# usexfg/xfg-stark

Measured on AMD Instinct MI355X. Metric: burn-proofs/sec (2^16-step trace, blowup=8), higher is better.
Workload: dtype u64; 1 GPU; batch of 64 burn proofs per GPU (configs[2]; configs[3] = 512 proofs on 8 GPUs); trace_length=65536, blowup=8, proof_options=42/8/4/None/8/31, parallelism=dp1 (independent proofs; RCCL scatter of inputs, gather of proof bytes), submission=pipelined, depth 6 (xfg_prove_batch_submit / xfg_batch_wait)

## Files before the change

include/xfg_stark.h:

```cpp
#ifndef XFG_STARK_H
#define XFG_STARK_H
#include <stddef.h>
#include <stdint.h>
#ifdef __cplusplus
extern "C" {
#endif

typedef struct xfg_ctx xfg_ctx;

typedef enum {
    XFG_OK = 0,
    XFG_INVALID_BURN_AMOUNT = 1,
    XFG_MINT_MISMATCH = 2,
    XFG_ZERO_TX_HASH = 3,
    XFG_BAD_RECIPIENT_LEN = 4,
    XFG_SHORT_SECRET = 5,
    XFG_PROVER_ERROR = 6,
    XFG_DEVICE_ERROR = 7,
    XFG_BUFFER_TOO_SMALL = 8,
    XFG_INVALID_ARGUMENT = 9,
    XFG_VERIFY_FAILED = 10,
    XFG_INVALID_TRACE = 11
} xfg_status;

typedef struct {
    uint32_t num_queries;
    uint32_t blowup_factor;
    uint32_t grinding_factor;
    uint32_t field_extension;
    uint32_t fri_folding_factor;
    uint32_t fri_remainder_max_degree;
} xfg_options;

typedef struct {
    uint64_t burn_amount;
    uint64_t mint_amount;
    uint8_t tx_prefix_hash[32];
    const uint8_t* recipient_address;
    size_t recipient_len;
    const uint8_t* secret;
    size_t secret_len;
    uint32_t network_id;
    uint32_t target_chain_id;
    uint32_t commitment_version;
} xfg_burn_inputs;

typedef struct {
    uint64_t pub_inputs[12];
    uint64_t nullifier;
    uint64_t commitment;
} xfg_air_consts;

xfg_ctx* xfg_ctx_create(int device_id);
void xfg_ctx_destroy(xfg_ctx* ctx);
int xfg_default_options(xfg_options* out);
int xfg_last_error(const xfg_ctx* ctx, char* buf, size_t len);
size_t xfg_proof_size_bound(uint64_t trace_length, const xfg_options* opts);

int xfg_prove_burn_mint(xfg_ctx* ctx, const xfg_burn_inputs* in, uint64_t trace_length, const xfg_options* opts,
                        uint8_t* out, size_t* out_len);
int xfg_prove_trace(xfg_ctx* ctx, const uint64_t* trace, uint32_t width, uint64_t n, const xfg_air_consts* air,
                    const xfg_options* opts, uint8_t* out, size_t* out_len);
int xfg_prove_batch(xfg_ctx* ctx, uint32_t count, const xfg_burn_inputs* inputs, uint64_t trace_length,
                    const xfg_options* opts, uint8_t* const* outs, size_t* out_lens, int* statuses);

int xfg_prove_batch_submit(xfg_ctx* ctx, uint32_t count, const xfg_burn_inputs* inputs, uint64_t trace_length,
                           const xfg_options* opts, uint8_t* const* outs, size_t* out_lens, int* statuses,
                           uint64_t* ticket);
int xfg_batch_wait(xfg_ctx* ctx, uint64_t ticket);

typedef struct {
    uint32_t kind;
    uint32_t index;
    uint32_t column;
    uint64_t step;
    uint64_t expected;
    uint64_t found;
} xfg_trace_fault;

#define XFG_TRACE_VALIDATE   1u
#define XFG_TRACE_ON_DEVICE  2u

int xfg_check_traces(xfg_ctx* ctx, uint32_t count, const uint64_t* traces, uint64_t n, const xfg_air_consts* airs,
                     uint32_t flags, xfg_trace_fault* faults);
int xfg_prove_trace_batch(xfg_ctx* ctx, uint32_t count, const uint64_t* traces, uint32_t width, uint64_t n,
                          const xfg_air_consts* airs, const xfg_options* opts, uint32_t flags, uint8_t* const* outs,
                          size_t* out_lens, int* statuses, xfg_trace_fault* faults);
int xfg_prove_trace_batch_submit(xfg_ctx* ctx, uint32_t count, const uint64_t* traces, uint32_t width, uint64_t n,
                                 const xfg_air_consts* airs, const xfg_options* opts, uint32_t flags,
                                 uint8_t* const* outs, size_t* out_lens, int* statuses, xfg_trace_fault* faults,
                                 uint64_t* ticket);

int xfg_prepare(xfg_ctx* ctx, uint32_t count, uint64_t trace_length, const xfg_options* opts);

int xfg_burn_air_consts(const xfg_burn_inputs* in, xfg_air_consts* out);

typedef struct {
    uint32_t trace_width;
    uint64_t trace_length;
    xfg_options options;
    uint32_t num_unique_queries;
    uint32_t num_fri_layers;
    uint32_t remainder_len;
    uint64_t pow_nonce;
    uint8_t trace_root[32];
    uint8_t constraint_root[32];
    uint64_t ood_trace[14];
    uint64_t ood_composition;
    size_t size;
} xfg_proof_info;

int xfg_proof_parse(const uint8_t* proof, size_t len, xfg_proof_info* info, char* err, size_t err_len);

int xfg_verify(const uint8_t* proof, size_t len, const xfg_air_consts* air, const xfg_options* acceptable, char* err,
               size_t err_len);
int xfg_verify_batch(uint32_t count, const uint8_t* const* proofs, const size_t* lens, const xfg_air_consts* airs,
                     const xfg_options* acceptable, int* results, uint32_t threads);

int xfg_verify_batch_gpu(xfg_ctx* ctx, uint32_t count, const uint8_t* const* proofs, const size_t* lens,
                         const xfg_air_consts* airs, const xfg_options* acceptable, int* results);

int xfg_selftest_blake3(const uint8_t* in, size_t len, uint8_t out[32]);
int xfg_selftest_field(uint64_t a, uint64_t b, uint64_t* out3);
int xfg_set_timing(xfg_ctx* ctx, int enabled);
int xfg_stage_times(const xfg_ctx* ctx, double* ms, const char** names, int max);
int xfg_bench_lde(xfg_ctx* ctx, uint32_t count, uint64_t n, uint32_t blowup, uint32_t iters, double* avg_ms);
int xfg_lde_probe(xfg_ctx* ctx, int enabled, double* total_ms, uint64_t* launch_sets, uint64_t* polys);
int xfg_debug_lde(xfg_ctx* ctx, const uint64_t* coef, uint32_t npoly, uint64_t n, uint32_t blowup, uint64_t* out);
int xfg_debug_interpolate(xfg_ctx* ctx, const uint64_t* evals, uint32_t npoly, uint64_t n, int offset7,
                          uint64_t* out);
int xfg_debug_const_columns(xfg_ctx* ctx, const uint64_t* trace, uint32_t count, uint32_t width, uint64_t n,
                            uint8_t* flags_out);
int xfg_debug_lde_skip(xfg_ctx* ctx, const uint64_t* coef, uint32_t npoly, uint64_t n, uint32_t blowup,
                       const uint8_t* skip, uint64_t* out);
int xfg_debug_interpolate_skip(xfg_ctx* ctx, const uint64_t* evals, uint32_t npoly, uint64_t n, int offset7,
                               const uint8_t* skip, uint64_t* out);
int xfg_debug_field(xfg_ctx* ctx, uint32_t op, uint64_t count, const uint64_t* a, const uint64_t* b, uint64_t* out);
int xfg_debug_ood_deep(xfg_ctx* ctx, uint32_t count, uint64_t n, const uint64_t* coef, const uint64_t* hcoef,
                       const uint64_t* zpts, const uint64_t* coeffs, uint64_t* ood_out, uint64_t* deep_out);
int xfg_debug_ood_deep_e(xfg_ctx* ctx, uint32_t count, uint64_t n, uint32_t ext, const uint64_t* coef,
                         const uint64_t* hcoef, const uint64_t* zpts, const uint64_t* coeffs,
                         const uint32_t* coin_seeds, const uint64_t* coin_counters, uint64_t ginv, uint64_t* ood_out,
                         uint64_t* deep_out, uint64_t* dp_out, uint32_t* seeds_out, uint64_t* counters_out,
                         int* fail_out);
int xfg_debug_constraint_eval(xfg_ctx* ctx, uint32_t count, uint64_t n, uint32_t blowup, uint32_t ext,
                              const uint64_t* trace, const xfg_air_consts* airs, const uint64_t* coeffs,
                              uint64_t* ce);
int xfg_debug_fri_fold(xfg_ctx* ctx, uint32_t count, uint32_t ext, uint32_t logn, uint32_t logbeta, int coset_major,
                       const uint64_t* vals, const uint64_t* alpha, uint64_t* out);
int xfg_debug_fri_fold_f(xfg_ctx* ctx, uint32_t count, uint32_t ext, uint32_t logn, uint32_t logbeta, int coset_major,
                         uint32_t fold, const uint64_t* vals, const uint64_t* alpha, uint64_t* out);
int xfg_debug_coin_draws(xfg_ctx* ctx, const uint32_t seed[8], uint64_t counter, uint32_t k, uint32_t ext,
                         const uint64_t reject[4], uint64_t* out_wave, uint64_t* out_seq, uint64_t counters[2],
                         int ok[2]);
int xfg_debug_merkle_lde(xfg_ctx* ctx, uint32_t count, uint32_t nc, uint64_t n, uint32_t blowup, const uint64_t* lde,
                         const uint64_t* entries, uint64_t nentries, uint8_t* nodes_out, uint8_t* local_out);
int xfg_debug_merkle_lde_const(xfg_ctx* ctx, uint32_t count, uint32_t nc, uint64_t n, uint32_t blowup,
                               const uint64_t* lde, const uint8_t* flags, const uint64_t* vals,
                               const uint64_t* entries, uint64_t nentries, uint8_t* nodes_out, uint8_t* local_out);
int xfg_debug_poison_lde(xfg_ctx* ctx, int on);
int xfg_debug_merkle_fri(xfg_ctx* ctx, uint32_t count, uint32_t ext, uint32_t logn, uint32_t logbeta, int coset_major,
                         const uint64_t* vals, uint8_t* nodes_out);
int xfg_debug_merkle_fri_f(xfg_ctx* ctx, uint32_t count, uint32_t ext, uint32_t logn, uint32_t logbeta, int coset_major,
                           uint32_t fold, const uint64_t* vals, uint8_t* nodes_out);
int xfg_debug_grind(xfg_ctx* ctx, uint32_t count, const uint32_t* seeds, uint32_t grind, uint64_t first_nonce,
                    uint64_t max_nonce, uint32_t chunk_log, uint32_t blocks, uint64_t* nonces_out);
int xfg_grind_probe(const xfg_ctx* ctx, uint32_t* device_min, uint64_t* device_searches, uint64_t* host_searches);
int xfg_debug_verify_batch_gpu(xfg_ctx* ctx, uint32_t count, const uint8_t* const* proofs, const size_t* lens,
                               const xfg_air_consts* airs, const xfg_options* acceptable, int* results,
                               uint64_t* flags, char* errs, size_t err_stride);

#ifdef __cplusplus
}
#endif
#endif
```

xfg-stark_amd/csrc/debug_abi.hip:

```cpp
#include <cstring>
#include <vector>

#include "dev_coin.hpp"
#include "field_dft.hpp"
#include "prover_internal.hpp"

using namespace xfg;

__global__ void field_op_kernel(int op, const u64* a, const u64* b, u64* out, u64 count) {
    const u64 i = (u64)blockIdx.x * blockDim.x + threadIdx.x;
    if (i >= count) return;
    const u64 x = a[i], y = b[i];
    u64 r = 0;
    switch (op) {
        case 0: r = gl_mul(x, y); break;
        case 1: r = gl_add(x, y); break;
        case 2: r = gl_sub(x, y); break;
        case 3: r = gl_canon(x); break;
        case 4: {
            const int sh = (int)(y % 96);
            static_for<96>([&](auto sc) {
                if (sh == decltype(sc)::value) r = mul_pow2<decltype(sc)::value>(x);
            });
            break;
// ... 73 lines not shown
                                  u64* ctr, int* ok, hipStream_t s) {
    hipLaunchKernelGGL(coin_draw_test_kernel, dim3(1), dim3(64), 0, s, c0, k, ext, rej, out_wave, out_seq, ctr, ok);
}

static int debug_lde(xfg_ctx* c, const uint64_t* coef, uint32_t npoly, uint64_t n, uint32_t blowup, const uint8_t* skip,
                     uint64_t* out) {
    if (!c || !coef || !out || !is_pow2(n) || !is_pow2(blowup) || n < 8 || blowup < 2 || blowup > 128)
        return XFG_INVALID_ARGUMENT;
    if (!lde_supported((int)ilog2(n), (int)ilog2(blowup))) return XFG_INVALID_ARGUMENT;
    return on_lane0(c, [&](Lane* L) -> int {
        const int logn = (int)ilog2(n), logbeta = (int)ilog2(blowup);
        const u64 N = n * blowup;
        ensure_tables(c, logn + logbeta);
        ensure_fourstep(c, logn, logbeta);
        Tables T = tables_of(c);
        L->coef.ensure((size_t)npoly * n);
        L->scratch.ensure((size_t)npoly * N);
        L->lde.ensure((size_t)npoly * N);
        HIPCHK(hipMemcpy(L->coef.p, coef, (size_t)npoly * n * 8, hipMemcpyHostToDevice));
        if (skip) {
            L->const_col.ensure(npoly);
            HIPCHK(hipMemcpy(L->const_col.p, skip, npoly, hipMemcpyHostToDevice));
            HIPCHK(hipMemsetAsync(L->scratch.p, 0xFF, (size_t)npoly * N * 8, L->stream));
            HIPCHK(hipMemsetAsync(L->lde.p, 0xFF, (size_t)npoly * N * 8, L->stream));
        }
        launch_lde(L->coef.p, n, L->lde.p, L->scratch.p, npoly, logn, logbeta, T, L->stream, skip ? L->const_col.p : nullptr);
        if (skip) launch_const_fill(L->const_col.p, L->coef.p, n, nullptr, L->lde.p, npoly, logn, logbeta, L->stream);
        std::vector<u64> cm((size_t)npoly * N);
        HIPCHK(hipMemcpyAsync(cm.data(), L->lde.p, cm.size() * 8, hipMemcpyDeviceToHost, L->stream));
        HIPCHK(hipStreamSynchronize(L->stream));
        for (u64 p = 0; p < npoly; p++)
            for (u64 t = 0; t < blowup; t++)
                for (u64 m = 0; m < n; m++) out[p * N + t + blowup * m] = cm[(p * blowup + t) * n + m];
        return XFG_OK;
    });
}

static int debug_interpolate(xfg_ctx* c, const uint64_t* evals, uint32_t npoly, uint64_t n, int offset7,
                             const uint8_t* skip, uint64_t* out) {
    if (!c || !evals || !out || !is_pow2(n) || n < 8 || !ntt_supported((int)ilog2(n), 0, true)) return XFG_INVALID_ARGUMENT;
    return on_lane0(c, [&](Lane* L) -> int {
        const int logn = (int)ilog2(n);
        ensure_tables(c, std::max(logn, c->tables.LM));
        if (logn >= 4) ensure_fourstep(c, logn - 1, 1);
        Tables T = tables_of(c);
        L->trace.ensure((size_t)npoly * n);
        L->coef.ensure((size_t)npoly * n);
        L->scratch.ensure((size_t)npoly * n);
        HIPCHK(hipMemcpy(L->trace.p, evals, (size_t)npoly * n * 8, hipMemcpyHostToDevice));
        if (skip) {
            L->const_col.ensure(npoly);
            HIPCHK(hipMemcpy(L->const_col.p, skip, npoly, hipMemcpyHostToDevice));
            HIPCHK(hipMemsetAsync(L->scratch.p, 0xFF, (size_t)npoly * n * 8, L->stream));
            HIPCHK(hipMemsetAsync(L->coef.p, 0xFF, (size_t)npoly * n * 8, L->stream));
        }
        launch_interpolate(L->trace.p, n, L->coef.p, n, L->scratch.p, npoly, logn, offset7 != 0, n, T, L->stream,
                           skip ? L->const_col.p : nullptr);
        if (skip) launch_const_fill(L->const_col.p, L->trace.p, n, L->coef.p, nullptr, npoly, logn, 0, L->stream);
        HIPCHK(hipMemcpyAsync(out, L->coef.p, (size_t)npoly * n * 8, hipMemcpyDeviceToHost, L->stream));
        HIPCHK(hipStreamSynchronize(L->stream));
        return XFG_OK;
    });
}

extern "C" {

int xfg_bench_lde(xfg_ctx* c, uint32_t count, uint64_t n, uint32_t blowup, uint32_t iters, double* avg_ms) {
    if (!c || !avg_ms || !is_pow2(n) || !is_pow2(blowup) || n < 8 || blowup < 2 || blowup > 128 || iters == 0)
        return XFG_INVALID_ARGUMENT;
    if (!lde_supported((int)ilog2(n), (int)ilog2(blowup))) return XFG_INVALID_ARGUMENT;
    return on_lane0(c, [&](Lane* L) -> int {
        const int logn = (int)ilog2(n), logbeta = (int)ilog2(blowup);
        const u64 N = n * blowup;
        ensure_tables(c, logn + logbeta);
        ensure_fourstep(c, logn, logbeta);
        Tables T = tables_of(c);
        L->coef.ensure((size_t)count * 7 * n);
        L->scratch.ensure((size_t)count * 7 * N);
        L->lde.ensure((size_t)count * 7 * N);
        std::vector<u64> h((size_t)count * 7 * n);
        u64 x = 0x46472d535441524bULL;
        for (auto& v : h) {
            x += 0x9E3779B97F4A7C15ULL;
            u64 z = x;
            z = (z ^ (z >> 30)) * 0xBF58476D1CE4E5B9ULL;
            z = (z ^ (z >> 27)) * 0x94D049BB133111EBULL;
            v = (z ^ (z >> 31)) % P;
        }
        HIPCHK(hipMemcpy(L->coef.p, h.data(), h.size() * 8, hipMemcpyHostToDevice));
        launch_lde(L->coef.p, n, L->lde.p, L->scratch.p, count * 7, logn, logbeta, T, L->stream);
        HIPCHK(hipEventRecord(L->ev[0], L->stream));
        for (uint32_t i = 0; i < iters; i++)
            launch_lde(L->coef.p, n, L->lde.p, L->scratch.p, count * 7, logn, logbeta, T, L->stream);
        HIPCHK(hipEventRecord(L->ev[1], L->stream));
        HIPCHK(hipEventSynchronize(L->ev[1]));
        float ms = 0;
        HIPCHK(hipEventElapsedTime(&ms, L->ev[0], L->ev[1]));
        *avg_ms = ms / iters;
        return XFG_OK;
    });
}

int xfg_lde_probe(xfg_ctx* c, int enabled, double* total_ms, uint64_t* launch_sets, uint64_t* polys) {
    if (!c) return XFG_INVALID_ARGUMENT;
    return on_lane0(c, [&](Lane*) -> int {
        double ms = 0;
        u64 sets = 0, np = 0;
        for (auto& L : c->lanes) {
            ms += L->lde_ms;
            sets += L->lde_sets;
            np += L->lde_polys;
            if (enabled) L->lde_ms = 0, L->lde_sets = 0, L->lde_polys = 0;
            L->lde_probe = enabled != 0;
        }
        if (total_ms) *total_ms = ms;
        c->lde_probe = enabled != 0;
        if (launch_sets) *launch_sets = sets;
        if (polys) *polys = np;
        return XFG_OK;
    });
}

int xfg_debug_lde(xfg_ctx* c, const uint64_t* coef, uint32_t npoly, uint64_t n, uint32_t blowup, uint64_t* out) {
    return debug_lde(c, coef, npoly, n, blowup, nullptr, out);
}
int xfg_debug_lde_skip(xfg_ctx* c, const uint64_t* coef, uint32_t npoly, uint64_t n, uint32_t blowup,
                       const uint8_t* skip, uint64_t* out) {
    if (!skip) return XFG_INVALID_ARGUMENT;
    return debug_lde(c, coef, npoly, n, blowup, skip, out);
}

int xfg_debug_interpolate(xfg_ctx* c, const uint64_t* evals, uint32_t npoly, uint64_t n, int offset7, uint64_t* out) {
    return debug_interpolate(c, evals, npoly, n, offset7, nullptr, out);
}
int xfg_debug_interpolate_skip(xfg_ctx* c, const uint64_t* evals, uint32_t npoly, uint64_t n, int offset7,
                               const uint8_t* skip, uint64_t* out) {
    if (!skip) return XFG_INVALID_ARGUMENT;
    return debug_interpolate(c, evals, npoly, n, offset7, skip, out);
}

int xfg_debug_const_columns(xfg_ctx* c, const uint64_t* trace, uint32_t count, uint32_t width, uint64_t n,
                            uint8_t* flags_out) {
    if (!c || !trace || !flags_out || count == 0 || width == 0 || !is_pow2(n) || n < 8 ||
        (uint64_t)count * width > 0xFFFF)
        return XFG_INVALID_ARGUMENT;
    return on_lane0(c, [&](Lane* L) -> int {
        const size_t cols = (size_t)count * width;
        L->trace.ensure(cols * n);
        L->const_col.ensure(cols);
        HIPCHK(hipMemcpy(L->trace.p, trace, cols * n * 8, hipMemcpyHostToDevice));
        launch_const_detect(L->trace.p, (int)cols, (int)ilog2(n), L->const_col.p, L->stream);
        HIPCHK(hipMemcpyAsync(flags_out, L->const_col.p, cols, hipMemcpyDeviceToHost, L->stream));
        HIPCHK(hipStreamSynchronize(L->stream));
        return XFG_OK;
    });
}

int xfg_debug_field(xfg_ctx* c, uint32_t op, uint64_t count, const uint64_t* a, const uint64_t* b, uint64_t* out) {
    if (!c || !a || !b || !out || op > 12 || count == 0 || (op >= 9 && count % 2)) return XFG_INVALID_ARGUMENT;
    return on_lane0(c, [&](Lane* L) -> int {
        L->trace.ensure((size_t)count * 3);
        u64* da = L->trace.p;
        u64* db = da + count;
        u64* dout = db + count;
        HIPCHK(hipMemcpy(da, a, count * 8, hipMemcpyHostToDevice));
        HIPCHK(hipMemcpy(db, b, count * 8, hipMemcpyHostToDevice));
        launch_field_op((int)op, da, db, dout, count, L->stream);
        HIPCHK(hipMemcpyAsync(out, dout, count * 8, hipMemcpyDeviceToHost, L->stream));
        HIPCHK(hipStreamSynchronize(L->stream));
        return XFG_OK;
    });
}

int xfg_debug_coin_draws(xfg_ctx* c, const uint32_t seed[8], uint64_t counter, uint32_t k, uint32_t ext,
                         const uint64_t reject[4], uint64_t* out_wave, uint64_t* out_seq, uint64_t counters[2],
                         int ok[2]) {
    if (!c || !seed || !reject || !out_wave || !out_seq || !counters || !ok || k == 0 || k > 64 ||
        (ext != 1 && ext != 2))
        return XFG_INVALID_ARGUMENT;
    return on_lane0(c, [&](Lane* L) -> int {
        L->trace.ensure(4 + 4 * (size_t)k + 2 + 1);
        u64* drej = L->trace.p;
        u64* dw = drej + 4;
        u64* ds = dw + 2 * k;
        u64* dctr = ds + 2 * k;
        int* dok = (int*)(dctr + 2);
        HIPCHK(hipMemcpy(drej, reject, 32, hipMemcpyHostToDevice));
        HIPCHK(hipMemset(dw, 0, 16 * (size_t)k));
        DevCoin c0;
        memcpy(c0.seed.w, seed, 32);
        c0.counter = counter;
        c0.pad = 0;
        launch_coin_draw_test(c0, (int)k, (int)ext, drej, dw, ds, dctr, dok, L->stream);
        HIPCHK(hipMemcpyAsync(out_wave, dw, 16 * (size_t)k, hipMemcpyDeviceToHost, L->stream));
        HIPCHK(hipMemcpyAsync(out_seq, ds, 16 * (size_t)k, hipMemcpyDeviceToHost, L->stream));
        HIPCHK(hipMemcpyAsync(counters, dctr, 16, hipMemcpyDeviceToHost, L->stream));
        HIPCHK(hipMemcpyAsync(ok, dok, 8, hipMemcpyDeviceToHost, L->stream));
        HIPCHK(hipStreamSynchronize(L->stream));
        return XFG_OK;
    });
}

int xfg_debug_grind(xfg_ctx* c, uint32_t count, const uint32_t* seeds, uint32_t grind, uint64_t first_nonce,
                    uint64_t max_nonce, uint32_t chunk_log, uint32_t blocks, uint64_t* nonces_out) {
    if (!c || !seeds || !nonces_out || count == 0 || grind > GRIND_MAX || first_nonce == 0 ||
        (chunk_log != 0 && (chunk_log < GRIND_CHUNK_LOG_MIN || chunk_log > GRIND_CHUNK_LOG_MAX)) ||
        blocks > GRIND_FORCED_BLOCKS_MAX)
        return XFG_INVALID_ARGUMENT;
    return on_lane0(c, [&](Lane* L) -> int {
        const GrindPlan gp = grind_plan(grind, count, (unsigned)L->cus);
        memcpy(grind_seeds(L, count), seeds, (size_t)count * sizeof(Digest));
        const u64* got = grind_search(L, (int)count, grind, first_nonce, max_nonce ? max_nonce : gp.max_nonce,
                                      chunk_log ? chunk_log : gp.chunk_log, blocks ? blocks : gp.blocks);
        memcpy(nonces_out, got, (size_t)count * 8);
        return XFG_OK;
    });
}

int xfg_grind_probe(const xfg_ctx* c, uint32_t* device_min, uint64_t* device_searches, uint64_t* host_searches) {
    if (!c) return XFG_INVALID_ARGUMENT;
    uint64_t dev = 0, host = 0;
    for (auto& L : c->lanes) {
        dev += L->grind_dev;
        host += L->grind_host;
    }
    if (device_min) *device_min = GRIND_DEVICE_MIN;
    if (device_searches) *device_searches = dev;
    if (host_searches) *host_searches = host;
    return XFG_OK;
}

int xfg_debug_ood_deep(xfg_ctx* c, uint32_t count, uint64_t n, const uint64_t* coef, const uint64_t* hcoef,
                       const uint64_t* zpts, const uint64_t* coeffs, uint64_t* ood_out, uint64_t* deep_out) {
    return xfg_debug_ood_deep_e(c, count, n, 1, coef, hcoef, zpts, coeffs, nullptr, nullptr, 0, ood_out, deep_out,
                                nullptr, nullptr, nullptr, nullptr);
}

int xfg_debug_ood_deep_e(xfg_ctx* c, uint32_t count, uint64_t n, uint32_t ext, const uint64_t* coef,
                         const uint64_t* hcoef, const uint64_t* zpts, const uint64_t* coeffs,
                         const uint32_t* coin_seeds, const uint64_t* coin_counters, uint64_t ginv, uint64_t* ood_out,
                         uint64_t* deep_out, uint64_t* dp_out, uint32_t* seeds_out, uint64_t* counters_out,
                         int* fail_out) {
    if (!c) return XFG_INVALID_ARGUMENT;
    c->err.clear();
    const bool coin = coin_seeds != nullptr;
    if ((ext != 1 && ext != 2) || !is_pow2(n) || n < 8 || n > (1ULL << 21) || count == 0 || count > 0xFFFF) {
        c->err = "xfg_debug_ood_deep: ext is 1 or 2, n a power of two in [8, 2^21], count in [1, 65535]";
        return XFG_INVALID_ARGUMENT;
    }
    if (!coef || !hcoef || !zpts || !ood_out || !deep_out ||
        (coin ? !coin_counters || !dp_out || !seeds_out || !counters_out || !fail_out : !coeffs)) {
        c->err = "xfg_debug_ood_deep: null argument";
        return XFG_INVALID_ARGUMENT;
    }
    const size_t B = count, D = ext;
    if (!all_canonical(coef, B * 7 * n) || !all_canonical(hcoef, B * D * n) || !all_canonical(zpts, B * 2 * D) ||
        (coin ? ginv >= P : !all_canonical(coeffs, B * 8 * D))) {
        c->err = "xfg_debug_ood_deep: a word is not a canonical field element";
        return XFG_INVALID_ARGUMENT;
    }
    auto e_at = [D](const u64* v) { return E2{v[0], D == 2 ? v[1] : 0}; };
    if (!coin)
        for (size_t k = 0; k < B * 2; k++)
            if (e2_eq(e_at(zpts + k * D), E2{0, 0})) {
                c->err = "xfg_debug_ood_deep: z and z g must not be zero";
                return XFG_INVALID_ARGUMENT;
            }
    return on_lane0(c, [&](Lane* L) -> int {
        const ProofShape sh(n, Opts{0, 2, 0, ext, 8, 31});
        const int logn = sh.logn;
        L->coef.ensure(B * 7 * n);
        size_ood_deep(L, B, sh);
        hipStream_t s = L->stream;
        HIPCHK(hipMemcpyAsync(L->coef.p, coef, B * 7 * n * 8, hipMemcpyHostToDevice, s));
        HIPCHK(hipMemcpyAsync(L->hcoef.p, hcoef, B * D * n * 8, hipMemcpyHostToDevice, s));
        HIPCHK(hipMemcpyAsync(L->zpts.p, zpts, B * 2 * D * 8, hipMemcpyHostToDevice, s));
        const size_t nblk = ood_partial_count(logn);
        HIPCHK(hipMemsetAsync(L->partial.p, 0xFF, B * nblk * 15 * D * 8, s));
        HIPCHK(hipMemsetAsync(L->carry.p, 0xFF, B * nblk * 2 * D * 8, s));
        HIPCHK(hipMemsetAsync(L->ood.p, 0xFF, B * 15 * D * 8, s));
        HIPCHK(hipMemsetAsync(L->dp.p, 0xFF, B * sizeof(DeepParams), s));
        HIPCHK(hipMemsetAsync(L->deep.p, 0xFF, B * D * n * 8, s));
        if (coin) {
            L->dcoin.ensure(B);
            L->dfail.ensure(B);
            std::vector<DevCoin> hc(B);
            for (size_t b = 0; b < B; b++) {
                memcpy(hc[b].seed.w, coin_seeds + 8 * b, 32);
                hc[b].counter = coin_counters[b];
                hc[b].pad = 0;
            }
            HIPCHK(hipMemcpyAsync(L->dcoin.p, hc.data(), B * sizeof(DevCoin), hipMemcpyHostToDevice, s));
            HIPCHK(hipMemsetAsync(L->dfail.p, 0, B * sizeof(int), s));
            DeepCoinStep dc;
            dc.coins = L->dcoin.p;
            dc.fail = L->dfail.p;
            dc.zpts = L->zpts.p;
            dc.dp = L->dp.p;
            dc.ginv = ginv;
            launch_ood(L->coef.p, L->hcoef.p, L->zpts.p, L->partial.p, L->ood.p, logn, (int)B, (int)ext, s, dc);
            launch_deep(L->coef.p, L->hcoef.p, L->dp.p, L->partial.p, L->carry.p, L->deep.p, logn, (int)B, (int)ext, s);
            std::vector<DeepParams> dps(B);
            HIPCHK(hipMemcpyAsync(ood_out, L->ood.p, B * 15 * D * 8, hipMemcpyDeviceToHost, s));
            HIPCHK(hipMemcpyAsync(deep_out, L->deep.p, B * D * n * 8, hipMemcpyDeviceToHost, s));
            HIPCHK(hipMemcpyAsync(dps.data(), L->dp.p, B * sizeof(DeepParams), hipMemcpyDeviceToHost, s));
            HIPCHK(hipMemcpyAsync(hc.data(), L->dcoin.p, B * sizeof(DevCoin), hipMemcpyDeviceToHost, s));
            HIPCHK(hipMemcpyAsync(fail_out, L->dfail.p, B * sizeof(int), hipMemcpyDeviceToHost, s));
            HIPCHK(hipStreamSynchronize(s));
            for (size_t b = 0; b < B; b++) {
                static_assert(sizeof(DeepParams) == 30 * 8, "dp_out: the 28 words before DeepParams::pad");
                memcpy(dp_out + 28 * b, &dps[b], 28 * 8);
                memcpy(seeds_out + 8 * b, hc[b].seed.w, 32);
                counters_out[b] = hc[b].counter;
            }
            return XFG_OK;
        }
        launch_ood(L->coef.p, L->hcoef.p, L->zpts.p, L->partial.p, L->ood.p, logn, (int)B, (int)ext, s);
        HIPCHK(hipMemcpyAsync(ood_out, L->ood.p, B * 15 * D * 8, hipMemcpyDeviceToHost, s));
        HIPCHK(hipStreamSynchronize(s));
        std::vector<DeepParams> dps(B);
        for (size_t b = 0; b < B; b++) {
            DeepParams& dp = dps[b];
            memset(&dp, 0, sizeof dp);
            auto put = [D](u64* d, E2 v) {
                d[0] = v.a;
                if (D == 2) d[1] = v.b;
            };
            const u64* cf = coeffs + b * 8 * D;
            const u64* o = ood_out + b * 15 * D;
            const E2 z = e_at(zpts + b * 2 * D), zg = e_at(zpts + b * 2 * D + D), gamma = e_at(cf + 7 * D);
            E2 c1 = e2_mul(gamma, e_at(o + 14 * D)), c2{0, 0};
            for (int k = 0; k < 7; k++) {
                const E2 a = e_at(cf + k * D);
                put(dp.a[k], a);
                c1 = e2_add(c1, e2_mul(a, e_at(o + 2 * k * D)));
                c2 = e2_add(c2, e2_mul(a, e_at(o + (2 * k + 1) * D)));
            }
            put(dp.gamma, gamma);
            put(dp.z, z);
            put(dp.zg, zg);
            put(dp.zinv, e2_inv(z));
            put(dp.zginv, e2_inv(zg));
            put(dp.c1, c1);
            put(dp.c2, c2);
        }
        HIPCHK(hipMemcpyAsync(L->dp.p, dps.data(), B * sizeof(DeepParams), hipMemcpyHostToDevice, s));
        launch_deep(L->coef.p, L->hcoef.p, L->dp.p, L->partial.p, L->carry.p, L->deep.p, logn, (int)B, (int)ext, s);
        HIPCHK(hipMemcpyAsync(deep_out, L->deep.p, B * D * n * 8, hipMemcpyDeviceToHost, s));
        HIPCHK(hipStreamSynchronize(s));
        return XFG_OK;
    });
}

int xfg_debug_constraint_eval(xfg_ctx* c, uint32_t count, uint64_t n, uint32_t blowup, uint32_t ext,
                              const uint64_t* trace, const xfg_air_consts* airs, const uint64_t* coeffs,
                              uint64_t* ce) {
    if (!c) return XFG_INVALID_ARGUMENT;
    c->err.clear();
    if (!trace || !airs || !coeffs || !ce || count == 0 || !is_pow2(n) || n < 8 || !is_pow2(blowup) || blowup < 2 ||
        blowup > 128 || wide_lde_too_large(n, blowup) || (ext != 1 && ext != 2)) {
        c->err = "xfg_debug_constraint_eval: null or unsupported argument";
        return XFG_INVALID_ARGUMENT;
    }
    return on_lane0(c, [&](Lane* L) -> int {
        const size_t B = count;
        if (!all_canonical(trace, B * 7 * n) || !all_canonical(coeffs, B * 15 * ext)) {
            c->err = "trace element or coefficient is not a canonical field element";
            return XFG_INVALID_ARGUMENT;
        }
        std::vector<AirConst> ha(B);
        for (size_t b = 0; b < B; b++) {
            if (!air_canonical(&airs[b])) {
                c->err = "AIR constant is not a canonical field element";
                return XFG_INVALID_ARGUMENT;
            }
            ha[b] = air_of(&airs[b]);
        }
        const ProofShape sh(n, Opts{0, blowup, 0, ext, 8, 31});
        ensure_tables(c, std::max(sh.logn + sh.logbeta, sh.logn + 1));
        ensure_fourstep(c, sh.logn, sh.logbeta);
        const Tables T = tables_of(c);
        const u64* ce_div = ensure_ce_table(c, sh.logn);
        size_trace_lde(L, B, sh);
        size_constraint_eval(L, B, sh);
        hipStream_t s = L->stream;
        HIPCHK(hipMemcpy(L->trace.p, trace, B * 7 * n * 8, hipMemcpyHostToDevice));
        HIPCHK(hipMemcpy(L->air.p, ha.data(), B * sizeof(AirConst), hipMemcpyHostToDevice));
        HIPCHK(hipMemcpy(L->coeffs.p, coeffs, B * 15 * ext * 8, hipMemcpyHostToDevice));
        launch_trace_lde(L, T, (int)B, sh, false);
        launch_constraint_eval(L->lde.p, L->air.p, L->coeffs.p, ce_div, L->ce.p, sh.logn, sh.logbeta, (int)B, sh.DE, s,
                               trace_const(L, sh));
        HIPCHK(hipMemcpyAsync(ce, L->ce.p, B * ext * 2 * n * 8, hipMemcpyDeviceToHost, s));
        HIPCHK(hipStreamSynchronize(s));
        return XFG_OK;
    });
}

static unsigned debug_logf(uint32_t fold) { return fold == 2 ? 1 : fold == 4 ? 2 : fold == 8 ? 3 : fold == 16 ? 4 : 0; }

int xfg_debug_fri_fold(xfg_ctx* c, uint32_t count, uint32_t ext, uint32_t logn, uint32_t logbeta, int coset_major,
                       const uint64_t* vals, const uint64_t* alpha, uint64_t* out) {
    return xfg_debug_fri_fold_f(c, count, ext, logn, logbeta, coset_major, 8, vals, alpha, out);
}

int xfg_debug_fri_fold_f(xfg_ctx* c, uint32_t count, uint32_t ext, uint32_t logn, uint32_t logbeta, int coset_major,
                         uint32_t fold, const uint64_t* vals, const uint64_t* alpha, uint64_t* out) {
    if (!c) return XFG_INVALID_ARGUMENT;
    c->err.clear();
    const unsigned logf = debug_logf(fold);
    if (!vals || !alpha || !out || count == 0 || (ext != 1 && ext != 2) || logn > 28 || logbeta > 28 || !logf ||
        logn + logbeta < logf + 1 || logn + logbeta > 28) {
        c->err = "xfg_debug_fri_fold: null or unsupported argument";
        return XFG_INVALID_ARGUMENT;
    }
    return on_lane0(c, [&](Lane* L) -> int {
        const size_t B = count;
        const int logD = (int)(logn + logbeta);
        const u64 D = 1ULL << logD, rows = D / fold;
        if (!all_canonical(vals, B * ext * D) || !all_canonical(alpha, B * ext)) {
            c->err = "layer value or alpha is not a canonical field element";
            return XFG_INVALID_ARGUMENT;
        }
        ensure_tables(c, logD);
        const Tables T = tables_of(c);
        L->f0.ensure(B * ext * D);
        L->alpha7.ensure(B * ext);
        L->deep.ensure(B * ext * rows);
        const u64 i7 = gl_inv(GEN);
        std::vector<u64> a7(B * ext);
        for (size_t k = 0; k < a7.size(); k++) a7[k] = gl_mul(alpha[k], i7);
        hipStream_t s = L->stream;
        HIPCHK(hipMemcpy(L->f0.p, vals, B * ext * D * 8, hipMemcpyHostToDevice));
        HIPCHK(hipMemcpy(L->alpha7.p, a7.data(), a7.size() * 8, hipMemcpyHostToDevice));
        launch_fri_fold(L->f0.p, ext * D, D, coset_major != 0, (int)logn, (int)logbeta, rows, logD, L->alpha7.p,
                        L->deep.p, rows, T, (int)B, (int)ext, (int)fold, s);
        HIPCHK(hipMemcpyAsync(out, L->deep.p, B * ext * rows * 8, hipMemcpyDeviceToHost, s));
        HIPCHK(hipStreamSynchronize(s));
        return XFG_OK;
    });
}

static int debug_merkle_lde(xfg_ctx* c, uint32_t count, uint32_t nc, uint64_t n, uint32_t blowup, uint32_t max_blowup,
                            const uint64_t* lde, const uint8_t* flags, const uint64_t* vals, const uint64_t* entries,
                            uint64_t nentries, uint8_t* nodes_out, uint8_t* local_out) {
    if (!c) return XFG_INVALID_ARGUMENT;
    c->err.clear();
    if (!lde || !nodes_out || (nentries && (!entries || !local_out)) || count == 0 || count > 0xFFFF ||
        (nc != 1 && nc != 2 && nc != 7) || !is_pow2(blowup) || blowup < 2 || blowup > max_blowup || !is_pow2(n) ||
        n < 8 || n > (1ULL << 24) || (flags && (!vals || nc != 7))) {
        c->err = "xfg_debug_merkle_lde: null or unsupported argument";
        return XFG_INVALID_ARGUMENT;
    }
    for (uint64_t e = 0; e < nentries; e++)
        if (entries[e] >= (uint64_t)count * n) {
            c->err = "xfg_debug_merkle_lde: entry names a proof or row out of range";
            return XFG_INVALID_ARGUMENT;
        }
    return on_lane0(c, [&](Lane* L) -> int {
        const int logn = (int)ilog2(n), logbeta = (int)ilog2(blowup);
        const size_t B = count, nlde = B * nc * blowup * n, nloc = (size_t)nentries * 2 * blowup;
        L->lde.ensure(nlde);
        L->tnodes.ensure(B * 2 * n);
        hipStream_t s = L->stream;
        HIPCHK(hipMemcpyAsync(L->lde.p, lde, nlde * 8, hipMemcpyHostToDevice, s));
        HIPCHK(hipMemsetAsync(L->tnodes.p, 0xFF, B * 2 * n * sizeof(Digest), s));
        ColConst cc;
        if (flags) {
            const size_t cols = B * nc, N = (size_t)blowup * n;
            L->const_col.ensure((cols + 3) & ~(size_t)3);
            L->coef.ensure(cols);
            HIPCHK(hipMemcpyAsync(L->const_col.p, flags, cols, hipMemcpyHostToDevice, s));
            HIPCHK(hipMemcpyAsync(L->coef.p, vals, cols * 8, hipMemcpyHostToDevice, s));
            for (size_t k = 0; k < cols; k++)
                if (flags[k]) HIPCHK(hipMemsetAsync(L->lde.p + k * N, 0xFF, N * 8, s));
            cc.flags = L->const_col.p;
            cc.vals = L->coef.p;
            cc.val_stride = 1;
        }
        launch_merkle_lde(L->lde.p, (int)nc, L->tnodes.p, (int)B, logn, logbeta, s, CoinStep{}, cc);
        HIPCHK(hipMemcpyAsync(nodes_out, L->tnodes.p, B * 2 * n * sizeof(Digest), hipMemcpyDeviceToHost, s));
        if (nentries) {
            L->scratch.ensure(nentries);
            L->hnodes.ensure(nloc);
            HIPCHK(hipMemcpyAsync(L->scratch.p, entries, nentries * 8, hipMemcpyHostToDevice, s));
            HIPCHK(hipMemsetAsync(L->hnodes.p, 0xFF, nloc * sizeof(Digest), s));
            launch_open_rows(L->lde.p, (int)nc, L->scratch.p, nentries, L->hnodes.p, logn, logbeta, s, cc);
            HIPCHK(hipMemcpyAsync(local_out, L->hnodes.p, nloc * sizeof(Digest), hipMemcpyDeviceToHost, s));
        }
        HIPCHK(hipStreamSynchronize(s));
        return XFG_OK;
    });
}

int xfg_debug_merkle_lde(xfg_ctx* c, uint32_t count, uint32_t nc, uint64_t n, uint32_t blowup, const uint64_t* lde,
                         const uint64_t* entries, uint64_t nentries, uint8_t* nodes_out, uint8_t* local_out) {
    return debug_merkle_lde(c, count, nc, n, blowup, 16, lde, nullptr, nullptr, entries, nentries, nodes_out, local_out);
}
int xfg_debug_merkle_lde_const(xfg_ctx* c, uint32_t count, uint32_t nc, uint64_t n, uint32_t blowup,
                               const uint64_t* lde, const uint8_t* flags, const uint64_t* vals, const uint64_t* entries,
                               uint64_t nentries, uint8_t* nodes_out, uint8_t* local_out) {
// ... 49 lines not shown
```

xfg-stark_amd/csrc/kernels.hip:

```cpp
#include "dev_coin.hpp"
#include "field_dft.hpp"
#include "hip_util.hpp"
#include <algorithm>
#include <stdexcept>

namespace xfg {

#define XFG_CHECK_LAUNCH() (void)hipGetLastError()

__device__ __forceinline__ unsigned brev(unsigned x, int bits) { return __brev(x) >> (32 - bits); }

__device__ __forceinline__ u64 shfl_xor_u64(u64 v, int m, int w) {
    u32 lo = __shfl_xor((u32)v, m, w), hi = __shfl_xor((u32)(v >> 32), m, w);
    return (u64)lo | ((u64)hi << 32);
}

__device__ __forceinline__ u64 tw_pow(const Tables& T, int k, u64 e) {
    u64 M = 1ULL << T.LM;
    return T.tw[(e << (T.LM - k)) & (M - 1)];
}
__device__ __forceinline__ u64 tw_ipow(const Tables& T, int k, u64 e) {
    u64 M = 1ULL << T.LM;
    return T.tw[(M - ((e << (T.LM - k)) & (M - 1))) & (M - 1)];
}

__global__ void trace_gen_kernel(const AirConst* air, u64* trace, int logn) {
    const u64 n = 1ULL << logn;
    const u64 s = (u64)blockIdx.x * blockDim.x + threadIdx.x;
    const int proof = blockIdx.y;
    if (s >= n) return;
    const AirConst& A = air[proof];
    u64* tr = trace + (u64)proof * 7 * n;
    tr[0 * n + s] = A.pub[0];
    tr[1 * n + s] = A.pub[1];
    tr[2 * n + s] = A.pub[2];
    tr[3 * n + s] = A.pub[3];
    tr[4 * n + s] = (4 * s) >> logn;
    tr[5 * n + s] = A.nullifier;
    tr[6 * n + s] = A.commitment;
}
void launch_trace_gen(const AirConst* air, u64* trace, int logn, int npoly, hipStream_t s) {
    u64 n = 1ULL << logn;
    dim3 g((unsigned)((n + 255) / 256), npoly);
    hipLaunchKernelGGL(trace_gen_kernel, g, dim3(256), 0, s, air, trace, logn);
    XFG_CHECK_LAUNCH();
}

__device__ __forceinline__ void air_transition(const AirConst& A, const u64 (&cur)[7], u64 nxt4, u64 (&r)[7]) {
    const u64 std_burn = 8000000ULL, large_burn = 8000000000ULL;
    r[0] = gl_mul(gl_sub(cur[0], std_burn), gl_sub(cur[0], large_burn));
    r[1] = gl_sub(cur[1], cur[0]);
    r[2] = gl_sub(cur[2], A.pub[2] & 0xFFFFFFFFULL);
    r[3] = gl_sub(cur[3], A.pub[3] & 0xFFFFFFFFULL);
    const u64 d = gl_sub(nxt4, cur[4]);
    r[4] = gl_mul(d, gl_sub(d, 1));
    r[5] = gl_sub(cur[5], A.nullifier);
    r[6] = gl_sub(cur[6], A.commitment);
}
__device__ __forceinline__ void air_step0_values(const AirConst& A, u64 (&v0)[7]) {
    v0[0] = A.pub[0]; v0[1] = A.pub[1]; v0[2] = A.pub[2]; v0[3] = A.pub[3];
    v0[4] = 0; v0[5] = A.nullifier; v0[6] = A.commitment;
}

struct CeArgs {
    const u64* lde;
    const AirConst* air;
    const u64* coeffs;
    const u64* div;
    u64* ce;
    int logn, logbeta;
    ColConst cc;
};
template <int D, bool CC>
__global__ __launch_bounds__(256) void constraint_eval_kernel(CeArgs a) {
    using F = FE<D>;
    const u64 n = 1ULL << a.logn, nce = 2 * n;
    const int proof = blockIdx.y;
    const u64 g = (u64)blockIdx.x * blockDim.x + threadIdx.x;
    const u64 par = g >> a.logn, m = g & (n - 1), i = 2 * m + par;
    const AirConst& A = a.air[proof];
    const u64* co = a.coeffs + (u64)proof * 15 * D;
    const u64 beta = 1ULL << a.logbeta;
    const u64* lde = a.lde + (u64)proof * 7 * beta * n;
    const u64 t = par * (beta / 2), mn = (m + 1) & (n - 1);
    u64 cur[7], nxt4;
    if constexpr (CC) {
        const RowConst rc = row_const_uniform(a.cc, (u64)proof);
#pragma unroll
        for (int c = 0; c < 7; c++) {
            if ((rc.mask >> c) & 1) cur[c] = rc.v[c];
            else cur[c] = lde[(((u64)c << a.logbeta) + t) * n + m];
        }
        if ((rc.mask >> 4) & 1) nxt4 = rc.v[4];
        else nxt4 = lde[((4ULL << a.logbeta) + t) * n + mn];
    } else {
#pragma unroll
        for (int c = 0; c < 7; c++) cur[c] = lde[(((u64)c << a.logbeta) + t) * n + m];
        nxt4 = lde[((4ULL << a.logbeta) + t) * n + mn];
    }
    const u64 di = par * n + m;
    const u64 dv0 = a.div[di], dv1 = a.div[nce + di], dv2 = a.div[2 * nce + di];
    u64 r[7];
    air_transition(A, cur, nxt4, r);
    F tr = F::zero();
#pragma unroll
    for (int c = 0; c < 7; c++) tr = fe_add(tr, fe_mulb(F::load(co + c * D), r[c]));
    u64 v0[7];
    air_step0_values(A, v0);
    F b0 = F::zero();
#pragma unroll
    for (int c = 0; c < 7; c++) b0 = fe_add(b0, fe_mulb(F::load(co + (7 + c) * D), gl_sub(cur[c], v0[c])));
    const F b1 = fe_mulb(F::load(co + 14 * D), gl_sub(cur[4], AIR_LAST_STATE));
    F val = fe_mulb(tr, dv0);
    val = fe_add(val, fe_mulb(b0, dv1));
    val = fe_add(val, fe_mulb(b1, dv2));
#pragma unroll
    for (int c = 0; c < D; c++) a.ce[((u64)proof * D + c) * nce + i] = val.c(c);
}
void launch_constraint_eval(const u64* lde, const AirConst* air, const u64* coeffs, const u64* div, u64* ce, int logn,
                            int logbeta, int npoly, int ext, hipStream_t s, const ColConst& cc) {
    CeArgs a;
    a.lde = lde; a.air = air; a.coeffs = coeffs; a.div = div; a.ce = ce; a.logn = logn; a.logbeta = logbeta;
    a.cc = cc;
    u64 nce = 2ULL << logn;
    int threads = nce < 256 ? (int)nce : 256;
    dim3 g((unsigned)(nce / threads), npoly);
    if (cc.flags) {
        if (ext == 2) hipLaunchKernelGGL((constraint_eval_kernel<2, true>), g, dim3(threads), 0, s, a);
        else hipLaunchKernelGGL((constraint_eval_kernel<1, true>), g, dim3(threads), 0, s, a);
    } else {
        if (ext == 2) hipLaunchKernelGGL((constraint_eval_kernel<2, false>), g, dim3(threads), 0, s, a);
        else hipLaunchKernelGGL((constraint_eval_kernel<1, false>), g, dim3(threads), 0, s, a);
    }
    XFG_CHECK_LAUNCH();
}

template <bool AIR>
__global__ __launch_bounds__(256) void trace_check_kernel(u64* trace, const AirConst* air, u64* keys, int logn) {
    const u64 n = 1ULL << logn;
    const u64 s = (u64)blockIdx.x * blockDim.x + threadIdx.x;
    const int proof = blockIdx.y;
    u64 key = TRACE_KEY_VALID;
    if (s < n) {
        u64* tr = trace + (u64)proof * 7 * n;
        u64 cur[7];
#pragma unroll
        for (int c = 0; c < 7; c++) cur[c] = tr[(u64)c * n + s];
        u64 nxt4 = 0;
        if (AIR && s + 1 < n) nxt4 = tr[4 * n + s + 1];
#pragma unroll
        for (int c = 6; c >= 0; c--) {
            if (cur[c] >= P) {
                key = trace_key(TRACE_KEY_NONCANONICAL, s, (unsigned)c);
                cur[c] -= P;
                tr[(u64)c * n + s] = cur[c];
            }
        }
        if (AIR && key == TRACE_KEY_VALID) {
            const AirConst& A = air[proof];
            if (s + 1 < n) {
                if (nxt4 >= P) nxt4 -= P;
                u64 r[7];
                air_transition(A, cur, nxt4, r);
#pragma unroll
                for (int c = 6; c >= 0; c--)
                    if (r[c] != 0) key = trace_key(TRACE_KEY_TRANSITION, s, (unsigned)c);
            } else if (cur[4] != AIR_LAST_STATE) {
                key = trace_key(TRACE_KEY_ASSERTION, s, 7);
            }
            if (s == 0) {
                u64 v0[7];
                air_step0_values(A, v0);
#pragma unroll
                for (int c = 6; c >= 0; c--)
                    if (cur[c] != v0[c]) key = trace_key(TRACE_KEY_ASSERTION, 0, (unsigned)c);
            }
        }
    }
#pragma unroll
    for (int m = 32; m > 0; m >>= 1) {
        const u64 o = shfl_xor_u64(key, m, 64);
        key = o < key ? o : key;
    }
    if ((threadIdx.x & 63) == 0 && key != TRACE_KEY_VALID) atomicMin((unsigned long long*)(keys + proof), (unsigned long long)key);
}
void launch_trace_check(u64* trace, const AirConst* air, u64* keys, int logn, int npoly, bool with_air, hipStream_t s) {
    const u64 n = 1ULL << logn;
    HIPCHK(hipMemsetAsync(keys, 0xFF, (size_t)npoly * 8, s));
    dim3 g((unsigned)((n + 255) / 256), npoly);
    if (with_air) hipLaunchKernelGGL(trace_check_kernel<true>, g, dim3(256), 0, s, trace, air, keys, logn);
    else hipLaunchKernelGGL(trace_check_kernel<false>, g, dim3(256), 0, s, trace, air, keys, logn);
    XFG_CHECK_LAUNCH();
}

#define OOD_R 8
static inline int ood_threads(u64 n) { return (int)std::min<u64>(256, n / OOD_R); }

template <int D>
__device__ __forceinline__ FE<D> fe_pow(FE<D> b, u64 e) {
    FE<D> r = FE<D>::zero();
    r.a = 1;
    while (e) {
        if (e & 1) r = fe_mul(r, b);
        b = fe_mul(b, b);
        e >>= 1;
    }
    return r;
}
template <int D>
__device__ __forceinline__ FE<D> fe_plane(const u64* planes, u64 plane_stride, u64 j) {
    FE<D> v;
    v.a = planes[j];
    if constexpr (D == 2) v.b = planes[plane_stride + j];
    return v;
}

template <int D>
__global__ __launch_bounds__(256) void ood_kernel(const u64* coef, const u64* hcoef, const u64* zpts, u64* partial,
                                                  int logn) {
    using F = FE<D>;
    __shared__ u64 zb[4][D];
    __shared__ u64 red[4][15][D];
    const u64 n = 1ULL << logn;
    const int proof = blockIdx.y, t = threadIdx.x, T = blockDim.x;
    const u64 base = (u64)blockIdx.x * T * OOD_R;
    const F z = F::load(zpts + (u64)proof * 2 * D), zg = F::load(zpts + (u64)proof * 2 * D + D);
    for (int k = t; k < 4; k += T)
        fe_pow(k & 1 ? zg : z, k < 2 ? base : (u64)T).store(zb[k]);
    __syncthreads();
    F pz = fe_mul(F::load(zb[0]), fe_pow(z, (u64)t)), pzg = fe_mul(F::load(zb[1]), fe_pow(zg, (u64)t));
    const F zT = F::load(zb[2]), zgT = F::load(zb[3]);
    const u64* co = coef + (u64)proof * 7 * n;
    const u64* h = hcoef + (u64)proof * D * n;
    F acc[15];
#pragma unroll
    for (int q = 0; q < 15; q++) acc[q] = F::zero();
    u64 cur[7], nxt[7];
    F hc, hn;
    {
        const u64 j = base + t;
#pragma unroll
        for (int c = 0; c < 7; c++) cur[c] = co[(u64)c * n + j];
        hc = fe_plane<D>(h, n, j);
    }
#pragma unroll
    for (int r = 0; r < OOD_R; r++) {
        if (r + 1 < OOD_R) {
            const u64 j = base + (u64)(r + 1) * T + t;
#pragma unroll
            for (int c = 0; c < 7; c++) nxt[c] = co[(u64)c * n + j];
            hn = fe_plane<D>(h, n, j);
        }
#pragma unroll
        for (int c = 0; c < 7; c++) {
            acc[2 * c] = fe_add(acc[2 * c], fe_mulb(pz, cur[c]));
            acc[2 * c + 1] = fe_add(acc[2 * c + 1], fe_mulb(pzg, cur[c]));
        }
        acc[14] = fe_add(acc[14], fe_mul(hc, pz));
        pz = fe_mul(pz, zT);
        pzg = fe_mul(pzg, zgT);
        if (r + 1 < OOD_R) {
#pragma unroll
            for (int c = 0; c < 7; c++) cur[c] = nxt[c];
            hc = hn;
        }
    }
    const int W = T < 64 ? T : 64;
    for (int m = W / 2; m > 0; m >>= 1) {
#pragma unroll
        for (int q = 0; q < 15; q++) {
            acc[q].a = gl_add(acc[q].a, shfl_xor_u64(acc[q].a, m, W));
            if constexpr (D == 2) acc[q].b = gl_add(acc[q].b, shfl_xor_u64(acc[q].b, m, W));
        }
    }
    if ((t & 63) == 0) {
#pragma unroll
        for (int q = 0; q < 15; q++) acc[q].store(red[t >> 6][q]);
    }
    __syncthreads();
    for (int qc = t; qc < 15 * D; qc += T) {
        const int q = qc / D, cc = qc % D;
        u64 v = red[0][q][cc];
        for (int w = 1; w < (T + 63) / 64; w++) v = gl_add(v, red[w][q][cc]);
        partial[((u64)proof * gridDim.x + blockIdx.x) * 15 * D + qc] = v;
    }
}
__device__ void deep_coin_block(const DeepCoinStep& dc, int b, const u64* o, int D) {
    __shared__ u64 ab[8][2];
    __shared__ E2 zinv;
    __shared__ int ok_s;
    const u64* zb = dc.zpts + (u64)b * 2 * D;
    const E2 z{zb[0], D == 2 ? zb[1] : 0}, zg{zb[D], D == 2 ? zb[D + 1] : 0};
    const bool zz = z.a == 0 && z.b == 0;
    if (threadIdx.x < 64) {
        DevCoin c = dc.coins[b];
        dev_reseed(c, dev_hash_elems(o, 14 * D));
        dev_reseed(c, dev_hash_elems(o + 14 * D, D));
        const bool ok = wave_draw_e(c, 8, D, &ab[0][0], 2);
        if (threadIdx.x == 0) {
            dc.coins[b] = c;
            ok_s = ok;
        }
    } else if (threadIdx.x == 64) {
        zinv = zz ? E2{0, 0} : e2_inv(z);
    }
    __syncthreads();
    if (threadIdx.x != 0) return;
    DeepParams P = {};
    for (int k = 0; k < 7; k++)
        for (int d = 0; d < D; d++) P.a[k][d] = ab[k][d];
    for (int d = 0; d < D; d++) P.gamma[d] = ab[7][d];
    auto put = [](u64* d, E2 v) { d[0] = v.a; d[1] = v.b; };
    auto ood_e = [&](int q) { return E2{o[q * D], D == 2 ? o[q * D + 1] : 0}; };
    put(P.z, z);
    put(P.zg, zg);
    put(P.zinv, zinv);
    put(P.zginv, e2_mulb(zinv, dc.ginv));
    E2 c1 = e2_mul(E2{P.gamma[0], P.gamma[1]}, ood_e(14)), c2{0, 0};
    for (int k = 0; k < 7; k++) {
        const E2 a{P.a[k][0], P.a[k][1]};
        c1 = e2_add(c1, e2_mul(a, ood_e(2 * k)));
        c2 = e2_add(c2, e2_mul(a, ood_e(2 * k + 1)));
    }
    put(P.c1, c1);
    put(P.c2, c2);
    dc.dp[b] = P;
    if (!ok_s || zz) dc.fail[b] = 1;
}
__global__ __launch_bounds__(128) void ood_final_kernel(const u64* partial, int nblk, int d, u64* ood, DeepCoinStep dc) {
    __shared__ u64 o[30];
    __shared__ u64 red[8][30];
    const int proof = blockIdx.x, t = threadIdx.x, nq = 15 * d;
    int S = 1;
    while (nq * S * 2 <= (int)blockDim.x && S < 8) S <<= 1;
    const int q = t % nq, k = t / nq;
    if (k < S) {
        const u64* pp = partial + (u64)proof * nblk * nq + q;
        u64 s = 0;
        for (int b0 = k; b0 < nblk; b0 += 8 * S) {
            u64 v[8];
#pragma unroll
            for (int u = 0; u < 8; u++) {
                const int b = b0 + u * S;
                v[u] = b < nblk ? pp[(u64)b * nq] : 0;
            }
#pragma unroll
            for (int u = 0; u < 8; u++) s = gl_add(s, v[u]);
        }
        red[k][q] = s;
    }
    __syncthreads();
    if (t < nq) {
        u64 s = red[0][t];
        for (int j = 1; j < S; j++) s = gl_add(s, red[j][t]);
        ood[(u64)proof * nq + t] = s;
        o[t] = s;
    }
    if (!dc.coins) return;
    __syncthreads();
    deep_coin_block(dc, proof, o, d);
}
void launch_ood(const u64* coef, const u64* hcoef, const u64* zpts, u64* partial, u64* ood, int logn, int npoly,
                int ext, hipStream_t s, const DeepCoinStep& dc) {
    const u64 n = 1ULL << logn;
    const int T = ood_threads(n), nblk = (int)(n / ((u64)T * OOD_R));
    if (ext == 2)
        hipLaunchKernelGGL(ood_kernel<2>, dim3(nblk, npoly), dim3(T), 0, s, coef, hcoef, zpts, partial, logn);
    else
        hipLaunchKernelGGL(ood_kernel<1>, dim3(nblk, npoly), dim3(T), 0, s, coef, hcoef, zpts, partial, logn);
    hipLaunchKernelGGL(ood_final_kernel, dim3(npoly), dim3(dc.coins ? 128 : 64), 0, s, partial, nblk, ext, ood, dc);
    XFG_CHECK_LAUNCH();
}
u64 ood_partial_count(int logn) {
    const u64 n = 1ULL << logn;
    return n / ((u64)ood_threads(n) * OOD_R);
}

template <int D>
__global__ __launch_bounds__(1024) void deep_carry_kernel(const u64* partial, const DeepParams* dp, u64* carry,
                                                          int nblk, int logch) {
    using F = FE<D>;
    __shared__ u64 S1[1024][D], S2[1024][D];
    const int proof = blockIdx.x, b = threadIdx.x;
    const DeepParams& P = dp[proof];
    F b1 = F::zero(), b2 = F::zero();
    if (b < nblk) {
        const u64* pp = partial + ((u64)proof * nblk + b) * 15 * D;
        F t1 = F::zero(), t2 = F::zero();
#pragma unroll
        for (int c = 0; c < 7; c++) {
            const F a = F::load(P.a[c]);
            t1 = fe_add(t1, fe_mul(a, F::load(pp + 2 * c * D)));
            t2 = fe_add(t2, fe_mul(a, F::load(pp + (2 * c + 1) * D)));
        }
        b1 = fe_add(t1, fe_mul(F::load(P.gamma), F::load(pp + 14 * D)));
        b2 = t2;
        if (b == 0) {
            b1 = fe_sub(b1, F::load(P.c1));
            b2 = fe_sub(b2, F::load(P.c2));
        }
    }
    b1.store(S1[b]);
    b2.store(S2[b]);
    __syncthreads();
    for (int off = 1; off < (int)blockDim.x; off <<= 1) {
        F v1 = F::load(S1[b]), v2 = F::load(S2[b]);
        if (b + off < (int)blockDim.x) {
            v1 = fe_add(v1, F::load(S1[b + off]));
            v2 = fe_add(v2, F::load(S2[b + off]));
        }
        __syncthreads();
        v1.store(S1[b]);
        v2.store(S2[b]);
        __syncthreads();
    }
    if (b < nblk) {
        const u64 e = (u64)(b + 1) << logch;
        const F x1 = b + 1 < nblk ? F::load(S1[b + 1]) : F::zero();
        const F x2 = b + 1 < nblk ? F::load(S2[b + 1]) : F::zero();
        fe_mul(x1, fe_pow(F::load(P.zinv), e)).store(carry + (((u64)proof * nblk + b) * 2) * D);
        fe_mul(x2, fe_pow(F::load(P.zginv), e)).store(carry + (((u64)proof * nblk + b) * 2 + 1) * D);
    }
}
__device__ __forceinline__ int dpad(int i) { return i + i / OOD_R; }
template <int D>
__global__ __launch_bounds__(256) void deep_final_kernel(const u64* coef, const u64* hcoef, const DeepParams* dp,
                                                         const u64* carry, u64* deep, int logn) {
    using F = FE<D>;
    constexpr int R = OOD_R, CHMAX = 256 * OOD_R, PADN = CHMAX + CHMAX / R;
    __shared__ u64 s1[D][PADN], s2[D][PADN];
    __shared__ u64 S1[256][D], S2[256][D];
    const u64 n = 1ULL << logn;
    const int proof = blockIdx.y, t = threadIdx.x, T = blockDim.x;
    const u64 base = (u64)blockIdx.x * T * R;
    const DeepParams& P = dp[proof];
    const F z = F::load(P.z), zg = F::load(P.zg), gam = F::load(P.gamma);
    F ac[7];
#pragma unroll
    for (int c = 0; c < 7; c++) ac[c] = F::load(P.a[c]);
    const u64* co = coef + (u64)proof * 7 * n;
    const u64* h = hcoef + (u64)proof * D * n;
    auto lds_ld = [&](u64 (*arr)[PADN], int k) {
        F v;
        v.a = arr[0][k];
        if constexpr (D == 2) v.b = arr[1][k];
        return v;
    };
    auto lds_st = [&](u64 (*arr)[PADN], int k, F v) {
        arr[0][k] = v.a;
        if constexpr (D == 2) arr[1][k] = v.b;
    };
#pragma unroll 2
    for (int r = 0; r < R; r++) {
        const int li = r * T + t;
        const u64 j = base + li;
        F sacc = F::zero();
#pragma unroll
        for (int c = 0; c < 7; c++) sacc = fe_add(sacc, fe_mulb(ac[c], co[(u64)c * n + j]));
        F p1 = fe_add(sacc, fe_mul(gam, fe_plane<D>(h, n, j))), p2 = sacc;
        if (j == 0) {
            p1 = fe_sub(p1, F::load(P.c1));
            p2 = fe_sub(p2, F::load(P.c2));
        }
        lds_st(s1, dpad(li), p1);
        lds_st(s2, dpad(li), p2);
    }
    __syncthreads();
    const int a = t * R;
    F L1 = F::zero(), L2 = F::zero();
#pragma unroll
    for (int i = R - 1; i >= 0; i--) {
        L1 = fe_add(lds_ld(s1, dpad(a + i)), fe_mul(z, L1));
        L2 = fe_add(lds_ld(s2, dpad(a + i)), fe_mul(zg, L2));
    }
    F w1 = z, w2 = zg;
#pragma unroll
    for (int i = 1; i < R; i <<= 1) {
        w1 = fe_mul(w1, w1);
        w2 = fe_mul(w2, w2);
    }
    const F cin1 = F::load(carry + (((u64)proof * gridDim.x + blockIdx.x) * 2) * D);
    const F cin2 = F::load(carry + (((u64)proof * gridDim.x + blockIdx.x) * 2 + 1) * D);
    if (t == T - 1) {
        L1 = fe_add(L1, fe_mul(w1, cin1));
        L2 = fe_add(L2, fe_mul(w2, cin2));
    }
    L1.store(S1[t]);
    L2.store(S2[t]);
    __syncthreads();
    for (int off = 1; off < T; off <<= 1) {
        F v1 = F::load(S1[t]), v2 = F::load(S2[t]);
        if (t + off < T) {
            v1 = fe_add(v1, fe_mul(w1, F::load(S1[t + off])));
            v2 = fe_add(v2, fe_mul(w2, F::load(S2[t + off])));
        }
        __syncthreads();
        v1.store(S1[t]);
        v2.store(S2[t]);
        __syncthreads();
        w1 = fe_mul(w1, w1);
        w2 = fe_mul(w2, w2);
    }
    F q1 = t + 1 < T ? F::load(S1[t + 1]) : cin1, q2 = t + 1 < T ? F::load(S2[t + 1]) : cin2;
#pragma unroll
    for (int i = R - 1; i >= 0; i--) {
        const int k = dpad(a + i);
        const F p1 = lds_ld(s1, k), p2 = lds_ld(s2, k);
        lds_st(s1, k, fe_add(q1, q2));
        q1 = fe_add(p1, fe_mul(z, q1));
        q2 = fe_add(p2, fe_mul(zg, q2));
    }
    __syncthreads();
#pragma unroll
    for (int c = 0; c < D; c++) {
        u64* out = deep + ((u64)proof * D + c) * n + base;
#pragma unroll
        for (int r = 0; r < R; r++) out[r * T + t] = s1[c][dpad(r * T + t)];
    }
}
void launch_deep(const u64* coef, const u64* hcoef, const DeepParams* dp, const u64* partial, u64* carry, u64* deep,
                 int logn, int npoly, int ext, hipStream_t s) {
    const u64 n = 1ULL << logn;
    const int T = ood_threads(n), nblk = (int)(n / ((u64)T * OOD_R));
    int logch = 0;
    while ((1ULL << logch) < (u64)T * OOD_R) logch++;
    int ct = 64;
    while (ct < nblk) ct <<= 1;
    if (ext == 2) {
        hipLaunchKernelGGL(deep_carry_kernel<2>, dim3(npoly), dim3(ct), 0, s, partial, dp, carry, nblk, logch);
        hipLaunchKernelGGL(deep_final_kernel<2>, dim3(nblk, npoly), dim3(T), 0, s, coef, hcoef, dp, carry, deep, logn);
    } else {
        hipLaunchKernelGGL(deep_carry_kernel<1>, dim3(npoly), dim3(ct), 0, s, partial, dp, carry, nblk, logch);
        hipLaunchKernelGGL(deep_final_kernel<1>, dim3(nblk, npoly), dim3(T), 0, s, coef, hcoef, dp, carry, deep, logn);
    }
    XFG_CHECK_LAUNCH();
}

struct FoldArgs {
    const u64* vals;
    u64 val_stride, comp_stride;
    int coset_major, logn, logbeta;
    u64 rows;
    int logD;
    const u64* alpha7;
    u64* out;
    u64 out_stride;
    Tables T;
};
template <int D, int LOGF>
__global__ __launch_bounds__(256) void fri_fold_kernel(FoldArgs a) {
    using F = FE<D>;
    constexpr int NF = 1 << LOGF;
    const int proof = blockIdx.y;
    const u64 i = (u64)blockIdx.x * blockDim.x + threadIdx.x;
    if (i >= a.rows) return;
    const u64* base = a.vals + (u64)proof * a.val_stride;
    u64 c[D][NF];
#pragma unroll
    for (int k = 0; k < NF; k++) {
        const u64 K = i + (u64)k * a.rows;
        c[0][k] = layer_at(base, a.coset_major, a.logn, a.logbeta, K);
        if constexpr (D == 2) c[1][k] = layer_at(base + a.comp_stride, a.coset_major, a.logn, a.logbeta, K);
    }
    F v[NF];
#pragma unroll
    for (int d = 0; d < D; d++) {
        dft_reg<LOGF, true>(c[d]);
#pragma unroll
        for (int k = 0; k < NF; k++) {
            if (d == 0) v[k].a = canon(c[d][k]);
            if constexpr (D == 2) if (d == 1) v[k].b = canon(c[d][k]);
        }
    }
    const F y = fe_mulb(F::load(a.alpha7 + (u64)proof * D), tw_ipow(a.T, a.logD, i));
    F r = v[NF - 1];
#pragma unroll
    for (int j = NF - 2; j >= 0; j--) r = fe_add(fe_mul(r, y), v[j]);
#pragma unroll
    for (int d = 0; d < D; d++) {
        const u64 x = gl_neg(mul_pow2<96 - LOGF>(r.c(d)));
        if (d == 0) r.a = x;
        if constexpr (D == 2) if (d == 1) r.b = x;
    }
#pragma unroll
    for (int c = 0; c < D; c++) a.out[((u64)proof * D + c) * a.out_stride + i] = r.c(c);
}
template <int D>
static void fold_launch(int fold, dim3 g, dim3 b, hipStream_t s, const FoldArgs& a) {
    switch (fold) {
        case 2: hipLaunchKernelGGL((fri_fold_kernel<D, 1>), g, b, 0, s, a); break;
        case 4: hipLaunchKernelGGL((fri_fold_kernel<D, 2>), g, b, 0, s, a); break;
        case 8: hipLaunchKernelGGL((fri_fold_kernel<D, 3>), g, b, 0, s, a); break;
        case 16: hipLaunchKernelGGL((fri_fold_kernel<D, 4>), g, b, 0, s, a); break;
        default: throw std::invalid_argument("FRI fold: no kernel for this folding factor");
    }
}
void launch_fri_fold(const u64* vals, u64 val_stride, u64 comp_stride, bool coset_major, int logn, int logbeta,
                     u64 rows, int logD, const u64* alpha7, u64* out, u64 out_stride, const Tables& T, int npoly,
                     int ext, int fold, hipStream_t s) {
    FoldArgs a;
    a.vals = vals; a.val_stride = val_stride; a.comp_stride = comp_stride; a.coset_major = coset_major ? 1 : 0;
    a.logn = logn; a.logbeta = logbeta; a.rows = rows; a.logD = logD; a.alpha7 = alpha7; a.out = out;
    a.out_stride = out_stride;
    a.T = T;
    int threads = rows < 256 ? (int)rows : 256;
    dim3 g((unsigned)((rows + threads - 1) / threads), npoly);
    if (ext == 2) fold_launch<2>(fold, g, dim3(threads), s, a);
    else fold_launch<1>(fold, g, dim3(threads), s, a);
    XFG_CHECK_LAUNCH();
}

__global__ void gather_set_kernel(GatherSet g, const u64* idx) {
    const u64 i = (u64)blockIdx.x * blockDim.x + threadIdx.x;
    if (i >= g.first[g.nseg]) return;
    int k = 0;
    while (i >= g.first[k + 1]) k++;
    const u64 src = idx[i];
    if (g.digest[k]) {
        const Digest* s = (const Digest*)g.src[k];
        ((Digest*)g.dst[k])[i - g.first[k]] = s[src];
    } else {
        u64 v;
        const u64 plane = src >> g.cc_shift;
        if (k == g.cc_seg && g.cc.flags[plane]) v = g.cc.vals[plane * g.cc.val_stride];
        else v = ((const u64*)g.src[k])[src];
        ((u64*)g.dst[k])[i - g.first[k]] = v;
    }
}
void launch_gather_set(const GatherSet& g, const u64* idx, hipStream_t s) {
    const u64 total = g.first[g.nseg];
    if (!total) return;
    hipLaunchKernelGGL(gather_set_kernel, dim3((unsigned)((total + 255) / 256)), dim3(256), 0, s, g, idx);
    XFG_CHECK_LAUNCH();
}

__global__ void pack_kernel(PackSet p, u32* dst) {
    const int k = blockIdx.y;
    const u32* src = (const u32*)p.src[k];
    u32* out = dst + p.off[k];
    for (u64 i = (u64)blockIdx.x * blockDim.x + threadIdx.x; i < p.words[k]; i += (u64)gridDim.x * blockDim.x)
        out[i] = src[i];
}
void launch_pack(const PackSet& p, void* dst, hipStream_t s) {
    u64 most = 0;
    for (int k = 0; k < p.nseg; k++) most = std::max(most, p.words[k]);
    if (!most) return;
    const unsigned bx = (unsigned)std::min<u64>(32, (most + 255) / 256);
    hipLaunchKernelGGL(pack_kernel, dim3(bx, p.nseg), dim3(256), 0, s, p, (u32*)dst);
    XFG_CHECK_LAUNCH();
}

}
```

xfg-stark_amd/csrc/kernels.hpp:

```cpp
#pragma once
#include <hip/hip_runtime.h>
#include "gl.hpp"
#include "blake3.hpp"
#include "ntt_plan.hpp"

namespace xfg {

struct AirConst {
    u64 pub[12];
    u64 nullifier;
    u64 commitment;
    u64 pad[2];
};

struct DeepParams {
    u64 a[7][2];
    u64 gamma[2];
    u64 z[2], zg[2], zinv[2], zginv[2];
    u64 c1[2], c2[2];
    u64 pad[2];
};

struct FourStep {
    const u64* fwd[FOURSTEP_MAX_LOG + 1][5] = {};
    const u64* inv[FOURSTEP_MAX_LOG + 1] = {};
    const u64* pass_fwd[PASS_MAX_LOG + 1][5] = {};
};
struct Tables {
    const u64* tw;
    int LM;
    const u64* pow7;
    const u64* ipow7;
    const FourStep* fs;
};

void launch_lde(const u64* coef, u64 coef_stride, u64* out, u64* scratch, int npoly, int logn, int logbeta,
                const Tables& T, hipStream_t s, const unsigned char* skip = nullptr);
void build_fourstep(u64* out, int logn, int logbeta, const Tables& T, hipStream_t s);
void build_pass_tables(u64* out, int logn, int logbeta, const Tables& T, hipStream_t s);
void launch_interpolate(const u64* evals, u64 in_stride, u64* out, u64 out_stride, u64* scratch, int npoly, int logn,
                        bool off7, u64 keep, const Tables& T, hipStream_t s, const unsigned char* skip = nullptr);
constexpr int CONST_DETECT_SPAN = 1024, CONST_FILL_SPAN = 4096;
void launch_const_detect(const u64* cols, int ncols, int logn, unsigned char* flags, hipStream_t s);
void launch_const_fill(const unsigned char* flags, const u64* src, u64 src_stride, u64* coef, u64* lde, int ncols,
                       int logn, int logbeta, hipStream_t s);

struct ColConst {
    const unsigned char* flags = nullptr;
    const u64* vals = nullptr;
    u64 val_stride = 0;
};
struct RowConst {
    unsigned mask;
    u64 v[7];
};
__device__ __forceinline__ RowConst row_const_uniform(const ColConst& cc, u64 proof) {
    const u64 o = proof * 7;
    const uint32_t* w = reinterpret_cast<const uint32_t*>(cc.flags) + (o >> 2);
    const unsigned r = (unsigned)(o & 3);
    u64 bytes = ((u64)w[0] | ((u64)w[1] << 32)) >> (8 * r);
    if (r >= 2) bytes |= (u64)w[2] << (64 - 8 * r);
    RowConst rc;
    rc.mask = 0;
#pragma unroll
    for (int c = 0; c < 7; c++) rc.mask |= ((bytes >> (8 * c)) & 0xFF ? 1u : 0u) << c;
    rc.mask = __builtin_amdgcn_readfirstlane(rc.mask);
#pragma unroll
    for (int c = 0; c < 7; c++) {
        rc.v[c] = 0;
        if ((rc.mask >> c) & 1) {
            const u64 v = cc.vals[(o + c) * cc.val_stride];
            const uint32_t lo = (uint32_t)__builtin_amdgcn_readfirstlane((int)(uint32_t)v);
            const uint32_t hi = (uint32_t)__builtin_amdgcn_readfirstlane((int)(uint32_t)(v >> 32));
            rc.v[c] = (u64)lo | ((u64)hi << 32);
        }
    }
    return rc;
}
__device__ __forceinline__ RowConst row_const_lane(const ColConst& cc, u64 proof) {
    RowConst rc;
    rc.mask = 0;
#pragma unroll
    for (int c = 0; c < 7; c++) {
        rc.v[c] = cc.vals[(proof * 7 + c) * cc.val_stride];
        rc.mask |= (cc.flags[proof * 7 + c] ? 1u : 0u) << c;
    }
    return rc;
}

struct DevCoin {
    Digest seed;
    u64 counter;
    u64 pad;
};
struct CoinStep {
    enum Kind : int { NONE = 0, COEFFS = 1, OOD_POINT = 2, FRI_ALPHA = 3 };
    int kind = NONE;
    int ext = 1;
    DevCoin* coins = nullptr;
    int* fail = nullptr;
    u64* out = nullptr;
    u64 g = 0;
    Digest* root_out = nullptr;
    u64* hist = nullptr;
};
struct DeepCoinStep {
    DevCoin* coins = nullptr;
    int* fail = nullptr;
    const u64* zpts = nullptr;
    DeepParams* dp = nullptr;
    u64 ginv = 0;
};

void launch_merkle_lde(const u64* lde, int nc, Digest* nodes, int npoly, int logn, int logbeta, hipStream_t s,
                       const CoinStep& cs = CoinStep{}, const ColConst& cc = ColConst{});
void launch_open_rows(const u64* lde, int nc, const u64* entries, u64 count, Digest* out, int logn, int logbeta,
                      hipStream_t s, const ColConst& cc = ColConst{});
void launch_merkle_fri(const u64* vals, u64 val_stride, u64 comp_stride, bool coset_major, int logn, int logbeta,
                       u64 rows, Digest* nodes, int npoly, int ext, int fold, hipStream_t s,
                       const CoinStep& cs = CoinStep{});

void launch_trace_gen(const AirConst* air, u64* trace, int logn, int npoly, hipStream_t s);
constexpr u64 AIR_LAST_STATE = 3;
constexpr u64 TRACE_KEY_VALID = ~0ULL;
enum : unsigned { TRACE_KEY_NONCANONICAL = 0, TRACE_KEY_ASSERTION = 1, TRACE_KEY_TRANSITION = 2 };
__host__ __device__ constexpr u64 trace_key(unsigned kind, u64 step, unsigned index) {
    return ((u64)kind << 62) | (step << 3) | index;
}
void launch_trace_check(u64* trace, const AirConst* air, u64* keys, int logn, int npoly, bool with_air, hipStream_t s);
void launch_constraint_eval(const u64* lde, const AirConst* air, const u64* coeffs, const u64* div, u64* ce, int logn,
                            int logbeta, int npoly, int ext, hipStream_t s, const ColConst& cc = ColConst{});

void launch_ood(const u64* coef, const u64* hcoef, const u64* zpts, u64* partial, u64* ood, int logn, int npoly,
                int ext, hipStream_t s, const DeepCoinStep& dc = DeepCoinStep{});
u64 ood_partial_count(int logn);
void launch_deep(const u64* coef, const u64* hcoef, const DeepParams* dp, const u64* partial, u64* carry, u64* deep,
                 int logn, int npoly, int ext, hipStream_t s);

__device__ __forceinline__ u64 layer_at(const u64* base, bool coset_major, int logn, int logbeta, u64 K) {
    if (!coset_major) return base[K];
    u64 t = K & ((1ULL << logbeta) - 1), m = K >> logbeta;
    return base[(t << logn) + m];
}
void launch_fri_fold(const u64* vals, u64 val_stride, u64 comp_stride, bool coset_major, int logn, int logbeta,
                     u64 rows, int logD, const u64* alpha7, u64* out, u64 out_stride, const Tables& T, int npoly,
                     int ext, int fold, hipStream_t s);

struct GatherSet {
    static constexpr int MAX = 24;
    int nseg = 0;
    const void* src[MAX];
    void* dst[MAX];
    int digest[MAX];
    u64 first[MAX + 1] = {0};
    int cc_seg = -1, cc_shift = 0;
    ColConst cc;
};
void launch_gather_set(const GatherSet& g, const u64* idx, hipStream_t s);

struct PackSet {
    static constexpr int MAX = 12;
    int nseg = 0;
    const void* src[MAX];
    u64 off[MAX], words[MAX];
};
void launch_pack(const PackSet& p, void* dst, hipStream_t s);

constexpr size_t grind_state_words(size_t B) { return 2 * ((B + 1) & ~(size_t)1); }
void launch_grind(const Digest* seeds, u64* state, u64* out, unsigned B, unsigned grind, u64 first, u64 max_nonce,
                  unsigned chunk_log, unsigned blocks, hipStream_t s);

}
```

xfg-stark_amd/csrc/lane_unit.hip:

```cpp
#include <algorithm>
#include <chrono>
#include <cstring>

#include "host_pool.hpp"
#include "prover_internal.hpp"

namespace xfg {

static void stage_mark(Lane* c, int k, hipStream_t on = nullptr) {
    if (c->timing) HIPCHK(hipEventRecord(c->ev[k], on ? on : c->stream));
}

static hipStream_t gather_stream(Lane* c) {
    if (!c->gstream) {
        int least = 0, greatest = 0;
        if (hipDeviceGetStreamPriorityRange(&least, &greatest) != hipSuccess) greatest = 0;
        HIPCHK(hipStreamCreateWithPriority(&c->gstream, hipStreamNonBlocking, greatest));
    }
    return c->gstream;
}

void size_trace_lde(Lane* c, size_t B, const ProofShape& sh) {
    c->trace.ensure(B * 7 * sh.n);
    c->coef.ensure(B * 7 * sh.n);
    c->scratch.ensure(B * 7 * sh.N);
    c->lde.ensure(B * 7 * sh.N);
    c->const_col.ensure((B * 7 + 3) & ~(size_t)3);
}
void size_constraint_eval(Lane* c, size_t B, const ProofShape& sh) {
    c->air.ensure(B);
    c->coeffs.ensure(B * 15 * sh.DE);
    c->ce.ensure(B * sh.DE * 2 * sh.n);
}
void size_ood_deep(Lane* c, size_t B, const ProofShape& sh) {
    c->hcoef.ensure(B * sh.DE * sh.n);
    c->zpts.ensure(B * 2 * sh.DE);
    c->partial.ensure(B * 15 * sh.DE * ood_partial_count(sh.logn));
    c->ood.ensure(B * 15 * sh.DE);
    c->dp.ensure(B);
    c->carry.ensure(B * 2 * sh.DE * ood_partial_count(sh.logn));
    c->deep.ensure(B * sh.DE * sh.n);
}

static void size_lane_buffers(Lane* c, size_t B, const ProofShape& sh, const Opts& o, const TraceSrc& ts) {
    const u64 n = sh.n, N = sh.N;
    const size_t DE = sh.DE;
    const unsigned nl = sh.nl;
    size_trace_lde(c, B, sh);
    size_constraint_eval(c, B, sh);
    size_ood_deep(c, B, sh);
    c->tnodes.ensure(B * 2 * n);
    c->hlde.ensure(B * DE * N);
    c->hnodes.ensure(B * 2 * n);
    c->f0.ensure(B * DE * N);
    c->alpha7.ensure(B * DE);
    c->falpha.ensure((size_t)std::max(1u, nl) * B * DE);
    c->dn2.ensure(B * DE);
    c->dcoin.ensure(B);
    c->dfail.ensure(B);
    c->droots.ensure((size_t)(2 + nl) * B);
    if (c->flayer.size() < nl + 1) {
        c->flayer.resize(nl + 1);
        c->fnodes.resize(nl + 1);
    }
    for (unsigned l = 0; l < nl; l++) {
        c->fnodes[l].ensure(B * 2 * (sh.D[l] / o.fold));
        c->flayer[l + 1].ensure(B * DE * sh.D[l + 1]);
    }
    c->rem.ensure(B * DE * std::max<u64>(sh.rem_len, 1));
    const size_t q = o.q, depth = sh.logn + sh.logbeta;
    const size_t vals = B * q * (7 + DE + o.fold * DE * nl);
    size_t digs = B * q * 2 * depth;
    for (unsigned l = 0; l < nl; l++) digs += B * q * ilog2(sh.D[l] / o.fold);
    const size_t opens = B * q * 2 * 2 * 2 * sh.beta;
    c->h_idx.ensure(vals + digs + B * 2 * q);
    c->h_gv.ensure(vals);
    c->h_gd.ensure(digs + opens);
    size_grind(c, B);
    if (ts.checks()) c->tkeys.ensure(B);
    if (ts.kind == TraceSrc::HOST_STAGED || ts.size_staging) c->h_trace.ensure(B * 7 * n);
}

static void upload(void* dst, const void* host, size_t bytes, hipStream_t s) {
    void* hd = nullptr;
    HIPCHK(hipHostGetDevicePointer(&hd, const_cast<void*>(host), 0));
    PackSet u;
    u.src[0] = hd;
    u.off[0] = 0;
    u.words[0] = bytes / 4;
    u.nseg = 1;
    launch_pack(u, dst, s);
}
static_assert(sizeof(AirConst) % 4 == 0 && sizeof(DevCoin) % 4 == 0, "uploads copy 32-bit words");

void size_grind(Lane* c, size_t B) {
    c->h_gseed.ensure(B);
    c->h_gnonce.ensure(B);
    c->gseed.ensure(B);
    c->gstate.ensure(grind_state_words(B));
}
Digest* grind_seeds(Lane* c, size_t B) {
    size_grind(c, B);
    return c->h_gseed.p;
}
const u64* grind_search(Lane* c, int B, unsigned grind, u64 first, u64 max_nonce, unsigned chunk_log, unsigned blocks) {
    size_grind(c, B);
    const hipStream_t s = gather_stream(c);
    void* out = nullptr;
    HIPCHK(hipHostGetDevicePointer(&out, c->h_gnonce.p, 0));
    upload(c->gseed.p, c->h_gseed.p, (size_t)B * sizeof(Digest), s);
    launch_grind(c->gseed.p, c->gstate.p, (u64*)out, (unsigned)B, grind, first, max_nonce, chunk_log, blocks, s);
    HIPCHK(hipStreamSynchronize(s));
    return c->h_gnonce.p;
}

static void upload_unit_inputs(Lane* c, ProofJob* jobs, int B, const ProofShape& sh, const Opts& o) {
    hipStream_t s = c->stream;
    AirConst* airs = c->h_air.ensure(B);
    for (int b = 0; b < B; b++) airs[b] = jobs[b].air;
    upload(c->air.p, airs, B * sizeof(AirConst), s);
    DevCoin* hc = c->h_coin.ensure(B);
    for (int b = 0; b < B; b++) {
        ProofJob& j = jobs[b];
        u64 e[20];
        context_elements(sh.n, o, e);
        memcpy(e + 8, j.air.pub, 12 * 8);
        j.coin.init(e, 20);
        j.commitments.clear();
        hc[b].seed = j.coin.seed;
        hc[b].counter = j.coin.counter;
        hc[b].pad = 0;
    }
    upload(c->dcoin.p, hc, B * sizeof(DevCoin), s);
    HIPCHK(hipMemsetAsync(c->dfail.p, 0, B * sizeof(int), s));
}

ColConst trace_const(const Lane* c, const ProofShape& sh) {
    ColConst cc;
    cc.flags = c->const_col.p;
    cc.vals = c->coef.p;
    cc.val_stride = sh.n;
    return cc;
}

void launch_trace_lde(Lane* c, const Tables& T, int B, const ProofShape& sh, bool probe) {
    hipStream_t s = c->stream;
    const unsigned char* skip = c->const_col.p;
    if (c->poison_lde) HIPCHK(hipMemsetAsync(c->lde.p, 0xFF, (size_t)B * 7 * sh.N * 8, s));
    launch_const_detect(c->trace.p, B * 7, sh.logn, c->const_col.p, s);
    launch_interpolate(c->trace.p, sh.n, c->coef.p, sh.n, c->scratch.p, B * 7, sh.logn, false, sh.n, T, s, skip);
    if (probe) {
        if (!c->lde_ev[0]) {
            HIPCHK(hipEventCreate(&c->lde_ev[0]));
            HIPCHK(hipEventCreate(&c->lde_ev[1]));
        }
        HIPCHK(hipEventRecord(c->lde_ev[0], s));
    }
    launch_lde(c->coef.p, sh.n, c->lde.p, c->scratch.p, B * 7, sh.logn, sh.logbeta, T, s, skip);
    if (probe) HIPCHK(hipEventRecord(c->lde_ev[1], s));
    launch_const_fill(skip, c->trace.p, sh.n, c->coef.p, nullptr, B * 7, sh.logn, sh.logbeta, s);
}

static void enqueue_fri_layers(Lane* c, const Tables& T, int B, const ProofShape& sh, int fold, CoinStep& cs,
                               HostTrace& ht) {
    hipStream_t s = c->stream;
    const int DE = sh.DE;
    const unsigned nl = sh.nl;
    for (unsigned l = 0; l < nl; l++) {
        const u64 rows = sh.D[l] / fold;
        const bool cm = (l == 0);
        const u64* src = cm ? c->f0.p : c->flayer[l].p;
        const u64 cstride = cm ? sh.N : sh.D[l], sstride = DE * cstride;
        cs.kind = CoinStep::FRI_ALPHA;
        cs.out = c->alpha7.p;
        cs.hist = c->falpha.p + (size_t)l * B * DE;
        cs.root_out = c->droots.p + (size_t)(2 + l) * B;
        launch_merkle_fri(src, sstride, cstride, cm, sh.logn, sh.logbeta, rows, c->fnodes[l].p, B, DE, fold, s, cs);
        launch_fri_fold(src, sstride, cstride, cm, sh.logn, sh.logbeta, rows, (int)ilog2(sh.D[l]), c->alpha7.p,
                        c->flayer[l + 1].p, rows, T, B, DE, fold, s);
    }
    ht.mark("chain_launch");
    if (nl > 0) {
        launch_interpolate(c->flayer[nl].p, sh.D[nl], c->rem.p, sh.rem_len, c->scratch.p, B * DE,
                           (int)ilog2(sh.D[nl]), true, sh.rem_len, T, s);
    } else {
        HIPCHK(hipMemcpy2DAsync(c->rem.p, sh.rem_len * 8, c->deep.p, sh.n * 8, sh.rem_len * 8, (size_t)B * DE,
                                hipMemcpyDeviceToDevice, s));
    }
}

static ReplayView pack_replay_block(Lane* c, size_t B, const ProofShape& sh, bool with_keys) {
    const size_t DE = sh.DE, nl = sh.nl;
    PackSet pk;
    u64 words = 0;
    auto seg = [&](const void* src, size_t bytes) {
        const u64 at = words;
        pk.src[pk.nseg] = src;
        pk.off[pk.nseg] = at;
        pk.words[pk.nseg++] = bytes / 4;
        words = (at + bytes / 4 + 63) & ~63ULL;
        return at * 4;
    };
    const u64 o_roots = seg(c->droots.p, (2 + nl) * B * sizeof(Digest));
    const u64 o_ood = seg(c->ood.p, B * 15 * DE * 8);
    const u64 o_co = seg(c->coeffs.p, B * 15 * DE * 8);
    const u64 o_dp = seg(c->dp.p, B * sizeof(DeepParams));
    const u64 o_falpha = seg(c->falpha.p, nl * B * DE * 8);
    const u64 o_fail = seg(c->dfail.p, B * sizeof(int));
    const u64 o_rem = seg(c->rem.p, B * DE * sh.rem_len * 8);
    const u64 o_dn2 = seg(c->dn2.p, B * DE * 8);
    const u64 o_const = seg(c->const_col.p, (B * 7 + 3) & ~(size_t)3);
    const u64 o_keys = with_keys ? seg(c->tkeys.p, B * 8) : 0;
    unsigned char* hx = c->h_xfer.ensure(words * 4);
    void* hx_dev = nullptr;
    HIPCHK(hipHostGetDevicePointer(&hx_dev, hx, 0));
    launch_pack(pk, hx_dev, c->stream);
    ReplayView rv;
    rv.roots = (const Digest*)(hx + o_roots);
    rv.ood = (const u64*)(hx + o_ood);
    rv.co = (const u64*)(hx + o_co);
    rv.dps = (const DeepParams*)(hx + o_dp);
    rv.falpha = (const u64*)(hx + o_falpha);
    rv.ffail = (const int*)(hx + o_fail);
    rv.remh = (const u64*)(hx + o_rem);
    rv.dn2h = (const u64*)(hx + o_dn2);
    c->h_const_col = hx + o_const;
    c->h_tkeys = with_keys ? (const u64*)(hx + o_keys) : nullptr;
    return rv;
}

static ReplayView enqueue_commit_chain(Lane* c, const Tables& T, const u64* ce_div, ProofJob* jobs, int B,
                                       const TraceSrc& ts, const ProofShape& sh, const Opts& o, u64 g,
                                       HostTrace& ht) {
    const u64 n = sh.n;
    const int logn = sh.logn, logbeta = sh.logbeta, DE = sh.DE;
    hipStream_t s = c->stream;
    upload_unit_inputs(c, jobs, B, sh, o);
    ht.mark("setup");
    stage_mark(c, 0);
    const size_t tbytes = (size_t)7 * n * 8;
    switch (ts.kind) {
        case TraceSrc::GENERATED: launch_trace_gen(c->air.p, c->trace.p, logn, B, s); break;
        case TraceSrc::HOST_DIRECT:
            HIPCHK(hipMemcpyAsync(c->trace.p, ts.p, B * tbytes, hipMemcpyHostToDevice, s));
            break;
        case TraceSrc::HOST_STAGED: {
            u64* st = c->h_trace.p;
            const u64* src = ts.p;
            const int* refused = ts.refused;
            host_pool().parallel_for(B, [st, src, refused, n, tbytes](int b) {
                if (refused[b]) memset(st + (size_t)b * 7 * n, 0, tbytes);
                else memcpy(st + (size_t)b * 7 * n, src + (size_t)b * 7 * n, tbytes);
            });
            HIPCHK(hipMemcpyAsync(c->trace.p, st, B * tbytes, hipMemcpyHostToDevice, s));
            break;
        }
        case TraceSrc::DEVICE:
            HIPCHK(hipMemcpyAsync(c->trace.p, ts.p, B * tbytes, hipMemcpyDeviceToDevice, s));
            break;
    }
    if (ts.checks()) launch_trace_check(c->trace.p, c->air.p, c->tkeys.p, logn, B, ts.validate, s);
    launch_trace_lde(c, T, B, sh, c->lde_probe);
    stage_mark(c, 1);
    CoinStep cs;
    cs.ext = DE;
    cs.coins = c->dcoin.p;
    cs.fail = c->dfail.p;
    cs.kind = CoinStep::COEFFS;
    cs.out = c->coeffs.p;
    cs.root_out = c->droots.p;
    const ColConst cc = trace_const(c, sh);
    launch_merkle_lde(c->lde.p, 7, c->tnodes.p, B, logn, logbeta, s, cs, cc);
    stage_mark(c, 2);
    launch_constraint_eval(c->lde.p, c->air.p, c->coeffs.p, ce_div, c->ce.p, logn, logbeta, B, DE, s, cc);
    stage_mark(c, 3);
    launch_interpolate(c->ce.p, 2 * n, c->hcoef.p, n, c->scratch.p, B * DE, logn + 1, true, n, T, s);
    launch_lde(c->hcoef.p, n, c->hlde.p, c->scratch.p, B * DE, logn, logbeta, T, s);
    stage_mark(c, 4);
    cs.kind = CoinStep::OOD_POINT;
    cs.out = c->zpts.p;
    cs.root_out = c->droots.p + B;
    cs.g = g;
    launch_merkle_lde(c->hlde.p, DE, c->hnodes.p, B, logn, logbeta, s, cs);
    stage_mark(c, 5);
    DeepCoinStep dc;
    dc.coins = c->dcoin.p;
    dc.fail = c->dfail.p;
    dc.zpts = c->zpts.p;
    dc.dp = c->dp.p;
    dc.ginv = gl_inv(g);
    launch_ood(c->coef.p, c->hcoef.p, c->zpts.p, c->partial.p, c->ood.p, logn, B, DE, s, dc);
    stage_mark(c, 6);
    launch_deep(c->coef.p, c->hcoef.p, c->dp.p, c->partial.p, c->carry.p, c->deep.p, logn, B, DE, s);
    launch_lde(c->deep.p, n, c->f0.p, c->scratch.p, B * DE, logn, logbeta, T, s);
    HIPCHK(hipMemcpy2DAsync(c->dn2.p, 8, c->deep.p + (n - 2), n * 8, 8, (size_t)B * DE, hipMemcpyDeviceToDevice, s));
    stage_mark(c, 7);
    enqueue_fri_layers(c, T, B, sh, (int)o.fold, cs, ht);
    const ReplayView rv = pack_replay_block(c, B, sh, ts.checks());
    stage_mark(c, 8);
    ht.mark("launch_rem");
    return rv;
}

struct Gathered {
    const u64* gv;
    const Digest* gd;
};
static Gathered enqueue_gathers(Lane* c, const ProofShape& sh, const OpeningIndex& ix, HostTrace& ht) {
    const size_t nvals = ix.nvals, ndig = ix.ndig, nent = ix.nent, nopen = nent * 2 * sh.beta;
    u64* hidx = c->h_idx.ensure(ix.allidx.size());
    memcpy(hidx, ix.allidx.data(), ix.allidx.size() * 8);
    u64* gv = c->h_gv.ensure(nvals);
    Digest* gd = c->h_gd.ensure(ndig + 2 * nopen);
    void *didx = nullptr, *dgv = nullptr, *dgd = nullptr;
    HIPCHK(hipHostGetDevicePointer(&didx, hidx, 0));
    HIPCHK(hipHostGetDevicePointer(&dgv, gv, 0));
    HIPCHK(hipHostGetDevicePointer(&dgd, gd, 0));
    const u64* gidx = (const u64*)didx;
    u64* gval = (u64*)dgv;
    Digest* gdig = (Digest*)dgd;
    ht.mark("q_idx_host");
    const hipStream_t sq = gather_stream(c);
    ht.mark("q_h2d");
    GatherSet gs;
    size_t vo = 0, dof = 0, gbase = 0;
    auto add = [&](const void* src, void* dst, bool dig, size_t cnt) {
        if (gs.nseg == GatherSet::MAX) {
            launch_gather_set(gs, gidx + gbase, sq);
            gbase += gs.first[gs.nseg];
            gs = GatherSet{};
        }
        gs.src[gs.nseg] = src;
        gs.dst[gs.nseg] = dst;
        gs.digest[gs.nseg] = dig ? 1 : 0;
        gs.first[gs.nseg + 1] = gs.first[gs.nseg] + cnt;
        gs.nseg++;
    };
    const u64* vsrc[2] = {c->lde.p, c->hlde.p};
    const ColConst cc = trace_const(c, sh);
    gs.cc_seg = 0;
    gs.cc_shift = sh.logn + sh.logbeta;
    gs.cc = cc;
    for (size_t k = 0; k < ix.vseg.size(); k++) {
        const u64* src = k < 2 ? vsrc[k] : (k == 2 ? c->f0.p : c->flayer[k - 2].p);
        add(src, gval + vo, false, ix.vseg[k].second);
        vo += ix.vseg[k].second;
    }
    for (size_t k = 0; k < ix.dseg.size(); k++) {
        const Digest* src = k == 0 ? c->tnodes.p : (k == 1 ? c->hnodes.p : c->fnodes[k - 2].p);
        add(src, gdig + dof, true, ix.dseg[k].second);
        dof += ix.dseg[k].second;
    }
    launch_gather_set(gs, gidx + gbase, sq);
    const u64* ent = gidx + nvals + ndig;
    launch_open_rows(c->lde.p, 7, ent, nent, gdig + ndig, sh.logn, sh.logbeta, sq, cc);
    launch_open_rows(c->hlde.p, sh.DE, ent, nent, gdig + ndig + nopen, sh.logn, sh.logbeta, sq);
    ht.mark("q_launch");
    stage_mark(c, 9, sq);
    return Gathered{gv, gd};
}

void prove_lane(Lane* c, const Tables& T, const u64* ce_div, ProofJob* jobs, int B, const TraceSrc& ts,
                       u64 n, const Opts& o) {
    using clk = std::chrono::steady_clock;
    const auto t_host0 = clk::now();
    HostTrace ht;
    ht.mark("start");
    const ProofShape sh(n, o);
    const u64 g = gl_root(sh.logn);
    HostPool& pool = host_pool();

    size_lane_buffers(c, B, sh, o, ts);
    const ReplayView rv = enqueue_commit_chain(c, T, ce_div, jobs, B, ts, sh, o, g, ht);
    HIPCHK(hipStreamSynchronize(c->stream));
    ht.mark("sync_rem");
    u64 live_cols = 0;
    for (int k = 0; k < B * 7; k++) live_cols += c->h_const_col[k] ? 0 : 1;
    pool.parallel_for(B, [jobs, B, &sh, g, &rv](int b) { replay_transcript(jobs[b], b, B, sh, g, rv); });

    const auto t_q0 = clk::now();
    std::vector<LaneLayout>& lay = c->hs.lay;
    if (lay.size() < (size_t)B) lay.resize(B);
    if (o.grind < GRIND_DEVICE_MIN) {
        pool.parallel_for(B, [jobs, &sh, &o, &rv, &lay](int b) { plan_queries(jobs[b], b, sh, o, rv, lay[b]); });
        c->grind_host += (u64)B;
    } else {
        pool.parallel_for(B, [jobs, &sh, &rv, &lay](int b) { plan_commit_remainder(jobs[b], b, sh, rv, lay[b]); });
        Digest* seeds = grind_seeds(c, B);
        for (int b = 0; b < B; b++) seeds[b] = jobs[b].coin.seed;
        const GrindPlan gp = grind_plan((unsigned)o.grind, (uint32_t)B, (unsigned)c->cus);
        const u64* nonces = grind_search(c, B, (unsigned)o.grind, 1, gp.max_nonce, gp.chunk_log, gp.blocks);
        ht.mark("grind");
        for (int b = 0; b < B; b++) {
            if (nonces[b] == 0) {
                jobs[b].status = XFG_PROVER_ERROR;
                jobs[b].pow_exhausted = true;
            } else if (nonces[b] > gp.max_nonce || pow_zeros(jobs[b].coin.seed, nonces[b]) < o.grind) {
                throw std::runtime_error("device / host transcript diverged");
            }
        }
        pool.parallel_for(B, [jobs, &sh, &o, nonces, &lay](int b) { plan_openings(jobs[b], b, sh, o, nonces[b], lay[b]); });
        c->grind_dev += (u64)B;
    }
    ht.mark("queries_plan");
    OpeningIndex& ix = c->hs.ix;
    concat_indices(lay, B, sh, ix);
    const Gathered got = enqueue_gathers(c, sh, ix, ht);
    const auto t_q1 = clk::now();
    ht.mark("queries_host");
    HIPCHK(hipStreamSynchronize(c->gstream));
    ht.mark("sync_gather");
    const auto t_s0 = clk::now();

    pool.parallel_for(B, [jobs, B, &sh, &o, &lay, &ix, got](int b) {
        serialize_proof(jobs[b], b, B, sh, o, lay[b], ix, got.gv, got.gd);
    });
    ht.mark("serialize");
    for (int b = 0; b < B && ts.kind != TraceSrc::GENERATED; b++) {
        const u64 key = c->h_tkeys ? c->h_tkeys[b] : TRACE_KEY_VALID;
        const bool refused = ts.refused && ts.refused[b];
        if (ts.keys && !refused) ts.keys[b] = key;
        if (refused) jobs[b].status = ts.refused[b];
        else if (key != TRACE_KEY_VALID)
            jobs[b].status = (key >> 62) == TRACE_KEY_NONCANONICAL ? XFG_INVALID_ARGUMENT : XFG_INVALID_TRACE;
    }
    ht.dump(B, (long)((u64)B * 7 - live_cols));
    if (c->lde_probe) {
        float ms = 0;
        HIPCHK(hipEventSynchronize(c->lde_ev[1]));
        HIPCHK(hipEventElapsedTime(&ms, c->lde_ev[0], c->lde_ev[1]));
        c->lde_ms += ms;
        c->lde_sets++;
        c->lde_polys += live_cols;
    }
    if (c->timing) {
        for (int k = 0; k < 9; k++) {
            float ms = 0;
            HIPCHK(hipEventElapsedTime(&ms, c->ev[k], c->ev[k + 1]));
            c->stage_ms[k] = ms;
        }
        const auto t_end = clk::now();
        c->stage_ms[ST_HOST] = std::chrono::duration<double, std::milli>(t_end - t_host0).count();
        c->stage_ms[ST_HQUERY] = std::chrono::duration<double, std::milli>(t_q1 - t_q0).count();
        c->stage_ms[ST_HSER] = std::chrono::duration<double, std::milli>(t_end - t_s0).count();
    }
}

static void create_lane_stream(xfg_ctx* c, Lane* L) {
    L->lde_probe = c->lde_probe;
    L->poison_lde = c->poison_lde;
    HIPCHK(hipDeviceGetAttribute(&L->cus, hipDeviceAttributeMultiprocessorCount, c->device));
    HIPCHK(hipStreamCreateWithFlags(&L->stream, hipStreamNonBlocking));
    for (auto& e : L->ev) HIPCHK(hipEventCreate(&e));
}
Lane* lane0(xfg_ctx* c) {
    if (c->lanes.empty()) {
        c->lanes.emplace_back(new Lane());
        create_lane_stream(c, c->lanes[0].get());
    }
    return c->lanes[0].get();
}
void ensure_lanes(xfg_ctx* c, size_t k) {
    lane0(c);
    while (c->lanes.size() < k) {
        c->lanes.emplace_back(new Lane());
        create_lane_stream(c, c->lanes.back().get());
    }
    for (auto& L : c->lanes) gather_stream(L.get());
}

}
```

xfg-stark_amd/csrc/merkle.hip:

```cpp
#include "dev_coin.hpp"
#include <algorithm>
#include <stdexcept>
#include <type_traits>

namespace xfg {

#define XFG_CHECK_LAUNCH() (void)hipGetLastError()

constexpr u64 ROW2_MIN_N = 1024, ROW2_MAX_BLOCKS = 1024;
constexpr int LEAF_LANES_LOG = 1;
constexpr int UP_WMIN = 64;
constexpr int TREE_MID_WMIN = 64, TREE_MID_SHRINK = 8;
constexpr u64 MID4_MAX_BLOCKS = 256;
constexpr u64 TREE_TOP_MAX = 512;

__device__ __forceinline__ void lds_level(Digest& d, bool have, int slot, Digest* lds, int half, Digest* dst) {
    const int t = threadIdx.x;
    if (have) lds[slot] = d;
    __syncthreads();
    if (t < half) {
        d = b3_merge(lds[2 * t], lds[2 * t + 1]);
        dst[t] = d;
    }
}
__device__ __forceinline__ void block_tree_up(Digest d, Digest* nodes, u64 count, Digest* lds, int wmin) {
    u64 c = count;
    for (int w = blockDim.x; w > wmin; w >>= 1) {
        c >>= 1;
        lds_level(d, true, threadIdx.x, lds, w / 2, nodes + c + (u64)blockIdx.x * (w / 2));
        __syncthreads();
    }
}
__device__ __forceinline__ void quad_level(const Digest* src, bool act, int i, int q, Digest* lds, Digest* dst) {
    uint2 o = make_uint2(0, 0);
    if (act) {
        uint32_t m[16];
#pragma unroll
        for (int w = 0; w < 8; w++) {
            m[w] = src[2 * i].w[w];
            m[8 + w] = src[2 * i + 1].w[w];
        }
        o = b3_merge_quad(m, q);
    }
    __syncthreads();
    if (act) {
        lds[i].w[q] = o.x;
        lds[i].w[4 + q] = o.y;
        dst[i].w[q] = o.x;
        dst[i].w[4 + q] = o.y;
    }
    __syncthreads();
}

struct NoConst {};
template <bool CC>
using RowConstOf = std::conditional_t<CC, RowConst, NoConst>;
template <int NC, int LOGB, bool CC>
__device__ __forceinline__ void lde_row(const u64* base, u64 n, u64 m, int t, const RowConstOf<CC>& rc, u64 (&row)[NC]) {
    static_assert(!CC || NC == 7, "constant columns are those of the trace");
#pragma unroll
    for (int c = 0; c < NC; c++) {
        if constexpr (CC) {
            if ((rc.mask >> c) & 1) {
                row[c] = rc.v[c];
                continue;
            }
        }
        row[c] = base[((u64)c * (1 << LOGB) + t) * n + m];
    }
}

template <int NC, int LOGB, int LOG, int T0, bool CC>
__device__ __forceinline__ Digest lde_subtree(const u64* base, u64 n, u64 m, const RowConstOf<CC>& rc) {
    if constexpr (LOG == 0) {
        u64 row[NC];
        lde_row<NC, LOGB, CC>(base, n, m, T0, rc, row);
        return b3_hash_elems<NC>(row);
    } else {
        Digest l = lde_subtree<NC, LOGB, LOG - 1, T0, CC>(base, n, m, rc);
        Digest r = lde_subtree<NC, LOGB, LOG - 1, T0 + (1 << (LOG - 1)), CC>(base, n, m, rc);
        return b3_merge(l, r);
    }
}

template <int NC, int LOGB, int LOG, bool CC>
__device__ __forceinline__ Digest lde_subtree_wide(const u64* base, u64 n, u64 m, int t0, const RowConstOf<CC>& rc) {
    if constexpr (LOG <= 4) {
        return lde_subtree<NC, LOGB, LOG, 0, CC>(base + (u64)t0 * n, n, m, rc);
    } else {
        Digest l, d;
#pragma unroll 1
        for (int i = 0; i < 2; i++) {
            d = lde_subtree_wide<NC, LOGB, LOG - 1, CC>(base, n, m, t0 + (i << (LOG - 1)), rc);
            if (i == 0) l = d;
        }
        return b3_merge(l, d);
    }
}

template <bool CC>
__device__ __forceinline__ RowConstOf<CC> block_row_const(const ColConst& cc, int proof) {
    if constexpr (CC) return row_const_uniform(cc, (u64)proof);
    else return NoConst{};
}

template <int NC, int LOGB, bool CC>
__global__ __launch_bounds__(256) void leaves_row_kernel(const u64* lde, Digest* nodes_all,
                                                         u64 node_stride, int logn, ColConst cc) {
    __shared__ Digest lds[256];
    const u64 n = 1ULL << logn;
    const int proof = blockIdx.y;
    const u64 m = (u64)blockIdx.x * blockDim.x + threadIdx.x;
    const u64* base = lde + (u64)proof * NC * (1 << LOGB) * n;
    const RowConstOf<CC> rc = block_row_const<CC>(cc, proof);
    Digest d = lde_subtree_wide<NC, LOGB, LOGB, CC>(base, n, m, 0, rc);
    block_tree_up(d, nodes_all + (u64)proof * node_stride, n, lds, blockDim.x / 4);
}

template <int LOGB>
constexpr int leaf_lanes_log() { return LOGB < LEAF_LANES_LOG ? LOGB : LEAF_LANES_LOG; }
template <int NC, int LOGB, bool CC>
__global__ __launch_bounds__(256) void leaves_row2_kernel(const u64* lde, Digest* nodes_all,
                                                          u64 node_stride, int logn, ColConst cc) {
    constexpr int LOGL = leaf_lanes_log<LOGB>(), RB = 256 >> LOGL;
    __shared__ Digest lds[RB];
    const u64 n = 1ULL << logn;
    const int proof = blockIdx.y, t = threadIdx.x, h = t & ((1 << LOGL) - 1), rl = t >> LOGL;
    const u64 m = (u64)blockIdx.x * RB + rl;
    const u64* base = lde + (u64)proof * NC * (1 << LOGB) * n + (u64)h * (1 << (LOGB - LOGL)) * n;
    const RowConstOf<CC> rc = block_row_const<CC>(cc, proof);
    Digest d = lde_subtree_wide<NC, LOGB, LOGB - LOGL, CC>(base, n, m, 0, rc);
#pragma unroll
    for (int k = 0; k < LOGL; k++) {
        Digest r;
#pragma unroll
        for (int w = 0; w < 8; w++) r.w[w] = __shfl_xor(d.w[w], 1 << k);
        d = (h >> k) & 1 ? b3_merge(r, d) : b3_merge(d, r);
    }
    Digest* nodes = nodes_all + (u64)proof * node_stride;
    lds_level(d, h == 0, rl, lds, RB / 2, nodes + n / 2 + (u64)blockIdx.x * (RB / 2));
    __syncthreads();
    lds_level(d, t < RB / 2, t, lds, RB / 4, nodes + n / 4 + (u64)blockIdx.x * (RB / 4));
}

template <int LOGB>
constexpr int open_lanes_log() { return LOGB < 6 ? LOGB : 6; }
template <int NC, int LOGB, bool CC>
__global__ __launch_bounds__(64) void open_rows_kernel(const u64* lde, const u64* entries, u64 count, Digest* out,
                                                       int logn, ColConst cc) {
    constexpr int LOGL = open_lanes_log<LOGB>(), LPL = LOGB - LOGL;
    static_assert(LPL <= 1, "at most two leaves per lane");
    const u64 g = (u64)blockIdx.x * blockDim.x + threadIdx.x;
    const u64 e = g >> LOGL;
    const int t = (int)(g & ((1 << LOGL) - 1)) << LPL;
    if (e >= count) return;
    const u64 n = 1ULL << logn, ent = entries[e];
    const u64 proof = ent >> logn, m = ent & (n - 1);
    const u64* base = lde + proof * NC * (1 << LOGB) * n;
    Digest* local = out + e * (2 << LOGB);
    RowConstOf<CC> rc;
    if constexpr (CC) rc = row_const_lane(cc, proof);
    u64 row[NC];
    lde_row<NC, LOGB, CC>(base, n, m, t, rc, row);
    Digest d = b3_hash_elems<NC>(row);
    local[(1 << LOGB) + t] = d;
    if constexpr (LPL == 1) {
        lde_row<NC, LOGB, CC>(base, n, m, t + 1, rc, row);
        const Digest d1 = b3_hash_elems<NC>(row);
        local[(1 << LOGB) + t + 1] = d1;
        d = b3_merge(d, d1);
        local[((1 << LOGB) + t) >> 1] = d;
    }
#pragma unroll
    for (int k = LPL + 1; k <= LOGB; k++) {
        Digest r;
#pragma unroll
        for (int w = 0; w < 8; w++) r.w[w] = __shfl_xor(d.w[w], 1 << (k - 1 - LPL));
        d = b3_merge(d, r);
        if ((t & ((1 << k) - 1)) == 0) local[((1 << LOGB) + t) >> k] = d;
    }
}

template <int V>
using IntC = std::integral_constant<int, V>;
template <int NC, class F>
static bool with_logbeta(int logbeta, F f) {
    switch (logbeta) {
        case 1: f(IntC<NC>{}, IntC<1>{}); return true;
        case 2: f(IntC<NC>{}, IntC<2>{}); return true;
        case 3: f(IntC<NC>{}, IntC<3>{}); return true;
        case 4: f(IntC<NC>{}, IntC<4>{}); return true;
        case 5: f(IntC<NC>{}, IntC<5>{}); return true;
        case 6: f(IntC<NC>{}, IntC<6>{}); return true;
        case 7: f(IntC<NC>{}, IntC<7>{}); return true;
        default: return false;
    }
}
template <class F>
static void with_nc_logbeta(int nc, int logbeta, F f) {
    const bool found = nc == 7   ? with_logbeta<7>(logbeta, f)
                       : nc == 2 ? with_logbeta<2>(logbeta, f)
                       : nc == 1 ? with_logbeta<1>(logbeta, f)
                                 : false;
    if (!found) throw std::invalid_argument("Merkle kernels: no instantiation for this column count and blowup");
}

static void require_trace_width(int nc, const ColConst& cc) {
    if (cc.flags && nc != 7) throw std::invalid_argument("Merkle kernels: constant columns are those of a 7-column trace LDE");
}
template <class F>
static void with_const_logbeta(int logbeta, F f) {
    if (!with_logbeta<7>(logbeta, f))
        throw std::invalid_argument("Merkle kernels: no instantiation for this column count and blowup");
}

void launch_open_rows(const u64* lde, int nc, const u64* entries, u64 count, Digest* out, int logn, int logbeta,
                      hipStream_t s, const ColConst& cc) {
    if (!count) return;
    require_trace_width(nc, cc);
    const int logl = logbeta < 6 ? logbeta : 6;
    dim3 g((unsigned)(((count << logl) + 63) / 64)), b(64);
    if (cc.flags)
        with_const_logbeta(logbeta, [&](auto NC, auto LB) {
            hipLaunchKernelGGL((open_rows_kernel<decltype(NC)::value, decltype(LB)::value, true>), g, b, 0, s, lde, entries, count, out, logn, cc);
        });
    else
        with_nc_logbeta(nc, logbeta, [&](auto NC, auto LB) {
            hipLaunchKernelGGL((open_rows_kernel<decltype(NC)::value, decltype(LB)::value, false>), g, b, 0, s, lde, entries, count, out, logn, cc);
        });
    XFG_CHECK_LAUNCH();
}

__device__ void coin_root_step(const CoinStep& cs, int b, const Digest& root) {
    const int D = cs.ext, lane = threadIdx.x;
    DevCoin c = cs.coins[b];
    dev_reseed(c, root);
    bool ok;
    if (cs.kind == CoinStep::COEFFS) {
        ok = wave_draw_e(c, 15, D, cs.out + (u64)b * 15 * D, D);
    } else {
        u64 a[2] = {0, 0};
        ok = dev_draw_e(c, a, D);
        if (cs.kind == CoinStep::OOD_POINT) {
            if (a[0] == 0 && a[1] == 0) ok = false;
            if (lane == 0)
                for (int k = 0; k < D; k++) {
                    cs.out[(u64)b * 2 * D + k] = a[k];
                    cs.out[(u64)b * 2 * D + D + k] = gl_mul(a[k], cs.g);
                }
        } else if (lane == 0) {
            const u64 inv7 = 0x249249246DB6DB6EULL;
            for (int k = 0; k < D; k++) cs.out[(u64)b * D + k] = gl_mul(a[k], inv7);
            if (cs.hist)
                for (int k = 0; k < D; k++) cs.hist[(u64)b * D + k] = a[k];
        }
    }
    if (lane == 0) {
        if (!ok) cs.fail[b] = 1;
        cs.coins[b] = c;
        if (cs.root_out) cs.root_out[b] = root;
    }
}

__global__ __launch_bounds__(1024) void tree_top_kernel(Digest* nodes_all, u64 node_stride, u64 count, CoinStep cs) {
    __shared__ Digest lds[256];
    Digest* nodes = nodes_all + (u64)blockIdx.x * node_stride;
    const int tid = threadIdx.x, i = tid >> 2, q = tid & 3;
    for (u64 c = count; c > 1; c >>= 1) {
        const u64 half = c >> 1;
        quad_level(c == count ? nodes + c : lds, i < (int)half, i, q, lds, nodes + half);
    }
    if (cs.kind != CoinStep::NONE && tid < 64) coin_root_step(cs, blockIdx.x, count > 1 ? lds[0] : nodes[1]);
}
__global__ __launch_bounds__(256) void tree_mid_kernel(Digest* nodes_all, u64 node_stride, u64 count) {
    __shared__ Digest lds[256];
    Digest* nodes = nodes_all + (u64)blockIdx.y * node_stride;
    const u64 i = (u64)blockIdx.x * 256 + threadIdx.x;
    const Digest d = b3_merge(nodes[count + 2 * i], nodes[count + 2 * i + 1]);
    nodes[count / 2 + i] = d;
    block_tree_up(d, nodes, count / 2, lds, TREE_MID_WMIN);
}
__global__ __launch_bounds__(256) void tree_mid4_kernel(Digest* nodes_all, u64 node_stride, u64 count) {
    __shared__ Digest lds[64];
    Digest* nodes = nodes_all + (u64)blockIdx.y * node_stride;
    const int tid = threadIdx.x, i = tid >> 2, q = tid & 3;
    u64 c = count, first = (u64)blockIdx.x * 64;
    for (int w = 64; w >= 16; w >>= 1, c >>= 1, first >>= 1)
        quad_level(w == 64 ? nodes + c + 2 * first : lds, i < w, i, q, lds, nodes + c / 2 + first);
}
static void finish_tree(Digest* nodes, u64 node_stride, u64 count, int npoly, hipStream_t s, const CoinStep& cs) {
    while (count > TREE_TOP_MAX) {
        if ((count / 512) * (u64)npoly < MID4_MAX_BLOCKS)
            hipLaunchKernelGGL(tree_mid4_kernel, dim3((unsigned)(count / 128), npoly), dim3(256), 0, s, nodes,
                               node_stride, count);
        else
            hipLaunchKernelGGL(tree_mid_kernel, dim3((unsigned)(count / 512), npoly), dim3(256), 0, s, nodes,
                               node_stride, count);
        count /= TREE_MID_SHRINK;
    }
    if (count > 1 || cs.kind != CoinStep::NONE) {
        int threads = (int)(2 * count);
        threads = threads < 64 ? 64 : threads;
        hipLaunchKernelGGL(tree_top_kernel, dim3(npoly), dim3(threads), 0, s, nodes, node_stride, count, cs);
    }
    XFG_CHECK_LAUNCH();
}

void launch_merkle_lde(const u64* lde, int nc, Digest* nodes, int npoly, int logn, int logbeta, hipStream_t s,
                       const CoinStep& cs, const ColConst& cc) {
    const u64 n = 1ULL << logn, node_stride = 2 * n;
    require_trace_width(nc, cc);
    if (n >= ROW2_MIN_N && (u64)npoly * (n / 256) < ROW2_MAX_BLOCKS) {
        const int logl = logbeta < LEAF_LANES_LOG ? logbeta : LEAF_LANES_LOG;
        dim3 g((unsigned)(n >> (8 - logl)), npoly), b(256);
// ... 75 lines not shown
```

xfg-stark_amd/csrc/ntt.hip:

```cpp
#include <algorithm>
#include <atomic>
#include <cstdlib>
#include <string>
#include <type_traits>
#include <utility>
#include "hip_util.hpp"
#include "kernels.hpp"
#include "field_dft.hpp"
#include "ntt_plan.hpp"

namespace xfg {

typedef u32 u32x2 __attribute__((__vector_size__(8)));
__device__ __forceinline__ __amdgpu_buffer_rsrc_t buf_rsrc(const u64* p) {
    const u64 a = (u64)p;
    const u64 u = (u64)(u32)__builtin_amdgcn_readfirstlane((int)(u32)a) |
                  ((u64)(u32)__builtin_amdgcn_readfirstlane((int)(u32)(a >> 32)) << 32);
    return __builtin_amdgcn_make_buffer_rsrc(reinterpret_cast<void*>(u), (short)0, -1, 0x00020000);
}
__device__ __forceinline__ u64 buf_ld(__amdgpu_buffer_rsrc_t r, u32 voff, u32 soff) {
    const u32x2 v = __builtin_amdgcn_raw_buffer_load_b64(r, (int)voff, (int)soff, 0);
    return (u64)v[0] | ((u64)v[1] << 32);
}
__device__ __forceinline__ void buf_st(__amdgpu_buffer_rsrc_t r, u32 voff, u32 soff, u64 x) {
// ... 603 lines not shown
    constexpr int R1 = 1 << PLB::FIRST_LOGR, G1 = C / R1;
    static_assert(PLB::NSTEP > 1 && (1 << LOGE) == R1, "one full-radix first-step group per thread");
    constexpr int logTR = LOGT + LOGE - LOGC, TR = 1 << logTR;
    extern __shared__ u64 lds[];
    u64* tile = lds;
    u64* ltw = lds + lds_pass_b(LOGC, LOGT, LOGE, LOGT + LOGE - LOGC).tw;
    {
        const u64* pt4 = a.pt + a.tab().wC();
        for (int i = threadIdx.x; i < C; i += NT) ltw[i] = pt4[i];
    }
    __syncthreads();
    const u64 n = 1ULL << a.logn;
    const int per_x = gridDim.x >> 3, x = blockIdx.x & 7, slot = blockIdx.x >> 3;
    const int span = (ntiles + 7) >> 3, tend = min((x + 1) * span, ntiles);
    const int seq0 = threadIdx.x / G1, j0 = threadIdx.x % G1;
    auto load = [&](int ti, u64* dst) -> bool {
        const int pt = ti / ntx, k10 = (ti - pt * ntx) * TR;
        if (a.skipped(pt >> a.logbeta)) return true;
        const u64* y = a.y + (u64)pt * n + ((u64)(k10 + seq0) << LOGC) + j0;
#pragma unroll
        for (int r = 0; r < R1; r++) dst[r] = y[r * G1];
        return false;
    };
    int ti = x * span + slot;
    u64 yv[R1] = {};
    bool skip_cur = ti < tend && load(ti, yv);
    for (; ti < tend; ti += per_x) {
        const int pt = ti / ntx, k10 = (ti - pt * ntx) * TR;
        u64 nx[R1] = {};
        const bool skip_nx = ti + per_x < tend && load(ti + per_x, nx);
        if (skip_cur) {
#pragma unroll
            for (int r = 0; r < R1; r++) yv[r] = nx[r];
            skip_cur = skip_nx;
            continue;
        }
        auto ldg = [&](int, int, int o) -> u64 { return yv[o / G1]; };
        u64* out = a.plane_out(pt) + k10;
        auto stg = [&](int, int seq, int base, int stride, u64* v) {
            u64 o[RR];
#pragma unroll
            for (int r = 0; r < RR; r++) o[r] = canon(v[r]);
            store_pairs<RR>(o, [&](int r) { return out + (seq & ~1) + ((u64)(base + r * stride) << a.logR); });
        };
        pass_dft<LOGC, LOGE, false, false, NT>(tile, logTR, ltw, ldg, stg, [](int, int, int, int) {});
#pragma unroll
        for (int r = 0; r < R1; r++) yv[r] = nx[r];
        skip_cur = skip_nx;
    }
}

__global__ void fourstep_kernel(u64* out, int logn, int logbeta, int logC, u64 scale, Tables T) {
    const u64 i = (u64)blockIdx.x * blockDim.x + threadIdx.x;
    const u64 n = 1ULL << logn;
    if (logbeta < 0) {
        if (i >= n) return;
        const u64 k1 = i >> logC, j2 = i & ((1ULL << logC) - 1);
        out[i] = gl_mul(tw_get(T, logn, (j2 * k1) & (n - 1), true), scale);
    } else {
        const int logN = logn + logbeta;
        if (i >= (1ULL << logN)) return;
        const u64 t = i >> logn, k1 = (i & (n - 1)) >> logC, j2 = i & ((1ULL << logC) - 1);
        out[i] = gl_mul(T.pow7[j2], tw_get(T, logN, (j2 * (t + (k1 << logbeta))) & ((1ULL << logN) - 1), false));
    }
}
__global__ void pass_tables_kernel(u64* out, PassTableLayout L, Tables T) {
    const u64 i = (u64)blockIdx.x * blockDim.x + threadIdx.x;
    const int logR = L.logR, logC = L.logC, logbeta = L.logbeta;
    const u64 R = L.R(), C = L.C(), Z = 0;
    if (i >= L.total()) return;
    if (i < L.wC()) {
        out[i] = tw_get(T, logR, i, !L.fwd());
    } else if (i < L.pre(Z)) {
        out[i] = tw_get(T, logC, i - L.wC(), !L.fwd());
    } else if (i < L.comb(Z)) {
        const u64 t = (i - L.pre(Z)) >> logR, j = (i - L.pre(Z)) & (R - 1);
        out[i] = gl_mul(T.pow7[j << logC], tw_get(T, logR + logbeta, (t * j) & ((1ULL << (logR + logbeta)) - 1), false));
    } else if (L.has_r1024() && i < L.r1024_seed(Z)) {
        const u64 q = i - L.comb(Z);
        const u64 t = q >> 10, r = (q >> 5) & 31, k = q & 31;
        const u64 g = gl_mul(T.pow7[r << logC], tw_get(T, logR + logbeta, (t * r) & ((1ULL << (logR + logbeta)) - 1), false));
        out[i] = gl_mul(tw_get(T, logR, r * k, false), g);
    } else if (L.has_r1024()) {
        const int logn = logR + logC, logN = logn + logbeta;
        const u64 j2 = i & (C - 1);
        if (i < L.r1024_t4()) {
            const u64 t = (i - L.r1024_seed(Z)) >> logC;
            out[i] = gl_mul(T.pow7[j2], tw_get(T, logN, (j2 * t) & ((1ULL << logN) - 1), false));
        } else {
            const u64 k1 = (i - L.r1024_t4()) >> logC;
            out[i] = tw_get(T, logn, (j2 * k1) & ((1ULL << logn) - 1), false);
        }
    } else if (i < L.cos2_scal()) {
        const u64 q = i - L.comb(Z);
        const u64 t = q >> 8, r = (q >> 4) & 15, k = q & 15;
        const u64 grp = gl_mul(T.pow7[r << logC], tw_get(T, logR + logbeta, (t * r) & ((1ULL << (logR + logbeta)) - 1), false));
        out[i] = gl_mul(tw_get(T, logR, r * k, false), grp);
    } else {
        const u64 q = i - L.cos2_scal();
        const u64 c = q >> 4, r = q & 15;
        out[i] = gl_mul(T.pow7[(16 * r) << logC], tw_get(T, 4 + logbeta, (c * r) & ((1ULL << (4 + logbeta)) - 1), false));
    }
}
void build_pass_tables(u64* out, int logn, int logbeta, const Tables& T, hipStream_t s) {
    const PassTableLayout L = pass_table_layout(logn, logbeta);
    hipLaunchKernelGGL(pass_tables_kernel, dim3((unsigned)((L.total() + 255) / 256)), dim3(256), 0, s, out, L, T);
}
void build_fourstep(u64* out, int logn, int logbeta, const Tables& T, hipStream_t s) {
    const u64 cnt = fourstep_main(logn, logbeta);
    hipLaunchKernelGGL(fourstep_kernel, dim3((unsigned)((cnt + 255) / 256)), dim3(256), 0, s, out, logn, logbeta,
                       pass_table_layout(logn, logbeta).logC, gl_inv(1ULL << logn), T);
    build_pass_tables(out + cnt, logn, logbeta, T, s);
}

struct NttEntry {
    NttKey key;
    const void* fn;
    std::atomic<bool> big_lds;
};
#define XFG_NTT_ENTRY(K, SYM, S, INV, T, E) {{NttKernel::K, S, T, E, INV}, (const void*)SYM},
static NttEntry ntt_entries[] = {XFG_NTT_KERNELS(XFG_NTT_ENTRY)};
#undef XFG_NTT_ENTRY

static void ntt_launch(const NttPass& p, void** args, hipStream_t s) {
    for (NttEntry& e : ntt_entries) {
        if (!(e.key == p.key)) continue;
        if (p.lds > 65536 && !e.big_lds.load(std::memory_order_acquire)) {
            HIPCHK(hipFuncSetAttribute(e.fn, hipFuncAttributeMaxDynamicSharedMemorySize, 160 * 1024));
            e.big_lds.store(true, std::memory_order_release);
        }
        HIPCHK(hipLaunchKernel(e.fn, dim3(p.gx, p.gy), dim3(p.block), args, p.lds, s));
        return;
    }
    throw std::runtime_error("NTT: planned kernel is not in the kernel list");
}

static void ntt_run(NttArgs& a, int npoly, bool inv, hipStream_t s) {
    static const int cus = [] {
        int dev = 0, n = 256;
        if (hipGetDevice(&dev) == hipSuccess) (void)hipDeviceGetAttribute(&n, hipDeviceAttributeMultiprocessorCount, dev);
        return n;
    }();
    NttPlan p = ntt_plan(a.logn, a.logbeta, inv, npoly, a.t4 != nullptr, a.pt != nullptr, cus);
    if (!p.ok)
        throw std::runtime_error((inv ? "inverse NTT of size 2^" : "forward NTT of size 2^") + std::to_string(a.logn) +
                                 " has no kernel");
    a.logR = p.logR, a.logC = p.logC;
    a.xcd = p.xcd, a.tq_b = p.tq_b, a.preg = p.preg;
    void* args[] = {&a, &p.ntx, &p.ntiles};
    ntt_launch(p.a, args, s);
    ntt_launch(p.b, args, s);
}

__global__ void const_flags_init_kernel(unsigned char* flags, int count) {
    const int i = blockIdx.x * blockDim.x + threadIdx.x;
    if (i < count) flags[i] = 1;
}
__global__ __launch_bounds__(256) void const_detect_kernel(const u64* cols, u64 n, unsigned char* flags) {
    const int col = blockIdx.y;
    const u64* c = cols + (u64)col * n;
    const u64 first = c[0];
    const u64 i0 = (u64)blockIdx.x * CONST_DETECT_SPAN, i1 = i0 + CONST_DETECT_SPAN < n ? i0 + CONST_DETECT_SPAN : n;
    u64 diff = 0;
    for (u64 i = i0 + threadIdx.x; i < i1; i += blockDim.x) diff |= c[i] ^ first;
    if (diff) flags[col] = 0;
}
void launch_const_detect(const u64* cols, int ncols, int logn, unsigned char* flags, hipStream_t s) {
    const u64 n = 1ULL << logn;
    hipLaunchKernelGGL(const_flags_init_kernel, dim3((unsigned)((ncols + 255) / 256)), dim3(256), 0, s, flags, ncols);
    hipLaunchKernelGGL(const_detect_kernel, dim3((unsigned)((n + CONST_DETECT_SPAN - 1) / CONST_DETECT_SPAN), ncols),
                       dim3((unsigned)std::min<u64>(256, n)), 0, s, cols, n, flags);
}
__global__ __launch_bounds__(256) void const_fill_kernel(const unsigned char* flags, const u64* src, u64 src_stride,
                                                         u64* coef, u64* lde, u64 n, int logbeta) {
    const int col = blockIdx.y;
    if (!flags[col]) return;
    const u64 v = src[(u64)col * src_stride];
    const u64 i0 = (u64)blockIdx.x * CONST_FILL_SPAN;
    if (lde) {
        const u64 N = n << logbeta, i1 = i0 + CONST_FILL_SPAN < N ? i0 + CONST_FILL_SPAN : N;
        u64* o = lde + (u64)col * N;
        const u64x2 d = {v, v};
        for (u64 i = i0 + 2 * threadIdx.x; i < i1; i += 2 * blockDim.x) *reinterpret_cast<u64x2*>(o + i) = d;
    }
    if (coef) {
        const u64 span = lde ? (u64)CONST_FILL_SPAN >> logbeta : (u64)CONST_FILL_SPAN;
        const u64 c0 = (u64)blockIdx.x * span, c1 = c0 + span < n ? c0 + span : n;
        u64* o = coef + (u64)col * n;
        for (u64 i = c0 + 2 * threadIdx.x; i < c1; i += 2 * blockDim.x) {
            const u64x2 d = {i == 0 ? v : 0, 0};
            *reinterpret_cast<u64x2*>(o + i) = d;
        }
    }
}
void launch_const_fill(const unsigned char* flags, const u64* src, u64 src_stride, u64* coef, u64* lde, int ncols,
                       int logn, int logbeta, hipStream_t s) {
    if (!coef && !lde) return;
    const u64 n = 1ULL << logn, span = lde ? n << logbeta : n;
    hipLaunchKernelGGL(const_fill_kernel, dim3((unsigned)((span + CONST_FILL_SPAN - 1) / CONST_FILL_SPAN), ncols),
                       dim3(256), 0, s, flags, src, src_stride, coef, lde, n, lde ? logbeta : 0);
}

__global__ __launch_bounds__(256) void lde_twist_kernel(const u64* coef, u64 coef_stride, u64* tw, int logn, int logN,
                                                        const unsigned char* skip, Tables T) {
    const u64 n = 1ULL << logn, j = (u64)blockIdx.x * blockDim.x + threadIdx.x;
    const u64 poly = blockIdx.y, u = blockIdx.z + 1;
    if (j >= n || (skip && skip[poly])) return;
    tw[((u - 1) * gridDim.y + poly) * n + j] = gl_mul(coef[poly * coef_stride + j], tw_get(T, logN, u * j, false));
}

void launch_lde(const u64* coef, u64 coef_stride, u64* out, u64* scratch, int npoly, int logn, int logbeta,
                const Tables& T, hipStream_t s, const unsigned char* skip) {
    const LdePlan lp = lde_plan(logn, logbeta, npoly);
    if (!lp.ok) throw std::runtime_error("forward LDE of 2^" + std::to_string(logn) + " x 2^" + std::to_string(logbeta) + " has no kernel");
    const u64 n = 1ULL << logn;
    const int lb = lp.sub_logbeta;
    u64* twisted = scratch + lp.twist_off;
    if (lp.groups > 1) {
        if (T.LM < logn + logbeta) throw std::runtime_error("forward LDE: the root-of-unity table is smaller than the LDE domain");
        hipLaunchKernelGGL(lde_twist_kernel, dim3((unsigned)((n + 255) / 256), (unsigned)npoly, (unsigned)(lp.groups - 1)), dim3(256),
                           0, s, coef, coef_stride, twisted, logn, logn + logbeta, skip, T);
    }
    const TableKind k = T.fs ? table_kind(logn, lb) : TableKind::none;
    for (int u = 0; u < lp.groups; u++) {
        NttArgs a{u ? twisted + (u64)(u - 1) * npoly * n : coef, scratch, out + (u64)u * n, u ? n : coef_stride, n << logbeta, logn};
        a.out_plane = lp.out_plane;
        a.logbeta = lb;
        a.skip = skip;
        a.T = T;
        a.t4 = k == TableKind::fourstep ? T.fs->fwd[logn][lb] : nullptr;
        a.pt = a.t4 ? a.t4 + fourstep_main(logn, lb) : (k == TableKind::pass_only ? T.fs->pass_fwd[logn][lb] : nullptr);
        ntt_run(a, npoly, false, s);
    }
}

void launch_interpolate(const u64* evals, u64 in_stride, u64* out, u64 out_stride, u64* scratch, int npoly, int logn,
                        bool off7, u64 keep, const Tables& T, hipStream_t s, const unsigned char* skip) {
    NttArgs a{evals, scratch, out, in_stride, out_stride, logn};
    a.skip = skip;
    a.off7 = off7 ? 1 : 0;
    a.keep = keep;
    a.T = T;
    a.scale = gl_inv(1ULL << logn);
    a.t4 = (T.fs && logn <= FOURSTEP_MAX_LOG) ? T.fs->inv[logn] : nullptr;
    a.pt = a.t4 ? a.t4 + fourstep_main(logn, -1) : nullptr;
    ntt_run(a, npoly, true, s);
}

}
```

xfg-stark_amd/csrc/prover_internal.hpp:

```cpp
#pragma once
#include <algorithm>
#include <atomic>
#include <chrono>
#include <cstdlib>
#include <map>
#include <memory>
#include <string>
#include <thread>
#include <vector>

#include "../../include/xfg_stark.h"
#include "grind_plan.hpp"
#include "hip_util.hpp"
#include "host_common.hpp"
#include "kernels.hpp"
#include "proof_assembly.hpp"
#include "unit_queue.hpp"
#include "verifier.hpp"

namespace xfg {

struct TablesHost {
    int LM = -1;
    DBuf<u64> tw, pow7, ipow7;
    std::map<int, DBuf<u64>> ce_div;
    FourStep fs;
    std::map<int, DBuf<u64>> four_buf;
    std::map<int, DBuf<u64>> pass_buf;
};

enum {
    ST_LDE, ST_TCOMMIT, ST_CE, ST_COMP, ST_CCOMMIT, ST_OOD, ST_DEEP, ST_FRI, ST_GATHER, ST_HOST, ST_HQUERY, ST_HSER,
    ST_COUNT
};

struct Lane {
    hipStream_t stream = nullptr;
    hipStream_t gstream = nullptr;
    bool timing = false;
    double stage_ms[ST_COUNT] = {0};
    hipEvent_t ev[ST_COUNT + 1] = {};
    bool lde_probe = false;
    hipEvent_t lde_ev[2] = {};
    double lde_ms = 0;
    u64 lde_sets = 0, lde_polys = 0;
    bool poison_lde = false;
    DBuf<AirConst> air;
    DBuf<u64> coeffs, trace, coef, scratch, lde, ce, hcoef, hlde, zpts, partial, ood, carry, deep, f0, alpha7,
        rem, dn2, falpha;
    DBuf<Digest> tnodes, hnodes, droots;
    DBuf<DeepParams> dp;
    DBuf<DevCoin> dcoin;
    DBuf<int> dfail;
    DBuf<unsigned char> const_col;
    const unsigned char* h_const_col = nullptr;
    DBuf<u64> tkeys;
    const u64* h_tkeys = nullptr;
    HBuf<u64> h_trace;
    std::vector<DBuf<u64>> flayer;
    std::vector<DBuf<Digest>> fnodes;
    MappedHBuf<Digest> h_gd;
    MappedHBuf<u64> h_idx, h_gv;
    MappedHBuf<unsigned char> h_xfer;
    MappedHBuf<AirConst> h_air;
    MappedHBuf<DevCoin> h_coin;
    MappedHBuf<Digest> h_gseed;
    MappedHBuf<u64> h_gnonce;
    DBuf<Digest> gseed;
    DBuf<u64> gstate;
    int cus = 0;
    std::atomic<uint64_t> grind_dev{0}, grind_host{0};
    struct {
        OpeningIndex ix;
        std::vector<LaneLayout> lay;
    } hs;
    Lane() = default;
    Lane(const Lane&) = delete;
    Lane& operator=(const Lane&) = delete;
    ~Lane() {
        if (stream) (void)hipStreamSynchronize(stream);
        if (gstream) (void)hipStreamSynchronize(gstream);
        for (auto& e : ev)
            if (e) (void)hipEventDestroy(e);
        for (auto& e : lde_ev)
            if (e) (void)hipEventDestroy(e);
        if (stream) (void)hipStreamDestroy(stream);
        if (gstream) (void)hipStreamDestroy(gstream);
    }
};

struct TraceSrc {
    enum Kind { GENERATED, HOST_DIRECT, HOST_STAGED, DEVICE };
    Kind kind = GENERATED;
    const u64* p = nullptr;
    bool validate = false;
    bool size_staging = false;
    const int* refused = nullptr;
    u64* keys = nullptr;
    bool checks() const { return validate || kind == DEVICE; }
};

struct Batch {
    std::vector<ProofJob> jobs;
    std::vector<uint32_t> which;
    std::vector<uint8_t*> outs;
    size_t* out_lens = nullptr;
    int* statuses = nullptr;
    std::vector<int> st;
    TraceSrc trace;
    std::vector<int> refused;
    std::vector<u64> keys;
    xfg_trace_fault* faults = nullptr;
    u64 n = 0;
    Opts o{};
    Tables T{};
    const u64* ce_div = nullptr;
    int units_left = 0;
    std::exception_ptr err;
};

struct HostTrace {
    std::vector<std::pair<const char*, std::chrono::steady_clock::time_point>> m;
    std::map<std::string, double> acc;
    using clk = std::chrono::steady_clock;
    clk::time_point t_ = {};
    void tic() {
        if (trace_on()) t_ = clk::now();
    }
    void toc(const char* what) {
        if (!trace_on()) return;
        auto t = clk::now();
        acc[what] += std::chrono::duration<double, std::milli>(t - t_).count();
        t_ = t;
    }
    void mark(const char* what) {
        if (trace_on()) m.push_back({what, std::chrono::steady_clock::now()});
    }
    void dump(int B, long const_cols = -1) {
        if (!trace_on() || m.size() < 2) return;
        std::string line = "[xfg] B=" + std::to_string(B);
        if (const_cols >= 0) line += " const_cols=" + std::to_string(const_cols);
        for (size_t i = 1; i < m.size(); i++) {
            char buf[96];
            snprintf(buf, sizeof buf, " %s=%.2f", m[i].first,
                     std::chrono::duration<double, std::milli>(m[i].second - m[i - 1].second).count());
            line += buf;
        }
        for (auto& kv : acc) {
            char buf[96];
            snprintf(buf, sizeof buf, " [%s=%.3f]", kv.first.c_str(), kv.second);
            line += buf;
        }
        fprintf(stderr, "%s\n", line.c_str());
    }
};

}

struct xfg_ctx {
    int device = 0;
    std::string err;
    bool lde_probe = false;
    bool poison_lde = false;
    bool stage_traces = false;
    xfg::TablesHost tables;
    std::vector<std::unique_ptr<xfg::Lane>> lanes;
    xfg::UnitQueue<xfg::Batch> queue;
    std::vector<std::thread> workers;
    struct {
        xfg::HBuf<uint8_t> stage;
        xfg::DBuf<uint8_t> dstage;
        xfg::DBuf<xfg::u64> flags;
        std::vector<xfg::VState> st;
        std::vector<xfg::VerifyPlan> frag;
    } vb;
};

namespace xfg {

void ensure_tables(xfg_ctx* c, int LM);
const u64* ensure_ce_table(xfg_ctx* c, int logn);
bool fourstep_ready(xfg_ctx* c, int logn, int logbeta);
void ensure_fourstep(xfg_ctx* c, int logn, int logbeta);
Tables tables_of(xfg_ctx* c);
Lane* lane0(xfg_ctx* c);
void ensure_lanes(xfg_ctx* c, size_t k);
void prove_lane(Lane* c, const Tables& T, const u64* ce_div, ProofJob* jobs, int B, const TraceSrc& ts, u64 n,
                const Opts& o);
void size_trace_lde(Lane* c, size_t B, const ProofShape& sh);
void size_constraint_eval(Lane* c, size_t B, const ProofShape& sh);
void size_ood_deep(Lane* c, size_t B, const ProofShape& sh);
void launch_trace_lde(Lane* c, const Tables& T, int B, const ProofShape& sh, bool probe);
ColConst trace_const(const Lane* c, const ProofShape& sh);
void size_grind(Lane* c, size_t B);
Digest* grind_seeds(Lane* c, size_t B);
const u64* grind_search(Lane* c, int B, unsigned grind, u64 first, u64 max_nonce, unsigned chunk_log, unsigned blocks);

static inline bool all_canonical(const uint64_t* v, size_t k) {
    for (size_t i = 0; i < k; i++)
        if (v[i] >= P) return false;
    return true;
}
static inline bool air_canonical(const xfg_air_consts* a) {
    return all_canonical(a->pub_inputs, 12) && a->nullifier < P && a->commitment < P;
}

template <class F>
static int guarded(xfg_ctx* c, F f) {
    try {
        return f();
    } catch (const HipError& e) {
        c->err = e.what();
        return XFG_DEVICE_ERROR;
    } catch (const std::exception& e) {
        c->err = std::string("Prover error: ") + e.what();
        return XFG_PROVER_ERROR;
    }
}

template <class F>
static int on_lane0(xfg_ctx* c, F f) {
    if (c->queue.busy()) {
        c->err = "batches pending: call xfg_batch_wait first";
        return XFG_INVALID_ARGUMENT;
    }
    return guarded(c, [&]() -> int {
        Lane* L = lane0(c);
        L->timing = c->queue.whole_units();
        HIPCHK(hipSetDevice(c->device));
        return f(L);
    });
}

static int env_int(const char* name, int dflt) {
    const char* v = getenv(name);
    return v && *v ? atoi(v) : dflt;
}
static int max_lanes() {
    static const int v = std::max(1, env_int("XFG_LANES", 7));
    return v;
}
static int unit_size() {
    static const int v = std::max(1, env_int("XFG_UNIT", 32));
    return v;
}
static int unit_size(u64 beta) { return beta > 16 ? std::max(1, (int)(unit_size() * 16 / beta)) : unit_size(); }

static int split_min() {
    static const int v = std::max(0, env_int("XFG_SPLIT_MIN", 16));
    return v;
}

}
```

xfg-stark_amd/xfgstark/__init__.py:

```python
import ctypes as C
import mmap
import os
import sys

_HERE = os.path.dirname(os.path.abspath(__file__))
_PKG = os.path.dirname(_HERE)
LIB_PATH = os.environ.get("XFG_LIB") or os.path.join(_PKG, "libxfgstark.so")
HEADER_PATH = os.path.join(os.path.dirname(_PKG), "include", "xfg_stark.h")

if not os.path.exists(LIB_PATH):
    raise ImportError(f"libxfgstark.so not built at {LIB_PATH}: run `make -C xfg-stark_amd` "
                      "(or __graft_entry__.build()); the prover has no CPU fallback")

_lib = C.CDLL(LIB_PATH)

STATUS = {0: "OK", 1: "INVALID_BURN_AMOUNT", 2: "MINT_MISMATCH", 3: "ZERO_TX_HASH", 4: "BAD_RECIPIENT_LEN",
          5: "SHORT_SECRET", 6: "PROVER_ERROR", 7: "DEVICE_ERROR", 8: "BUFFER_TOO_SMALL", 9: "INVALID_ARGUMENT",
          10: "VERIFY_FAILED", 11: "INVALID_TRACE"}
TRACE_VALIDATE, TRACE_ON_DEVICE = 1, 2


class _Options(C.Structure):
    _fields_ = [("num_queries", C.c_uint32), ("blowup_factor", C.c_uint32), ("grinding_factor", C.c_uint32),
                ("field_extension", C.c_uint32), ("fri_folding_factor", C.c_uint32),
                ("fri_remainder_max_degree", C.c_uint32)]


class _BurnInputs(C.Structure):
    _fields_ = [("burn_amount", C.c_uint64), ("mint_amount", C.c_uint64), ("tx_prefix_hash", C.c_uint8 * 32),
                ("recipient_address", C.c_char_p), ("recipient_len", C.c_size_t), ("secret", C.c_char_p),
                ("secret_len", C.c_size_t), ("network_id", C.c_uint32), ("target_chain_id", C.c_uint32),
                ("commitment_version", C.c_uint32)]


class _AirConsts(C.Structure):
    _fields_ = [("pub_inputs", C.c_uint64 * 12), ("nullifier", C.c_uint64), ("commitment", C.c_uint64)]


class _ProofInfo(C.Structure):
    _fields_ = [("trace_width", C.c_uint32), ("trace_length", C.c_uint64), ("options", _Options),
                ("num_unique_queries", C.c_uint32), ("num_fri_layers", C.c_uint32), ("remainder_len", C.c_uint32),
                ("pow_nonce", C.c_uint64), ("trace_root", C.c_uint8 * 32), ("constraint_root", C.c_uint8 * 32),
                ("ood_trace", C.c_uint64 * 14), ("ood_composition", C.c_uint64), ("size", C.c_size_t)]


class _TraceFault(C.Structure):
    _fields_ = [("kind", C.c_uint32), ("index", C.c_uint32), ("column", C.c_uint32), ("step", C.c_uint64),
                ("expected", C.c_uint64), ("found", C.c_uint64)]


_u64p = C.POINTER(C.c_uint64)
_u8p = C.POINTER(C.c_uint8)
_lib.xfg_ctx_create.restype = C.c_void_p
_lib.xfg_ctx_create.argtypes = [C.c_int]
_lib.xfg_ctx_destroy.argtypes = [C.c_void_p]
_lib.xfg_default_options.argtypes = [C.POINTER(_Options)]
_lib.xfg_last_error.argtypes = [C.c_void_p, C.c_char_p, C.c_size_t]
_lib.xfg_proof_size_bound.restype = C.c_size_t
_lib.xfg_proof_size_bound.argtypes = [C.c_uint64, C.POINTER(_Options)]
_lib.xfg_prove_burn_mint.argtypes = [C.c_void_p, C.POINTER(_BurnInputs), C.c_uint64, C.POINTER(_Options), _u8p,
                                     C.POINTER(C.c_size_t)]
_lib.xfg_prove_trace.argtypes = [C.c_void_p, _u64p, C.c_uint32, C.c_uint64, C.POINTER(_AirConsts),
                                 C.POINTER(_Options), _u8p, C.POINTER(C.c_size_t)]
_lib.xfg_prove_batch.argtypes = [C.c_void_p, C.c_uint32, C.POINTER(_BurnInputs), C.c_uint64, C.POINTER(_Options),
                                 C.POINTER(_u8p), C.POINTER(C.c_size_t), C.POINTER(C.c_int)]
_lib.xfg_prove_batch_submit.argtypes = [C.c_void_p, C.c_uint32, C.POINTER(_BurnInputs), C.c_uint64,
                                         C.POINTER(_Options), C.POINTER(_u8p), C.POINTER(C.c_size_t),
                                         C.POINTER(C.c_int), C.POINTER(C.c_uint64)]
_lib.xfg_batch_wait.argtypes = [C.c_void_p, C.c_uint64]
_lib.xfg_proof_parse.argtypes = [_u8p, C.c_size_t, C.POINTER(_ProofInfo), C.c_char_p, C.c_size_t]
_lib.xfg_verify.argtypes = [_u8p, C.c_size_t, C.POINTER(_AirConsts), C.POINTER(_Options), C.c_char_p, C.c_size_t]
_lib.xfg_verify_batch.argtypes = [C.c_uint32, C.POINTER(_u8p), C.POINTER(C.c_size_t), C.POINTER(_AirConsts),
                                  C.POINTER(_Options), C.POINTER(C.c_int), C.c_uint32]
_lib.xfg_verify_batch_gpu.argtypes = [C.c_void_p, C.c_uint32, C.POINTER(_u8p), C.POINTER(C.c_size_t),
                                      C.POINTER(_AirConsts), C.POINTER(_Options), C.POINTER(C.c_int)]
if hasattr(_lib, "xfg_debug_verify_batch_gpu"):
    _lib.xfg_debug_verify_batch_gpu.argtypes = [C.c_void_p, C.c_uint32, C.POINTER(_u8p), C.POINTER(C.c_size_t),
                                                C.POINTER(_AirConsts), C.POINTER(_Options), C.POINTER(C.c_int),
                                                _u64p, C.c_char_p, C.c_size_t]
_lib.xfg_selftest_blake3.argtypes = [_u8p, C.c_size_t, _u8p]
_lib.xfg_prepare.argtypes = [C.c_void_p, C.c_uint32, C.c_uint64, C.POINTER(_Options)]
_lib.xfg_burn_air_consts.argtypes = [C.POINTER(_BurnInputs), C.POINTER(_AirConsts)]
_lib.xfg_set_timing.argtypes = [C.c_void_p, C.c_int]
_lib.xfg_stage_times.argtypes = [C.c_void_p, C.POINTER(C.c_double), C.POINTER(C.c_char_p), C.c_int]
_lib.xfg_bench_lde.argtypes = [C.c_void_p, C.c_uint32, C.c_uint64, C.c_uint32, C.c_uint32, C.POINTER(C.c_double)]
_lib.xfg_lde_probe.argtypes = [C.c_void_p, C.c_int, C.POINTER(C.c_double), C.POINTER(C.c_uint64),
                               C.POINTER(C.c_uint64)]
_lib.xfg_debug_lde.argtypes = [C.c_void_p, _u64p, C.c_uint32, C.c_uint64, C.c_uint32, _u64p]
_lib.xfg_debug_ood_deep.argtypes = [C.c_void_p, C.c_uint32, C.c_uint64, _u64p, _u64p, _u64p, _u64p, _u64p, _u64p]
if hasattr(_lib, "xfg_debug_ood_deep_e"):
    _lib.xfg_debug_ood_deep_e.argtypes = [C.c_void_p, C.c_uint32, C.c_uint64, C.c_uint32, _u64p, _u64p, _u64p, _u64p,
                                          C.POINTER(C.c_uint32), _u64p, C.c_uint64, _u64p, _u64p, _u64p,
                                          C.POINTER(C.c_uint32), _u64p, C.POINTER(C.c_int)]
_lib.xfg_debug_interpolate.argtypes = [C.c_void_p, _u64p, C.c_uint32, C.c_uint64, C.c_int, _u64p]
if hasattr(_lib, "xfg_debug_const_columns"):
    _lib.xfg_debug_const_columns.argtypes = [C.c_void_p, _u64p, C.c_uint32, C.c_uint32, C.c_uint64, _u8p]
    _lib.xfg_debug_lde_skip.argtypes = [C.c_void_p, _u64p, C.c_uint32, C.c_uint64, C.c_uint32, _u8p, _u64p]
    _lib.xfg_debug_interpolate_skip.argtypes = [C.c_void_p, _u64p, C.c_uint32, C.c_uint64, C.c_int, _u8p, _u64p]
if hasattr(_lib, "xfg_debug_constraint_eval"):
    _lib.xfg_debug_constraint_eval.argtypes = [C.c_void_p, C.c_uint32, C.c_uint64, C.c_uint32, C.c_uint32, _u64p,
                                               C.POINTER(_AirConsts), _u64p, _u64p]
    _lib.xfg_debug_fri_fold.argtypes = [C.c_void_p, C.c_uint32, C.c_uint32, C.c_uint32, C.c_uint32, C.c_int, _u64p,
                                        _u64p, _u64p]
if hasattr(_lib, "xfg_debug_field"):
    _lib.xfg_debug_field.argtypes = [C.c_void_p, C.c_uint32, C.c_uint64, _u64p, _u64p, _u64p]
if hasattr(_lib, "xfg_debug_coin_draws"):
    _lib.xfg_debug_coin_draws.argtypes = [C.c_void_p, C.POINTER(C.c_uint32), C.c_uint64, C.c_uint32, C.c_uint32,
                                          _u64p, _u64p, _u64p, _u64p, C.POINTER(C.c_int)]
if hasattr(_lib, "xfg_debug_merkle_lde"):
    _lib.xfg_debug_merkle_lde.argtypes = [C.c_void_p, C.c_uint32, C.c_uint32, C.c_uint64, C.c_uint32, _u64p, _u64p,
                                          C.c_uint64, _u8p, _u8p]
    _lib.xfg_debug_merkle_fri.argtypes = [C.c_void_p, C.c_uint32, C.c_uint32, C.c_uint32, C.c_uint32, C.c_int, _u64p,
                                          _u8p]
if hasattr(_lib, "xfg_debug_merkle_lde_const"):
    _lib.xfg_debug_merkle_lde_const.argtypes = [C.c_void_p, C.c_uint32, C.c_uint32, C.c_uint64, C.c_uint32, _u64p, _u8p,
                                                _u64p, _u64p, C.c_uint64, _u8p, _u8p]
    _lib.xfg_debug_poison_lde.argtypes = [C.c_void_p, C.c_int]
if hasattr(_lib, "xfg_debug_fri_fold_f"):
    _lib.xfg_debug_fri_fold_f.argtypes = [C.c_void_p, C.c_uint32, C.c_uint32, C.c_uint32, C.c_uint32, C.c_int,
                                          C.c_uint32, _u64p, _u64p, _u64p]
    _lib.xfg_debug_merkle_fri_f.argtypes = [C.c_void_p, C.c_uint32, C.c_uint32, C.c_uint32, C.c_uint32, C.c_int,
                                            C.c_uint32, _u64p, _u8p]
if hasattr(_lib, "xfg_debug_grind"):
    _lib.xfg_debug_grind.argtypes = [C.c_void_p, C.c_uint32, C.POINTER(C.c_uint32), C.c_uint32, C.c_uint64, C.c_uint64,
                                     C.c_uint32, C.c_uint32, _u64p]
    _lib.xfg_grind_probe.argtypes = [C.c_void_p, C.POINTER(C.c_uint32), _u64p, _u64p]
if hasattr(_lib, "xfg_prove_trace_batch"):
    _lib.xfg_check_traces.argtypes = [C.c_void_p, C.c_uint32, C.c_void_p, C.c_uint64, C.POINTER(_AirConsts),
                                      C.c_uint32, C.POINTER(_TraceFault)]
    _lib.xfg_prove_trace_batch.argtypes = [C.c_void_p, C.c_uint32, C.c_void_p, C.c_uint32, C.c_uint64,
                                           C.POINTER(_AirConsts), C.POINTER(_Options), C.c_uint32, C.POINTER(_u8p),
                                           C.POINTER(C.c_size_t), C.POINTER(C.c_int), C.POINTER(_TraceFault)]
    _lib.xfg_prove_trace_batch_submit.argtypes = _lib.xfg_prove_trace_batch.argtypes + [C.POINTER(C.c_uint64)]


class XfgStarkError(Exception):

    def __init__(self, status, message):
        super().__init__(message)
        self.status = status
        self.kind = STATUS.get(status, str(status))


class TraceFault:
    ASSERTION, TRANSITION, NONCANONICAL = 1, 2, 3

    def __init__(self, kind, index, column, step, expected, found):
        self.kind, self.index, self.column, self.step = kind, index, column, step
        self.expected, self.found = expected, found

    @classmethod
    def _from_c(cls, f):
        return cls(f.kind, f.index, f.column, f.step, f.expected, f.found) if f.kind else None

    def astuple(self):
        return (self.kind, self.index, self.column, self.step, self.expected, self.found)

    def __eq__(self, other):
        return isinstance(other, TraceFault) and other.astuple() == self.astuple()

    def __str__(self):
        if self.kind == self.ASSERTION:
            return f"trace does not satisfy assertion main_trace({self.column}, {self.step}) == {self.expected}"
        if self.kind == self.TRANSITION:
            return f"main transition constraint {self.index} did not evaluate to ZERO at step {self.step}"
        return "trace element is not a canonical field element"

    def __repr__(self):
        return "TraceFault(kind={}, index={}, column={}, step={}, expected={}, found={})".format(*self.astuple())


class FieldExtension:
    NONE = 1
    QUADRATIC = 2
    CUBIC = 3


class ProofOptions:

    def __init__(self, num_queries, blowup_factor, grinding_factor, field_extension, fri_folding_factor,
                 fri_remainder_max_degree):
        self.num_queries = num_queries
        self.blowup_factor = blowup_factor
        self.grinding_factor = grinding_factor
        self.field_extension = field_extension
        self.fri_folding_factor = fri_folding_factor
        self.fri_remainder_max_degree = fri_remainder_max_degree

    @classmethod
    def reference(cls):
        o = _Options()
        _lib.xfg_default_options(C.byref(o))
        return cls(o.num_queries, o.blowup_factor, o.grinding_factor, o.field_extension, o.fri_folding_factor,
                   o.fri_remainder_max_degree)

    def _c(self):
        return _Options(self.num_queries, self.blowup_factor, self.grinding_factor, self.field_extension,
                        self.fri_folding_factor, self.fri_remainder_max_degree)

    def __repr__(self):
        return ("ProofOptions(num_queries={0.num_queries}, blowup_factor={0.blowup_factor}, grinding_factor="
                "{0.grinding_factor}, field_extension={0.field_extension}, fri_folding_factor="
                "{0.fri_folding_factor}, fri_remainder_max_degree={0.fri_remainder_max_degree})").format(self)


def _bytes_ptr(b):
    return C.cast(C.c_char_p(b), _u8p)


class StarkProof:

    def __init__(self, data: bytes):
        self._data = bytes(data)
        self._info = None

    @classmethod
    def from_bytes(cls, data: bytes):
        p = cls(data)
        p._parse()
        return p

    def _parse(self):
        if self._info is None:
            info, err = _ProofInfo(), C.create_string_buffer(256)
            st = _lib.xfg_proof_parse(_bytes_ptr(self._data), len(self._data), C.byref(info), err, 256)
            if st:
                raise XfgStarkError(st, err.value.decode())
            self._info = info
        return self._info

    def to_bytes(self) -> bytes:
        return self._data

    @property
    def trace_length(self):
        return self._parse().trace_length

    @property
    def options(self):
        o = self._parse().options
        return ProofOptions(o.num_queries, o.blowup_factor, o.grinding_factor, o.field_extension,
                            o.fri_folding_factor, o.fri_remainder_max_degree)

    @property
    def num_unique_queries(self):
        return self._parse().num_unique_queries

    @property
    def num_fri_layers(self):
        return self._parse().num_fri_layers

    @property
    def remainder_len(self):
        return self._parse().remainder_len

    @property
    def pow_nonce(self):
        return self._parse().pow_nonce

    @property
    def trace_root(self):
        return bytes(self._parse().trace_root)

    @property
    def constraint_root(self):
        return bytes(self._parse().constraint_root)

    @property
    def ood_frame(self):
        i = self._parse()
# ... 349 lines not shown
        if k == 0 or cap == 0 or nbytes < 8 * k + cap * k:
            raise XfgStarkError(9, f"submit_batch_record: record of {nbytes} B for {k} proofs of bound {cap} B")
        arr = (_BurnInputs * k)()
        keep = []
        for i, kw in enumerate(inputs):
            s = burn_inputs(**kw)
            keep.append(s._keep)
            arr[i] = s
        base = addr + 8 * k
        outs = (_u8p * k)(*[C.cast(base + i * cap, _u8p) for i in range(k)])
        lens = (C.c_size_t * k).from_address(addr)
        for i in range(k):
            lens[i] = cap
        sts = (C.c_int * k)()
        ticket = C.c_uint64(0)
        st = _lib.xfg_prove_batch_submit(self._ctx, k, arr, trace_length, C.byref(o), outs, lens, sts,
                                         C.byref(ticket))
        if st:
            raise self._err(st)
        return PendingBatch(self, ticket.value, None, base, cap, outs, lens, sts, record=True, owner=owner)

    def _trace_args(self, traces, airs):
        import numpy as np
        if hasattr(traces, "data_ptr"):
            t = traces
            if t.device.type != "cuda" or (t.device.index or 0) != self._device:
                raise XfgStarkError(9, f"traces tensor is on {t.device}, the prover on device {self._device}")
            if str(t.dtype) not in ("torch.int64", "torch.uint64") or not t.is_contiguous():
                raise XfgStarkError(9, "traces tensor must be contiguous with dtype int64 or uint64")
            shape, keep, flags = tuple(t.shape), t, TRACE_ON_DEVICE
            if len(shape) == 3 and t.numel():
                import torch
                torch.cuda.current_stream(t.device).synchronize()
            ptr = t.data_ptr()
        else:
            a = np.ascontiguousarray(np.asarray(traces, dtype=np.uint64))
            shape, keep, flags, ptr = a.shape, a, 0, a.ctypes.data
        if len(shape) != 3:
            raise XfgStarkError(9, "traces: [count][7][n]")
        count, width, n = shape
        if len(airs) != count:
            raise XfgStarkError(9, f"{count} traces, {len(airs)} AIR constants")
        air_np = np.array([list(a[0]) + [a[1], a[2]] for a in airs], dtype=np.uint64).reshape(count, 14)
        return (keep, air_np), ptr or None, count, width, n, air_np.ctypes.data_as(C.POINTER(_AirConsts)), flags

    def submit_traces(self, traces, airs, validate=False):
        keep, ptr, count, width, n, air_p, flags = self._trace_args(traces, airs)
        o = self._options._c()
        cap = _lib.xfg_proof_size_bound(n, C.byref(o)) if count else 0
        buf = self._take_buffer(cap * count)
        base = C.addressof(buf)
        outs = (_u8p * count)(*[C.cast(base + i * cap, _u8p) for i in range(count)])
        lens = (C.c_size_t * count)(*([cap] * count))
        sts = (C.c_int * count)()
        faults = (_TraceFault * count)()
        ticket = C.c_uint64(0)
        st = _lib.xfg_prove_trace_batch_submit(self._ctx, count, ptr, width, n, air_p, C.byref(o),
                                               flags | (TRACE_VALIDATE if validate else 0), outs, lens, sts, faults,
                                               C.byref(ticket))
        if st:
            self._free.append(buf)
            raise self._err(st)
        return PendingBatch(self, ticket.value, buf, base, cap, outs, lens, sts, owner=keep, faults=faults)

    def prove_traces(self, traces, airs, validate=False):
        return self.submit_traces(traces, airs, validate).result()

    def check_traces(self, traces, airs):
        keep, ptr, count, width, n, air_p, flags = self._trace_args(traces, airs)
        if width != 7:
            raise XfgStarkError(9, "XfgBurnMintAir traces have 7 columns")
        faults = (_TraceFault * max(count, 1))()
        st = _lib.xfg_check_traces(self._ctx, count, ptr, n, air_p, flags, faults)
        if st:
            raise self._err(st)
        return [TraceFault._from_c(faults[i]) for i in range(count)]

    def _take_buffer(self, size):
        free = self.__dict__.setdefault("_free", [])
        for i, b in enumerate(free):
            if C.sizeof(b) >= size:
                return free.pop(i)
        size = max(size, 1)
        return (C.c_char * size).from_buffer(_anon_map(size))

    def prepare(self, count, trace_length=64, buffers=0):
        o = self._options._c()
        st = _lib.xfg_prepare(self._ctx, count, trace_length, C.byref(o))
        if st:
            raise self._err(st)
        if buffers:
            size = _lib.xfg_proof_size_bound(trace_length, C.byref(o)) * count
            free = self.__dict__.setdefault("_free", [])
            have = sum(1 for b in free if C.sizeof(b) >= size)
            for _ in range(max(0, buffers - have)):
                b = (C.c_char * size).from_buffer(_anon_map(size))
                C.memset(b, 0, size)
                free.append(b)

    def set_timing(self, on=True):
        _lib.xfg_set_timing(self._ctx, 1 if on else 0)

    def stage_times(self):
        ms = (C.c_double * 16)()
        names = (C.c_char_p * 16)()
        k = _lib.xfg_stage_times(self._ctx, ms, names, 16)
        return {names[i].decode(): ms[i] for i in range(k)}

    def bench_lde(self, count, n, blowup, iters):
        avg = C.c_double()
        st = _lib.xfg_bench_lde(self._ctx, count, n, blowup, iters, C.byref(avg))
        if st:
            raise self._err(st)
        return avg.value

    def lde_probe(self, enabled):
        ms, sets, polys = C.c_double(), C.c_uint64(), C.c_uint64()
        st = _lib.xfg_lde_probe(self._ctx, 1 if enabled else 0, C.byref(ms), C.byref(sets), C.byref(polys))
        if st:
            raise self._err(st)
        return ms.value, sets.value, polys.value

    def debug_lde(self, coef, n, blowup):
        import numpy as np
        c = np.ascontiguousarray(np.asarray(coef, dtype=np.uint64)).reshape(-1, n)
        out = np.zeros((c.shape[0], n * blowup), dtype=np.uint64)
        st = _lib.xfg_debug_lde(self._ctx, c.ctypes.data_as(_u64p), c.shape[0], n, blowup, out.ctypes.data_as(_u64p))
        if st:
            raise self._err(st)
        return out

    def debug_lde_skip(self, coef, n, blowup, skip):
        import numpy as np
        c = np.ascontiguousarray(np.asarray(coef, dtype=np.uint64)).reshape(-1, n)
        f = np.ascontiguousarray(np.asarray(skip, dtype=np.uint8))
        if f.shape != (c.shape[0],):
            raise XfgStarkError(9, "debug_lde_skip: one flag per polynomial")
        out = np.zeros((c.shape[0], n * blowup), dtype=np.uint64)
        st = _lib.xfg_debug_lde_skip(self._ctx, c.ctypes.data_as(_u64p), c.shape[0], n, blowup, f.ctypes.data_as(_u8p),
                                     out.ctypes.data_as(_u64p))
        if st:
            raise self._err(st)
        return out

    def debug_const_columns(self, trace):
        import numpy as np
        tr = np.ascontiguousarray(trace, dtype=np.uint64)
        B, width, n = tr.shape
        out = np.zeros((B, width), dtype=np.uint8)
        st = _lib.xfg_debug_const_columns(self._ctx, tr.ctypes.data_as(_u64p), B, width, n, out.ctypes.data_as(_u8p))
        if st:
            raise self._err(st)
        return out

    def debug_ood_deep(self, coef, hcoef, zpts, coeffs):
        import numpy as np
        c = np.ascontiguousarray(coef, dtype=np.uint64)
        B, _, n = c.shape
        hc = np.ascontiguousarray(hcoef, dtype=np.uint64)
        zp = np.ascontiguousarray(zpts, dtype=np.uint64)
        co = np.ascontiguousarray(coeffs, dtype=np.uint64)
        ood = np.zeros((B, 15), dtype=np.uint64)
        deep = np.zeros((B, n), dtype=np.uint64)
        p = lambda a: a.ctypes.data_as(_u64p)
        st = _lib.xfg_debug_ood_deep(self._ctx, B, n, p(c), p(hc), p(zp), p(co), p(ood), p(deep))
        if st:
            raise self._err(st)
        return ood, deep

    def debug_ood_deep_e(self, coef, hcoef, zpts, coeffs=None, coins=None, ginv=0):
        import numpy as np
        c = np.ascontiguousarray(coef, dtype=np.uint64)
        hc = np.ascontiguousarray(hcoef, dtype=np.uint64)
        zp = np.ascontiguousarray(zpts, dtype=np.uint64)
        B, _, n = c.shape
        ext = hc.shape[1]
        if c.shape[1] != 7 or hc.shape != (B, ext, n) or zp.shape != (B, 2, ext):
            raise XfgStarkError(9, "debug_ood_deep_e: coef [B,7,n], hcoef [B,ext,n], zpts [B,2,ext]")
        ood = np.zeros((B, 15, ext), dtype=np.uint64)
        deep = np.zeros((B, ext, n), dtype=np.uint64)
        p = lambda a: a.ctypes.data_as(_u64p)
        if coins is None:
            co = np.ascontiguousarray(coeffs, dtype=np.uint64)
            if co.shape != (B, 8, ext):
                raise XfgStarkError(9, "debug_ood_deep_e: coeffs [B,8,ext]")
            st = _lib.xfg_debug_ood_deep_e(self._ctx, B, n, ext, p(c), p(hc), p(zp), p(co), None, None, 0, p(ood),
                                           p(deep), None, None, None, None)
            if st:
                raise self._err(st)
            return ood, deep
        if len(coins) != B or any(len(bytes(sd)) != 32 for sd, _ in coins):
            raise XfgStarkError(9, "debug_ood_deep_e: coins are B x (32-byte seed, counter)")
        u32p = C.POINTER(C.c_uint32)
        seeds = np.frombuffer(b"".join(bytes(sd) for sd, _ in coins), dtype="<u4").copy()
        ctrs = np.array([ctr for _, ctr in coins], dtype=np.uint64)
        dp = np.zeros((B, 14, 2), dtype=np.uint64)
        seeds_out = np.zeros(B * 8, dtype="<u4")
        ctrs_out = np.zeros(B, dtype=np.uint64)
        fail = (C.c_int * max(B, 1))()
        st = _lib.xfg_debug_ood_deep_e(self._ctx, B, n, ext, p(c), p(hc), p(zp), None, seeds.ctypes.data_as(u32p),
                                       p(ctrs), ginv, p(ood), p(deep), p(dp), seeds_out.ctypes.data_as(u32p),
                                       p(ctrs_out), fail)
        if st:
            raise self._err(st)
        after = [(seeds_out[8 * b:8 * b + 8].tobytes(), int(ctrs_out[b])) for b in range(B)]
        return ood, deep, dp, after, [fail[b] for b in range(B)]

    def debug_constraint_eval(self, trace, airs, coeffs, blowup):
        import numpy as np
        tr = np.ascontiguousarray(trace, dtype=np.uint64)
        co = np.ascontiguousarray(coeffs, dtype=np.uint64)
        B, width, n = tr.shape
        if width != 7 or co.ndim != 3 or co.shape[:2] != (B, 15) or len(airs) != B:
            raise XfgStarkError(9, "debug_constraint_eval: trace [B,7,n], airs [B], coeffs [B,15,ext]")
        ext = co.shape[2]
        arr = (_AirConsts * B)(*[_air_struct(a) for a in airs])
        ce = np.zeros((B, ext, 2 * n), dtype=np.uint64)
        st = _lib.xfg_debug_constraint_eval(self._ctx, B, n, blowup, ext, tr.ctypes.data_as(_u64p), arr,
                                            co.ctypes.data_as(_u64p), ce.ctypes.data_as(_u64p))
        if st:
            raise self._err(st)
        return ce

    def debug_fri_fold(self, vals, alpha, logn, logbeta, coset_major, fold=8):
        import numpy as np
        v = np.ascontiguousarray(vals, dtype=np.uint64)
        al = np.ascontiguousarray(alpha, dtype=np.uint64)
        B, ext, D = v.shape
        if D != 1 << (logn + logbeta) or al.shape != (B, ext):
            raise XfgStarkError(9, "debug_fri_fold: vals [B,ext,2^(logn+logbeta)], alpha [B,ext]")
        if not 0 < fold < 1 << 32:
            raise XfgStarkError(9, "debug_fri_fold: fold is 2, 4, 8 or 16")
        out = np.zeros((B, ext, D // fold), dtype=np.uint64)
        st = _lib.xfg_debug_fri_fold_f(self._ctx, B, ext, logn, logbeta, 1 if coset_major else 0, fold,
                                       v.ctypes.data_as(_u64p), al.ctypes.data_as(_u64p), out.ctypes.data_as(_u64p))
        if st:
            raise self._err(st)
        return out

    FIELD_OPS = {"mul": 0, "add": 1, "sub": 2, "canon": 3, "pow2": 4, "fold": 5, "sub_weak": 6, "add_w": 7, "mul2": 8,
                 "mul2_pair": 9, "e2_mul": 10, "e2_mulb": 11, "e2_inv": 12}

    def debug_field(self, op, a, b):
        import numpy as np
        x = np.ascontiguousarray(a, dtype=np.uint64)
        y = np.ascontiguousarray(b, dtype=np.uint64)
        out = np.zeros_like(x)
        st = _lib.xfg_debug_field(self._ctx, self.FIELD_OPS[op], x.size, x.ctypes.data_as(_u64p),
                                  y.ctypes.data_as(_u64p), out.ctypes.data_as(_u64p))
        if st:
            raise self._err(st)
        return out

    def debug_coin_draws(self, seed, counter, k, ext=1, reject=(0, 0, 0, 0)):
        import numpy as np
        w = (C.c_uint32 * 8)(*np.frombuffer(bytes(seed), dtype="<u4").tolist())
        rej = np.array(reject, dtype=np.uint64)
        ow = np.zeros((k, 2), dtype=np.uint64)
        osq = np.zeros((k, 2), dtype=np.uint64)
        ctr = np.zeros(2, dtype=np.uint64)
        ok = (C.c_int * 2)()
        st = _lib.xfg_debug_coin_draws(self._ctx, w, counter, k, ext, rej.ctypes.data_as(_u64p),
                                       ow.ctypes.data_as(_u64p), osq.ctypes.data_as(_u64p),
                                       ctr.ctypes.data_as(_u64p), ok)
        if st:
            raise self._err(st)
        return ow, osq, (int(ctr[0]), int(ctr[1])), (ok[0], ok[1])

    def debug_grind(self, seeds, grind, first_nonce=1, max_nonce=0, chunk_log=0, blocks=0):
        import numpy as np
        k = len(seeds)
        if any(len(bytes(sd)) != 32 for sd in seeds):
            raise XfgStarkError(9, "debug_grind: seeds are 32 bytes each")
        w = np.frombuffer(b"".join(bytes(sd) for sd in seeds), dtype="<u4").copy()
        out = np.zeros(k, dtype=np.uint64)
        st = _lib.xfg_debug_grind(self._ctx, k, w.ctypes.data_as(C.POINTER(C.c_uint32)), grind, first_nonce, max_nonce,
                                  chunk_log, blocks, out.ctypes.data_as(_u64p))
        if st:
            raise self._err(st)
        return [int(v) for v in out]

    def grind_probe(self):
        dmin, dev, host = C.c_uint32(), C.c_uint64(), C.c_uint64()
        st = _lib.xfg_grind_probe(self._ctx, C.byref(dmin), C.byref(dev), C.byref(host))
        if st:
            raise self._err(st)
        return dmin.value, dev.value, host.value

    def debug_merkle_lde(self, lde, entries=()):
        import numpy as np
        v = np.ascontiguousarray(lde, dtype=np.uint64)
        ent = np.ascontiguousarray(entries, dtype=np.uint64)
        B, nc, blowup, n = v.shape
        nodes = np.zeros((B, 2 * n, 8), dtype="<u4")
        local = np.zeros((ent.size, 2 * blowup, 8), dtype="<u4")
        st = _lib.xfg_debug_merkle_lde(self._ctx, B, nc, n, blowup, v.ctypes.data_as(_u64p), ent.ctypes.data_as(_u64p),
                                       ent.size, nodes.ctypes.data_as(_u8p), local.ctypes.data_as(_u8p))
        if st:
            raise self._err(st)
        return nodes, local

    def debug_merkle_lde_const(self, lde, flags=None, vals=None, entries=()):
        import numpy as np
        v = np.ascontiguousarray(lde, dtype=np.uint64)
        ent = np.ascontiguousarray(entries, dtype=np.uint64)
        B, nc, blowup, n = v.shape
# ... 61 lines not shown
```

Before: 20380 proofs/s.

## Detect columns shared across proofs and skip constant columns in OOD/DEEP

Extends constant-column detection to also flag trace columns that are identical to the same column of the first proof in the batch, and adds a shared-column read path in the LDE/Merkle gather. OOD and DEEP kernels gain a constant-column template variant that skips loads and multiply-accumulates for constant columns and folds their values in once. The goal is to avoid redundant memory traffic and arithmetic for columns that are constant or duplicated across the batch. The cost is an extra comparison pass during detection and more template instantiations and branching.

```diff
diff --git a/include/xfg_stark.h b/include/xfg_stark.h
--- a/include/xfg_stark.h
+++ b/include/xfg_stark.h
@@ -131,6 +131,8 @@
                           uint64_t* out);
 int xfg_debug_const_columns(xfg_ctx* ctx, const uint64_t* trace, uint32_t count, uint32_t width, uint64_t n,
                             uint8_t* flags_out);
+int xfg_debug_col_classes(xfg_ctx* ctx, const uint64_t* trace, uint32_t count, uint64_t n, uint8_t* classes_out,
+                          uint64_t* vals_out);
 int xfg_debug_lde_skip(xfg_ctx* ctx, const uint64_t* coef, uint32_t npoly, uint64_t n, uint32_t blowup,
                        const uint8_t* skip, uint64_t* out);
 int xfg_debug_interpolate_skip(xfg_ctx* ctx, const uint64_t* evals, uint32_t npoly, uint64_t n, int offset7,
@@ -143,6 +145,11 @@
                          const uint32_t* coin_seeds, const uint64_t* coin_counters, uint64_t ginv, uint64_t* ood_out,
                          uint64_t* deep_out, uint64_t* dp_out, uint32_t* seeds_out, uint64_t* counters_out,
                          int* fail_out);
+int xfg_debug_ood_deep_const(xfg_ctx* ctx, uint32_t count, uint64_t n, uint32_t ext, const uint64_t* coef,
+                             const uint8_t* flags, const uint64_t* vals, const uint64_t* hcoef, const uint64_t* zpts,
+                             const uint64_t* coeffs, const uint32_t* coin_seeds, const uint64_t* coin_counters,
+                             uint64_t ginv, uint64_t* ood_out, uint64_t* deep_out, uint64_t* dp_out,
+                             uint32_t* seeds_out, uint64_t* counters_out, int* fail_out);
 int xfg_debug_constraint_eval(xfg_ctx* ctx, uint32_t count, uint64_t n, uint32_t blowup, uint32_t ext,
                               const uint64_t* trace, const xfg_air_consts* airs, const uint64_t* coeffs,
                               uint64_t* ce);
diff --git a/xfg-stark_amd/csrc/debug_abi.hip b/xfg-stark_amd/csrc/debug_abi.hip
--- a/xfg-stark_amd/csrc/debug_abi.hip
+++ b/xfg-stark_amd/csrc/debug_abi.hip
@@ -249,6 +249,26 @@
         launch_const_detect(L->trace.p, (int)cols, (int)ilog2(n), L->const_col.p, L->stream);
         HIPCHK(hipMemcpyAsync(flags_out, L->const_col.p, cols, hipMemcpyDeviceToHost, L->stream));
         HIPCHK(hipStreamSynchronize(L->stream));
+        return XFG_OK;
+    });
+}
+
+int xfg_debug_col_classes(xfg_ctx* c, const uint64_t* trace, uint32_t count, uint64_t n, uint8_t* classes_out,
+                          uint64_t* vals_out) {
+    if (!c || !trace || !classes_out || count == 0 || !is_pow2(n) || n < 8 || (uint64_t)count * 7 > 0xFFFF)
+        return XFG_INVALID_ARGUMENT;
+    return on_lane0(c, [&](Lane* L) -> int {
+        const size_t cols = (size_t)count * 7;
+        L->trace.ensure(cols * n);
+        L->const_col.ensure(const_flag_bytes(cols));
+        L->const_val.ensure(cols);
+        HIPCHK(hipMemcpy(L->trace.p, trace, cols * n * 8, hipMemcpyHostToDevice));
+        HIPCHK(hipMemsetAsync(L->const_val.p, 0xFF, cols * 8, L->stream));
+        launch_const_detect(L->trace.p, (int)cols, (int)ilog2(n), L->const_col.p, L->stream, 7, L->const_val.p);
+        HIPCHK(hipMemcpyAsync(classes_out, L->const_col.p, cols, hipMemcpyDeviceToHost, L->stream));
+        if (vals_out) HIPCHK(hipMemcpyAsync(vals_out, L->const_val.p, cols * 8, hipMemcpyDeviceToHost, L->stream));
+        HIPCHK(hipStreamSynchronize(L->stream));
+        for (size_t k = 0; k < cols; k++) classes_out[k] = (uint8_t)col_class(classes_out[k]);
         return XFG_OK;
     });
 }
@@ -338,9 +358,26 @@
                          const uint32_t* coin_seeds, const uint64_t* coin_counters, uint64_t ginv, uint64_t* ood_out,
                          uint64_t* deep_out, uint64_t* dp_out, uint32_t* seeds_out, uint64_t* counters_out,
                          int* fail_out) {
+    return xfg_debug_ood_deep_const(c, count, n, ext, coef, nullptr, nullptr, hcoef, zpts, coeffs, coin_seeds,
+                                    coin_counters, ginv, ood_out, deep_out, dp_out, seeds_out, counters_out, fail_out);
+}
+
+int xfg_debug_ood_deep_const(xfg_ctx* c, uint32_t count, uint64_t n, uint32_t ext, const uint64_t* coef,
+                             const uint8_t* flags, const uint64_t* vals, const uint64_t* hcoef, const uint64_t* zpts,
+                             const uint64_t* coeffs, const uint32_t* coin_seeds, const uint64_t* coin_counters,
+                             uint64_t ginv, uint64_t* ood_out, uint64_t* deep_out, uint64_t* dp_out, uint32_t* seeds_out,
+                             uint64_t* counters_out, int* fail_out) {
     if (!c) return XFG_INVALID_ARGUMENT;
     c->err.clear();
     const bool coin = coin_seeds != nullptr;
+    if (flags) {
+        bool ok = vals != nullptr && count <= 0xFFFF;
+        for (size_t k = 0; ok && k < (size_t)count * 7; k++) ok = flags[k] <= 2 && !(k < 7 && flags[k] == 2);
+        if (!ok) {
+            c->err = "xfg_debug_ood_deep_const: flags are 0, 1 or 2 (never 2 for instance 0) and come with vals";
+            return XFG_INVALID_ARGUMENT;
+        }
+    }
     if ((ext != 1 && ext != 2) || !is_pow2(n) || n < 8 || n > (1ULL << 21) || count == 0 || count > 0xFFFF) {
         c->err = "xfg_debug_ood_deep: ext is 1 or 2, n a power of two in [8, 2^21], count in [1, 65535]";
         return XFG_INVALID_ARGUMENT;
@@ -372,6 +409,19 @@
         HIPCHK(hipMemcpyAsync(L->coef.p, coef, B * 7 * n * 8, hipMemcpyHostToDevice, s));
         HIPCHK(hipMemcpyAsync(L->hcoef.p, hcoef, B * D * n * 8, hipMemcpyHostToDevice, s));
         HIPCHK(hipMemcpyAsync(L->zpts.p, zpts, B * 2 * D * 8, hipMemcpyHostToDevice, s));
+        ColConst cc;
+        if (flags) {
+            const size_t cols = B * 7;
+            L->const_col.ensure((cols + 3) & ~(size_t)3);
+            L->const_val.ensure(cols);
+            HIPCHK(hipMemcpyAsync(L->const_col.p, flags, cols, hipMemcpyHostToDevice, s));
+            HIPCHK(hipMemcpyAsync(L->const_val.p, vals, cols * 8, hipMemcpyHostToDevice, s));
+            for (size_t k = 0; k < cols; k++)
+                if (flags[k]) HIPCHK(hipMemsetAsync(L->coef.p + k * n, 0xFF, n * 8, s));
+            cc.flags = L->const_col.p;
+            cc.vals = L->const_val.p;
+            cc.val_stride = 1;
+        }
         const size_t nblk = ood_partial_count(logn);
         HIPCHK(hipMemsetAsync(L->partial.p, 0xFF, B * nblk * 15 * D * 8, s));
         HIPCHK(hipMemsetAsync(L->carry.p, 0xFF, B * nblk * 2 * D * 8, s));
@@ -395,8 +445,8 @@
             dc.zpts = L->zpts.p;
             dc.dp = L->dp.p;
             dc.ginv = ginv;
-            launch_ood(L->coef.p, L->hcoef.p, L->zpts.p, L->partial.p, L->ood.p, logn, (int)B, (int)ext, s, dc);
-            launch_deep(L->coef.p, L->hcoef.p, L->dp.p, L->partial.p, L->carry.p, L->deep.p, logn, (int)B, (int)ext, s);
+            launch_ood(L->coef.p, L->hcoef.p, L->zpts.p, L->partial.p, L->ood.p, logn, (int)B, (int)ext, s, dc, cc);
+            launch_deep(L->coef.p, L->hcoef.p, L->dp.p, L->partial.p, L->carry.p, L->deep.p, logn, (int)B, (int)ext, s, cc);
             std::vector<DeepParams> dps(B);
             HIPCHK(hipMemcpyAsync(ood_out, L->ood.p, B * 15 * D * 8, hipMemcpyDeviceToHost, s));
             HIPCHK(hipMemcpyAsync(deep_out, L->deep.p, B * D * n * 8, hipMemcpyDeviceToHost, s));
@@ -412,7 +462,7 @@
             }
             return XFG_OK;
         }
-        launch_ood(L->coef.p, L->hcoef.p, L->zpts.p, L->partial.p, L->ood.p, logn, (int)B, (int)ext, s);
+        launch_ood(L->coef.p, L->hcoef.p, L->zpts.p, L->partial.p, L->ood.p, logn, (int)B, (int)ext, s, DeepCoinStep{}, cc);
         HIPCHK(hipMemcpyAsync(ood_out, L->ood.p, B * 15 * D * 8, hipMemcpyDeviceToHost, s));
         HIPCHK(hipStreamSynchronize(s));
         std::vector<DeepParams> dps(B);
@@ -442,7 +492,7 @@
             put(dp.c2, c2);
         }
         HIPCHK(hipMemcpyAsync(L->dp.p, dps.data(), B * sizeof(DeepParams), hipMemcpyHostToDevice, s));
-        launch_deep(L->coef.p, L->hcoef.p, L->dp.p, L->partial.p, L->carry.p, L->deep.p, logn, (int)B, (int)ext, s);
+        launch_deep(L->coef.p, L->hcoef.p, L->dp.p, L->partial.p, L->carry.p, L->deep.p, logn, (int)B, (int)ext, s, cc);
         HIPCHK(hipMemcpyAsync(deep_out, L->deep.p, B * D * n * 8, hipMemcpyDeviceToHost, s));
         HIPCHK(hipStreamSynchronize(s));
         return XFG_OK;
diff --git a/xfg-stark_amd/csrc/kernels.hip b/xfg-stark_amd/csrc/kernels.hip
--- a/xfg-stark_amd/csrc/kernels.hip
+++ b/xfg-stark_amd/csrc/kernels.hip
@@ -89,10 +89,10 @@
 #pragma unroll
         for (int c = 0; c < 7; c++) {
             if ((rc.mask >> c) & 1) cur[c] = rc.v[c];
-            else cur[c] = lde[(((u64)c << a.logbeta) + t) * n + m];
+            else cur[c] = rc.plane(c, lde, a.lde)[(((u64)c << a.logbeta) + t) * n + m];
         }
         if ((rc.mask >> 4) & 1) nxt4 = rc.v[4];
-        else nxt4 = lde[((4ULL << a.logbeta) + t) * n + mn];
+        else nxt4 = rc.plane(4, lde, a.lde)[((4ULL << a.logbeta) + t) * n + mn];
     } else {
 #pragma unroll
         for (int c = 0; c < 7; c++) cur[c] = lde[(((u64)c << a.logbeta) + t) * n + m];
@@ -215,9 +215,9 @@
     return v;
 }
 
-template <int D>
+template <int D, bool CC>
 __global__ __launch_bounds__(256) void ood_kernel(const u64* coef, const u64* hcoef, const u64* zpts, u64* partial,
-                                                  int logn) {
+                                                  int logn, ColConst colc) {
     using F = FE<D>;
     __shared__ u64 zb[4][D];
     __shared__ u64 red[4][15][D];
@@ -235,12 +235,17 @@
     F acc[15];
 #pragma unroll
     for (int q = 0; q < 15; q++) acc[q] = F::zero();
-    u64 cur[7], nxt[7];
+    RowConst rc = {};
+    if constexpr (CC) rc = row_const_uniform(colc, (u64)proof);
+    auto live = [&](int c) { return !CC || !((rc.mask >> c) & 1); };
+    auto col = [&](int c) { return (CC ? rc.plane(c, co, coef) : co) + (u64)c * n; };
+    u64 cur[7] = {}, nxt[7] = {};
     F hc, hn;
     {
         const u64 j = base + t;
 #pragma unroll
-        for (int c = 0; c < 7; c++) cur[c] = co[(u64)c * n + j];
+        for (int c = 0; c < 7; c++)
+            if (live(c)) cur[c] = col(c)[j];
         hc = fe_plane<D>(h, n, j);
     }
 #pragma unroll
@@ -248,11 +253,13 @@
         if (r + 1 < OOD_R) {
             const u64 j = base + (u64)(r + 1) * T + t;
 #pragma unroll
-            for (int c = 0; c < 7; c++) nxt[c] = co[(u64)c * n + j];
+            for (int c = 0; c < 7; c++)
+                if (live(c)) nxt[c] = col(c)[j];
             hn = fe_plane<D>(h, n, j);
         }
 #pragma unroll
         for (int c = 0; c < 7; c++) {
+            if (!live(c)) continue;
             acc[2 * c] = fe_add(acc[2 * c], fe_mulb(pz, cur[c]));
             acc[2 * c + 1] = fe_add(acc[2 * c + 1], fe_mulb(pzg, cur[c]));
         }
@@ -282,6 +289,11 @@
         const int q = qc / D, cc = qc % D;
         u64 v = red[0][q][cc];
         for (int w = 1; w < (T + 63) / 64; w++) v = gl_add(v, red[w][q][cc]);
+        if constexpr (CC) {
+#pragma unroll
+            for (int c = 0; c < 7; c++)
+                if ((q >> 1) == c && q < 14 && ((rc.mask >> c) & 1)) v = (blockIdx.x == 0 && cc == 0) ? rc.v[c] : 0;
+        }
         partial[((u64)proof * gridDim.x + blockIdx.x) * 15 * D + qc] = v;
     }
 }
@@ -361,13 +373,17 @@
     deep_coin_block(dc, proof, o, d);
 }
 void launch_ood(const u64* coef, const u64* hcoef, const u64* zpts, u64* partial, u64* ood, int logn, int npoly,
-                int ext, hipStream_t s, const DeepCoinStep& dc) {
+                int ext, hipStream_t s, const DeepCoinStep& dc, const ColConst& cc) {
     const u64 n = 1ULL << logn;
     const int T = ood_threads(n), nblk = (int)(n / ((u64)T * OOD_R));
-    if (ext == 2)
-        hipLaunchKernelGGL(ood_kernel<2>, dim3(nblk, npoly), dim3(T), 0, s, coef, hcoef, zpts, partial, logn);
-    else
-        hipLaunchKernelGGL(ood_kernel<1>, dim3(nblk, npoly), dim3(T), 0, s, coef, hcoef, zpts, partial, logn);
+    const dim3 g(nblk, npoly), b(T);
+    if (cc.flags) {
+        if (ext == 2) hipLaunchKernelGGL((ood_kernel<2, true>), g, b, 0, s, coef, hcoef, zpts, partial, logn, cc);
+        else hipLaunchKernelGGL((ood_kernel<1, true>), g, b, 0, s, coef, hcoef, zpts, partial, logn, cc);
+    } else {
+        if (ext == 2) hipLaunchKernelGGL((ood_kernel<2, false>), g, b, 0, s, coef, hcoef, zpts, partial, logn, cc);
+        else hipLaunchKernelGGL((ood_kernel<1, false>), g, b, 0, s, coef, hcoef, zpts, partial, logn, cc);
+    }
     hipLaunchKernelGGL(ood_final_kernel, dim3(npoly), dim3(dc.coins ? 128 : 64), 0, s, partial, nblk, ext, ood, dc);
     XFG_CHECK_LAUNCH();
 }
@@ -423,9 +439,9 @@
     }
 }
 __device__ __forceinline__ int dpad(int i) { return i + i / OOD_R; }
-template <int D>
+template <int D, bool CC>
 __global__ __launch_bounds__(256) void deep_final_kernel(const u64* coef, const u64* hcoef, const DeepParams* dp,
-                                                         const u64* carry, u64* deep, int logn) {
+                                                         const u64* carry, u64* deep, int logn, ColConst colc) {
     using F = FE<D>;
     constexpr int R = OOD_R, CHMAX = 256 * OOD_R, PADN = CHMAX + CHMAX / R;
     __shared__ u64 s1[D][PADN], s2[D][PADN];
@@ -450,13 +466,29 @@
         arr[0][k] = v.a;
         if constexpr (D == 2) arr[1][k] = v.b;
     };
+    RowConst rc = {};
+    if constexpr (CC) rc = row_const_uniform(colc, (u64)proof);
 #pragma unroll 2
     for (int r = 0; r < R; r++) {
         const int li = r * T + t;
         const u64 j = base + li;
         F sacc = F::zero();
 #pragma unroll
-        for (int c = 0; c < 7; c++) sacc = fe_add(sacc, fe_mulb(ac[c], co[(u64)c * n + j]));
+        for (int c = 0; c < 7; c++) {
+            if constexpr (CC) {
+                if ((rc.mask >> c) & 1) continue;
+                sacc = fe_add(sacc, fe_mulb(ac[c], rc.plane(c, co, coef)[(u64)c * n + j]));
+            } else {
+                sacc = fe_add(sacc, fe_mulb(ac[c], co[(u64)c * n + j]));
+            }
+        }
+        if constexpr (CC) {
+            if (j == 0) {
+#pragma unroll
+                for (int c = 0; c < 7; c++)
+                    if ((rc.mask >> c) & 1) sacc = fe_add(sacc, fe_mulb(ac[c], rc.v[c]));
+            }
+        }
         F p1 = fe_add(sacc, fe_mul(gam, fe_plane<D>(h, n, j))), p2 = sacc;
         if (j == 0) {
             p1 = fe_sub(p1, F::load(P.c1));
@@ -519,19 +551,22 @@
     }
 }
 void launch_deep(const u64* coef, const u64* hcoef, const DeepParams* dp, const u64* partial, u64* carry, u64* deep,
-                 int logn, int npoly, int ext, hipStream_t s) {
+                 int logn, int npoly, int ext, hipStream_t s, const ColConst& cc) {
     const u64 n = 1ULL << logn;
     const int T = ood_threads(n), nblk = (int)(n / ((u64)T * OOD_R));
     int logch = 0;
     while ((1ULL << logch) < (u64)T * OOD_R) logch++;
     int ct = 64;
     while (ct < nblk) ct <<= 1;
-    if (ext == 2) {
-        hipLaunchKernelGGL(deep_carry_kernel<2>, dim3(npoly), dim3(ct), 0, s, partial, dp, carry, nblk, logch);
-        hipLaunchKernelGGL(deep_final_kernel<2>, dim3(nblk, npoly), dim3(T), 0, s, coef, hcoef, dp, carry, deep, logn);
+    const dim3 g(nblk, npoly), b(T);
+    if (ext == 2) hipLaunchKernelGGL(deep_carry_kernel<2>, dim3(npoly), dim3(ct), 0, s, partial, dp, carry, nblk, logch);
+    else hipLaunchKernelGGL(deep_carry_kernel<1>, dim3(npoly), dim3(ct), 0, s, partial, dp, carry, nblk, logch);
+    if (cc.flags) {
+        if (ext == 2) hipLaunchKernelGGL((deep_final_kernel<2, true>), g, b, 0, s, coef, hcoef, dp, carry, deep, logn, cc);
+        else hipLaunchKernelGGL((deep_final_kernel<1, true>), g, b, 0, s, coef, hcoef, dp, carry, deep, logn, cc);
     } else {
-        hipLaunchKernelGGL(deep_carry_kernel<1>, dim3(npoly), dim3(ct), 0, s, partial, dp, carry, nblk, logch);
-        hipLaunchKernelGGL(deep_final_kernel<1>, dim3(nblk, npoly), dim3(T), 0, s, coef, hcoef, dp, carry, deep, logn);
+        if (ext == 2) hipLaunchKernelGGL((deep_final_kernel<2, false>), g, b, 0, s, coef, hcoef, dp, carry, deep, logn, cc);
+        else hipLaunchKernelGGL((deep_final_kernel<1, false>), g, b, 0, s, coef, hcoef, dp, carry, deep, logn, cc);
     }
     XFG_CHECK_LAUNCH();
 }
@@ -622,7 +657,9 @@
     } else {
         u64 v;
         const u64 plane = src >> g.cc_shift;
-        if (k == g.cc_seg && g.cc.flags[plane]) v = g.cc.vals[plane * g.cc.val_stride];
+        const unsigned f = k == g.cc_seg ? g.cc.flags[plane] : 0u;
+        if (f & COL_CONST) v = g.cc.vals[plane * g.cc.val_stride];
+        else if (f & COL_SHARED) v = ((const u64*)g.src[k])[src - ((plane - plane % 7) << g.cc_shift)];
         else v = ((const u64*)g.src[k])[src];
         ((u64*)g.dst[k])[i - g.first[k]] = v;
     }
diff --git a/xfg-stark_amd/csrc/kernels.hpp b/xfg-stark_amd/csrc/kernels.hpp
--- a/xfg-stark_amd/csrc/kernels.hpp
+++ b/xfg-stark_amd/csrc/kernels.hpp
@@ -41,7 +41,12 @@
 void launch_interpolate(const u64* evals, u64 in_stride, u64* out, u64 out_stride, u64* scratch, int npoly, int logn,
                         bool off7, u64 keep, const Tables& T, hipStream_t s, const unsigned char* skip = nullptr);
 constexpr int CONST_DETECT_SPAN = 1024, CONST_FILL_SPAN = 4096;
-void launch_const_detect(const u64* cols, int ncols, int logn, unsigned char* flags, hipStream_t s);
+constexpr unsigned char COL_CONST = 1, COL_SHARED = 2;
+__host__ __device__ constexpr size_t detect_same_off(size_t ncols) { return (ncols + 3) & ~(size_t)3; }
+constexpr size_t const_flag_bytes(size_t ncols) { return 2 * detect_same_off(ncols); }
+__host__ __device__ constexpr int col_class(unsigned char f) { return (f & COL_CONST) ? 1 : ((f & COL_SHARED) ? 2 : 0); }
+void launch_const_detect(const u64* cols, int ncols, int logn, unsigned char* flags, hipStream_t s, int period = 0,
+                         u64* vals = nullptr);
 void launch_const_fill(const unsigned char* flags, const u64* src, u64 src_stride, u64* coef, u64* lde, int ncols,
                        int logn, int logbeta, hipStream_t s);
 
@@ -51,8 +56,11 @@
     u64 val_stride = 0;
 };
 struct RowConst {
-    unsigned mask;
+    unsigned mask, shared;
     u64 v[7];
+    __device__ __forceinline__ const u64* plane(int c, const u64* own, const u64* first) const {
+        return (shared >> c) & 1 ? first : own;
+    }
 };
 __device__ __forceinline__ RowConst row_const_uniform(const ColConst& cc, u64 proof) {
     const u64 o = proof * 7;
@@ -61,10 +69,15 @@
     u64 bytes = ((u64)w[0] | ((u64)w[1] << 32)) >> (8 * r);
     if (r >= 2) bytes |= (u64)w[2] << (64 - 8 * r);
     RowConst rc;
-    rc.mask = 0;
+    rc.mask = rc.shared = 0;
 #pragma unroll
-    for (int c = 0; c < 7; c++) rc.mask |= ((bytes >> (8 * c)) & 0xFF ? 1u : 0u) << c;
+    for (int c = 0; c < 7; c++) {
+        const unsigned f = (unsigned)(bytes >> (8 * c)) & 0xFF;
+        rc.mask |= (f & COL_CONST ? 1u : 0u) << c;
+        rc.shared |= ((f & (COL_CONST | COL_SHARED)) == COL_SHARED ? 1u : 0u) << c;
+    }
     rc.mask = __builtin_amdgcn_readfirstlane(rc.mask);
+    rc.shared = __builtin_amdgcn_readfirstlane(rc.shared);
 #pragma unroll
     for (int c = 0; c < 7; c++) {
         rc.v[c] = 0;
@@ -79,11 +92,13 @@
 }
 __device__ __forceinline__ RowConst row_const_lane(const ColConst& cc, u64 proof) {
     RowConst rc;
-    rc.mask = 0;
+    rc.mask = rc.shared = 0;
 #pragma unroll
     for (int c = 0; c < 7; c++) {
         rc.v[c] = cc.vals[(proof * 7 + c) * cc.val_stride];
-        rc.mask |= (cc.flags[proof * 7 + c] ? 1u : 0u) << c;
+        const unsigned f = cc.flags[proof * 7 + c];
+        rc.mask |= (f & COL_CONST ? 1u : 0u) << c;
+        rc.shared |= ((f & (COL_CONST | COL_SHARED)) == COL_SHARED ? 1u : 0u) << c;
     }
     return rc;
 }
@@ -132,10 +147,10 @@
                             int logbeta, int npoly, int ext, hipStream_t s, const ColConst& cc = ColConst{});
 
 void launch_ood(const u64* coef, const u64* hcoef, const u64* zpts, u64* partial, u64* ood, int logn, int npoly,
-                int ext, hipStream_t s, const DeepCoinStep& dc = DeepCoinStep{});
+                int ext, hipStream_t s, const DeepCoinStep& dc = DeepCoinStep{}, const ColConst& cc = ColConst{});
 u64 ood_partial_count(int logn);
 void launch_deep(const u64* coef, const u64* hcoef, const DeepParams* dp, const u64* partial, u64* carry, u64* deep,
-                 int logn, int npoly, int ext, hipStream_t s);
+                 int logn, int npoly, int ext, hipStream_t s, const ColConst& cc = ColConst{});
 
 __device__ __forceinline__ u64 layer_at(const u64* base, bool coset_major, int logn, int logbeta, u64 K) {
     if (!coset_major) return base[K];
diff --git a/xfg-stark_amd/csrc/lane_unit.hip b/xfg-stark_amd/csrc/lane_unit.hip
--- a/xfg-stark_amd/csrc/lane_unit.hip
+++ b/xfg-stark_amd/csrc/lane_unit.hip
@@ -25,7 +25,8 @@
     c->coef.ensure(B * 7 * sh.n);
     c->scratch.ensure(B * 7 * sh.N);
     c->lde.ensure(B * 7 * sh.N);
-    c->const_col.ensure((B * 7 + 3) & ~(size_t)3);
+    c->const_col.ensure(const_flag_bytes(B * 7));
+    c->const_val.ensure(B * 7);
 }
 void size_constraint_eval(Lane* c, size_t B, const ProofShape& sh) {
     c->air.ensure(B);
@@ -138,16 +139,19 @@
 ColConst trace_const(const Lane* c, const ProofShape& sh) {
     ColConst cc;
     cc.flags = c->const_col.p;
-    cc.vals = c->coef.p;
-    cc.val_stride = sh.n;
+    cc.vals = c->const_val.p;
+    cc.val_stride = 1;
     return cc;
 }
 
 void launch_trace_lde(Lane* c, const Tables& T, int B, const ProofShape& sh, bool probe) {
     hipStream_t s = c->stream;
     const unsigned char* skip = c->const_col.p;
-    if (c->poison_lde) HIPCHK(hipMemsetAsync(c->lde.p, 0xFF, (size_t)B * 7 * sh.N * 8, s));
-    launch_const_detect(c->trace.p, B * 7, sh.logn, c->const_col.p, s);
+    if (c->poison_lde) {
+        HIPCHK(hipMemsetAsync(c->lde.p, 0xFF, (size_t)B * 7 * sh.N * 8, s));
+        HIPCHK(hipMemsetAsync(c->coef.p, 0xFF, (size_t)B * 7 * sh.n * 8, s));
+    }
+    launch_const_detect(c->trace.p, B * 7, sh.logn, c->const_col.p, s, 7, c->const_val.p);
     launch_interpolate(c->trace.p, sh.n, c->coef.p, sh.n, c->scratch.p, B * 7, sh.logn, false, sh.n, T, s, skip);
     if (probe) {
         if (!c->lde_ev[0]) {
@@ -158,7 +162,6 @@
     }
     launch_lde(c->coef.p, sh.n, c->lde.p, c->scratch.p, B * 7, sh.logn, sh.logbeta, T, s, skip);
     if (probe) HIPCHK(hipEventRecord(c->lde_ev[1], s));
-    launch_const_fill(skip, c->trace.p, sh.n, c->coef.p, nullptr, B * 7, sh.logn, sh.logbeta, s);
 }
 
 static void enqueue_fri_layers(Lane* c, const Tables& T, int B, const ProofShape& sh, int fold, CoinStep& cs,
@@ -289,9 +292,9 @@
     dc.zpts = c->zpts.p;
     dc.dp = c->dp.p;
     dc.ginv = gl_inv(g);
-    launch_ood(c->coef.p, c->hcoef.p, c->zpts.p, c->partial.p, c->ood.p, logn, B, DE, s, dc);
+    launch_ood(c->coef.p, c->hcoef.p, c->zpts.p, c->partial.p, c->ood.p, logn, B, DE, s, dc, cc);
     stage_mark(c, 6);
-    launch_deep(c->coef.p, c->hcoef.p, c->dp.p, c->partial.p, c->carry.p, c->deep.p, logn, B, DE, s);
+    launch_deep(c->coef.p, c->hcoef.p, c->dp.p, c->partial.p, c->carry.p, c->deep.p, logn, B, DE, s, cc);
     launch_lde(c->deep.p, n, c->f0.p, c->scratch.p, B * DE, logn, logbeta, T, s);
     HIPCHK(hipMemcpy2DAsync(c->dn2.p, 8, c->deep.p + (n - 2), n * 8, 8, (size_t)B * DE, hipMemcpyDeviceToDevice, s));
     stage_mark(c, 7);
@@ -374,8 +377,12 @@
     const ReplayView rv = enqueue_commit_chain(c, T, ce_div, jobs, B, ts, sh, o, g, ht);
     HIPCHK(hipStreamSynchronize(c->stream));
     ht.mark("sync_rem");
-    u64 live_cols = 0;
-    for (int k = 0; k < B * 7; k++) live_cols += c->h_const_col[k] ? 0 : 1;
+    u64 live_cols = 0, shared_cols = 0;
+    for (int k = 0; k < B * 7; k++) {
+        const int cls = col_class(c->h_const_col[k]);
+        live_cols += cls == 0 ? 1 : 0;
+        shared_cols += cls == 2 ? 1 : 0;
+    }
     pool.parallel_for(B, [jobs, B, &sh, g, &rv](int b) { replay_transcript(jobs[b], b, B, sh, g, rv); });
 
     const auto t_q0 = clk::now();
@@ -424,7 +431,7 @@
         else if (key != TRACE_KEY_VALID)
             jobs[b].status = (key >> 62) == TRACE_KEY_NONCANONICAL ? XFG_INVALID_ARGUMENT : XFG_INVALID_TRACE;
     }
-    ht.dump(B, (long)((u64)B * 7 - live_cols));
+    ht.dump(B, (long)((u64)B * 7 - live_cols - shared_cols), (long)shared_cols);
     if (c->lde_probe) {
         float ms = 0;
         HIPCHK(hipEventSynchronize(c->lde_ev[1]));
diff --git a/xfg-stark_amd/csrc/merkle.hip b/xfg-stark_amd/csrc/merkle.hip
--- a/xfg-stark_amd/csrc/merkle.hip
+++ b/xfg-stark_amd/csrc/merkle.hip
@@ -53,8 +53,11 @@
 }
 
 struct NoConst {};
+struct RowConstBack : RowConst {
+    u64 back;
+};
 template <bool CC>
-using RowConstOf = std::conditional_t<CC, RowConst, NoConst>;
+using RowConstOf = std::conditional_t<CC, RowConstBack, NoConst>;
 template <int NC, int LOGB, bool CC>
 __device__ __forceinline__ void lde_row(const u64* base, u64 n, u64 m, int t, const RowConstOf<CC>& rc, u64 (&row)[NC]) {
     static_assert(!CC || NC == 7, "constant columns are those of the trace");
@@ -65,8 +68,10 @@
                 row[c] = rc.v[c];
                 continue;
             }
+            row[c] = (base - ((rc.shared >> c) & 1 ? rc.back : 0))[((u64)c * (1 << LOGB) + t) * n + m];
+        } else {
+            row[c] = base[((u64)c * (1 << LOGB) + t) * n + m];
         }
-        row[c] = base[((u64)c * (1 << LOGB) + t) * n + m];
     }
 }
 
@@ -99,9 +104,15 @@
 }
 
 template <bool CC>
-__device__ __forceinline__ RowConstOf<CC> block_row_const(const ColConst& cc, int proof) {
-    if constexpr (CC) return row_const_uniform(cc, (u64)proof);
-    else return NoConst{};
+__device__ __forceinline__ RowConstOf<CC> block_row_const(const ColConst& cc, int proof, u64 back) {
+    if constexpr (CC) {
+        RowConstBack rc;
+        static_cast<RowConst&>(rc) = row_const_uniform(cc, (u64)proof);
+        rc.back = back;
+        return rc;
+    } else {
+        return NoConst{};
+    }
 }
 
 template <int NC, int LOGB, bool CC>
@@ -111,8 +122,9 @@
     const u64 n = 1ULL << logn;
     const int proof = blockIdx.y;
     const u64 m = (u64)blockIdx.x * blockDim.x + threadIdx.x;
-    const u64* base = lde + (u64)proof * NC * (1 << LOGB) * n;
-    const RowConstOf<CC> rc = block_row_const<CC>(cc, proof);
+    const u64 back = (u64)proof * NC * (1 << LOGB) * n;
+    const u64* base = lde + back;
+    const RowConstOf<CC> rc = block_row_const<CC>(cc, proof, back);
     Digest d = lde_subtree_wide<NC, LOGB, LOGB, CC>(base, n, m, 0, rc);
     block_tree_up(d, nodes_all + (u64)proof * node_stride, n, lds, blockDim.x / 4);
 }
@@ -127,8 +139,9 @@
     const u64 n = 1ULL << logn;
     const int proof = blockIdx.y, t = threadIdx.x, h = t & ((1 << LOGL) - 1), rl = t >> LOGL;
     const u64 m = (u64)blockIdx.x * RB + rl;
-    const u64* base = lde + (u64)proof * NC * (1 << LOGB) * n + (u64)h * (1 << (LOGB - LOGL)) * n;
-    const RowConstOf<CC> rc = block_row_const<CC>(cc, proof);
+    const u64 back = (u64)proof * NC * (1 << LOGB) * n;
+    const u64* base = lde + back + (u64)h * (1 << (LOGB - LOGL)) * n;
+    const RowConstOf<CC> rc = block_row_const<CC>(cc, proof, back);
     Digest d = lde_subtree_wide<NC, LOGB, LOGB - LOGL, CC>(base, n, m, 0, rc);
 #pragma unroll
     for (int k = 0; k < LOGL; k++) {
@@ -159,7 +172,10 @@
     const u64* base = lde + proof * NC * (1 << LOGB) * n;
     Digest* local = out + e * (2 << LOGB);
     RowConstOf<CC> rc;
-    if constexpr (CC) rc = row_const_lane(cc, proof);
+    if constexpr (CC) {
+        static_cast<RowConst&>(rc) = row_const_lane(cc, proof);
+        rc.back = proof * NC * (1 << LOGB) * n;
+    }
     u64 row[NC];
     lde_row<NC, LOGB, CC>(base, n, m, t, rc, row);
     Digest d = b3_hash_elems<NC>(row);
diff --git a/xfg-stark_amd/csrc/ntt.hip b/xfg-stark_amd/csrc/ntt.hip
--- a/xfg-stark_amd/csrc/ntt.hip
+++ b/xfg-stark_amd/csrc/ntt.hip
@@ -779,24 +779,53 @@
     ntt_launch(p.b, args, s);
 }
 
-__global__ void const_flags_init_kernel(unsigned char* flags, int count) {
+__global__ void const_flags_init_kernel(unsigned char* flags, int count, int period) {
     const int i = blockIdx.x * blockDim.x + threadIdx.x;
-    if (i < count) flags[i] = 1;
-}
-__global__ __launch_bounds__(256) void const_detect_kernel(const u64* cols, u64 n, unsigned char* flags) {
+    if (i >= count) return;
+    flags[i] = 1;
+    if (period) flags[detect_same_off(count) + i] = i >= period ? 1 : 0;
+}
+template <bool SHARE>
+__global__ __launch_bounds__(256) void const_detect_kernel(const u64* cols, u64 n, unsigned char* flags, int period,
+                                                           u64* vals) {
     const int col = blockIdx.y;
     const u64* c = cols + (u64)col * n;
     const u64 first = c[0];
     const u64 i0 = (u64)blockIdx.x * CONST_DETECT_SPAN, i1 = i0 + CONST_DETECT_SPAN < n ? i0 + CONST_DETECT_SPAN : n;
+    if (vals && blockIdx.x == 0 && threadIdx.x == 0) vals[col] = first;
     u64 diff = 0;
-    for (u64 i = i0 + threadIdx.x; i < i1; i += blockDim.x) diff |= c[i] ^ first;
+    if (SHARE && col >= period) {
+        const u64* c0 = cols + (u64)(col % period) * n;
+        u64 diff0 = 0;
+#pragma unroll 4
+        for (u64 i = i0 + threadIdx.x; i < i1; i += blockDim.x) {
+            const u64 x = c[i];
+            diff |= x ^ first;
+            diff0 |= x ^ c0[i];
+        }
+        if (diff0) flags[detect_same_off(gridDim.y) + col] = 0;
+    } else {
+        for (u64 i = i0 + threadIdx.x; i < i1; i += blockDim.x) diff |= c[i] ^ first;
+    }
     if (diff) flags[col] = 0;
 }
-void launch_const_detect(const u64* cols, int ncols, int logn, unsigned char* flags, hipStream_t s) {
+__global__ void const_class_kernel(unsigned char* flags, int count) {
+    const int i = blockIdx.x * blockDim.x + threadIdx.x;
+    if (i < count) flags[i] = flags[i] ? COL_CONST : (flags[detect_same_off(count) + i] ? COL_SHARED : 0);
+}
+void launch_const_detect(const u64* cols, int ncols, int logn, unsigned char* flags, hipStream_t s, int period,
+                         u64* vals) {
     const u64 n = 1ULL << logn;
-    hipLaunchKernelGGL(const_flags_init_kernel, dim3((unsigned)((ncols + 255) / 256)), dim3(256), 0, s, flags, ncols);
-    hipLaunchKernelGGL(const_detect_kernel, dim3((unsigned)((n + CONST_DETECT_SPAN - 1) / CONST_DETECT_SPAN), ncols),
-                       dim3((unsigned)std::min<u64>(256, n)), 0, s, cols, n, flags);
+    if (period <= 0 || ncols <= period) period = 0;
+    const dim3 gi((unsigned)((ncols + 255) / 256)), bi(256);
+    hipLaunchKernelGGL(const_flags_init_kernel, gi, bi, 0, s, flags, ncols, period);
+    const dim3 g((unsigned)((n + CONST_DETECT_SPAN - 1) / CONST_DETECT_SPAN), ncols), b((unsigned)std::min<u64>(256, n));
+    if (period) {
+        hipLaunchKernelGGL(const_detect_kernel<true>, g, b, 0, s, cols, n, flags, period, vals);
+        hipLaunchKernelGGL(const_class_kernel, gi, bi, 0, s, flags, ncols);
+    } else {
+        hipLaunchKernelGGL(const_detect_kernel<false>, g, b, 0, s, cols, n, flags, period, vals);
+    }
 }
 __global__ __launch_bounds__(256) void const_fill_kernel(const unsigned char* flags, const u64* src, u64 src_stride,
                                                          u64* coef, u64* lde, u64 n, int logbeta) {
diff --git a/xfg-stark_amd/csrc/prover_internal.hpp b/xfg-stark_amd/csrc/prover_internal.hpp
--- a/xfg-stark_amd/csrc/prover_internal.hpp
+++ b/xfg-stark_amd/csrc/prover_internal.hpp
@@ -53,6 +53,7 @@
     DBuf<DevCoin> dcoin;
     DBuf<int> dfail;
     DBuf<unsigned char> const_col;
+    DBuf<u64> const_val;
     const unsigned char* h_const_col = nullptr;
     DBuf<u64> tkeys;
     const u64* h_tkeys = nullptr;
@@ -136,10 +137,11 @@
     void mark(const char* what) {
         if (trace_on()) m.push_back({what, std::chrono::steady_clock::now()});
     }
-    void dump(int B, long const_cols = -1) {
+    void dump(int B, long const_cols = -1, long shared_cols = -1) {
         if (!trace_on() || m.size() < 2) return;
         std::string line = "[xfg] B=" + std::to_string(B);
         if (const_cols >= 0) line += " const_cols=" + std::to_string(const_cols);
+        if (shared_cols >= 0) line += " shared_cols=" + std::to_string(shared_cols);
         for (size_t i = 1; i < m.size(); i++) {
             char buf[96];
             snprintf(buf, sizeof buf, " %s=%.2f", m[i].first,
diff --git a/xfg-stark_amd/xfgstark/__init__.py b/xfg-stark_amd/xfgstark/__init__.py
--- a/xfg-stark_amd/xfgstark/__init__.py
+++ b/xfg-stark_amd/xfgstark/__init__.py
@@ -116,6 +116,11 @@
     _lib.xfg_debug_merkle_lde_const.argtypes = [C.c_void_p, C.c_uint32, C.c_uint32, C.c_uint64, C.c_uint32, _u64p, _u8p,
                                                 _u64p, _u64p, C.c_uint64, _u8p, _u8p]
     _lib.xfg_debug_poison_lde.argtypes = [C.c_void_p, C.c_int]
+if hasattr(_lib, "xfg_debug_col_classes"):
+    _lib.xfg_debug_col_classes.argtypes = [C.c_void_p, _u64p, C.c_uint32, C.c_uint64, _u8p, _u64p]
+    _lib.xfg_debug_ood_deep_const.argtypes = [C.c_void_p, C.c_uint32, C.c_uint64, C.c_uint32, _u64p, _u8p, _u64p, _u64p,
+                                              _u64p, _u64p, C.POINTER(C.c_uint32), _u64p, C.c_uint64, _u64p, _u64p,
+                                              _u64p, C.POINTER(C.c_uint32), _u64p, C.POINTER(C.c_int)]
 if hasattr(_lib, "xfg_debug_fri_fold_f"):
     _lib.xfg_debug_fri_fold_f.argtypes = [C.c_void_p, C.c_uint32, C.c_uint32, C.c_uint32, C.c_uint32, C.c_int,
                                           C.c_uint32, _u64p, _u64p, _u64p]
@@ -771,6 +776,43 @@
         if st:
             raise self._err(st)
         return out
+
+    def debug_col_classes(self, trace, values=False):
+        import numpy as np
+        tr = np.ascontiguousarray(trace, dtype=np.uint64)
+        B, width, n = tr.shape
+        if width != 7:
+            raise XfgStarkError(9, "debug_col_classes: trace [B,7,n]")
+        out = np.zeros((B, 7), dtype=np.uint8)
+        vals = np.zeros((B, 7), dtype=np.uint64)
+        st = _lib.xfg_debug_col_classes(self._ctx, tr.ctypes.data_as(_u64p), B, n, out.ctypes.data_as(_u8p),
+                                        vals.ctypes.data_as(_u64p))
+        if st:
+            raise self._err(st)
+        return (out, vals) if values else out
+
+    def debug_ood_deep_const(self, coef, flags, vals, hcoef, zpts, coeffs):
+        import numpy as np
+        c = np.ascontiguousarray(coef, dtype=np.uint64)
+        hc = np.ascontiguousarray(hcoef, dtype=np.uint64)
+        zp = np.ascontiguousarray(zpts, dtype=np.uint64)
+        co = np.ascontiguousarray(coeffs, dtype=np.uint64)
+        f = np.ascontiguousarray(flags, dtype=np.uint8)
+        v = np.ascontiguousarray(vals, dtype=np.uint64)
+        B, _, n = c.shape
+        ext = hc.shape[1]
+        if (c.shape[1] != 7 or hc.shape != (B, ext, n) or zp.shape != (B, 2, ext) or co.shape != (B, 8, ext)
+                or f.shape != (B, 7) or v.shape != (B, 7)):
+            raise XfgStarkError(9, "debug_ood_deep_const: coef [B,7,n], flags and vals [B,7], hcoef [B,ext,n], "
+                                   "zpts [B,2,ext], coeffs [B,8,ext]")
+        ood = np.zeros((B, 15, ext), dtype=np.uint64)
+        deep = np.zeros((B, ext, n), dtype=np.uint64)
+        p = lambda a: a.ctypes.data_as(_u64p)
+        st = _lib.xfg_debug_ood_deep_const(self._ctx, B, n, ext, p(c), f.ctypes.data_as(_u8p), p(v), p(hc), p(zp), p(co),
+                                           None, None, 0, p(ood), p(deep), None, None, None, None)
+        if st:
+            raise self._err(st)
+        return ood, deep
 
     def debug_ood_deep(self, coef, hcoef, zpts, coeffs):
         import numpy as np
```

After: 22090 proofs/s (median of 6 runs). +8.4%, better.
